# lim0606/pytorch-ardae-vae

Measured on AMD Instinct MI355X. Metric: AR-DAE-VAE train-steps/sec (batch 512, nz_cdae 256) on dbMNIST, higher is better.
Workload: dtype f32

## Files before the change

include/ardae_hip.h:

```cpp
#ifndef ARDAE_HIP_H
#define ARDAE_HIP_H

#include <stddef.h>
#include <stdint.h>

#ifdef __cplusplus
extern "C" {
#endif

#define ARDAE_ABI_VERSION 1

enum { ARDAE_ACT_NONE = 0, ARDAE_ACT_RELU = 1, ARDAE_ACT_SOFTPLUS = 2, ARDAE_ACT_ELU = 3, ARDAE_ACT_TANH = 4, ARDAE_ACT_LEAKY_RELU = 5, ARDAE_ACT_SWISH = 6 };

enum {
  ARDAE_EPI_ACT = 0,
  ARDAE_EPI_DACT = 1,
  ARDAE_EPI_CHAIN = 2,
  ARDAE_EPI_DAE_LOSS = 3
};

typedef struct ardae_lin_src {
  const float* x;
  int ld;
  int K;
  const float* wp;
} ardae_lin_src;

typedef struct ardae_linear_args {
  int M, Nout;
  int nsrc;
  ardae_lin_src src[2];
  int act;
  const float* bias;
  const float* rowbias;
  int rowbias_ld;
  int rows_per_group;
  const float* rowscale;
  const float* rowscale_w;
  const float* S; int ldS;
  const float* R; int ldR;
  const float* Q; int ldQ;
  const float* sigma;
  const float* eps; int ldeps;
  float scale;
  float* Y;  int ldY;
  float* Y2; int ldY2;
  float* colsum;
  float* tile_loss;
} ardae_linear_args;

const char* ardae_last_error(void);
int ardae_abi_version(void);

size_t ardae_packed_floats(int nout, int k);
int ardae_linear_row_tiles(int M, int nout);
int ardae_linear_col_panels(int M, int nout);
int ardae_pack_weight(const float* W, int ldw, int nout, int k, int transpose, float* out, void* stream);
int ardae_linear(const ardae_linear_args* args, int epilogue, void* stream);
int ardae_linear_chain_eligible(const ardae_linear_args* layers, int nl, int epilogue);
int ardae_linear_chain(const ardae_linear_args* layers, int nl, int epilogue, void* stream);
int ardae_linear_wide_layers_eligible(const ardae_linear_args* layers, int nl, int epilogue);
int ardae_linear_wide_layers(const ardae_linear_args* layers, int nl, int epilogue, void* stream);


#define ARDAE_WGRAD_MAX_PROBLEMS 20
typedef struct ardae_wgrad_problem {
  int M, O, I;
  int npairs;
  const float* G[2]; int ldG[2];
  const float* X[2]; int ldX[2];
  int bias_pair;
  const float* rowscale;
  int splits;
  float* partial;
  float* partial_vec;
  float* out; int ldout;
  float* out_bias;
  float* out_rowscale; int ld_rowscale;
  float beta;
} ardae_wgrad_problem;
int ardae_wgrad_splits(int M, int O, int I, int nproblems_hint);
int ardae_wgrad_batch(const ardae_wgrad_problem* problems, int nproblems, void* stream);


int ardae_latent_perturb(const float* latent, const float* z0, const float* xi, const float* eps, int B, int nz, int z,
                         float std_scale, float delta, float* xbar, float* sigma, float* std_b, void* stream);
int ardae_latent_perturb_nstd(const float* latent, const float* z0, const float* xi, const float* eps, int B, int nz, int nstd, int z,
                              float std_scale, float delta, float* xbar, float* sigma, float* std_b, void* stream);
int ardae_latent_perturb_draw_ok(int nz, int nstd, int z);
int ardae_latent_perturb_draw(const float* latent, const float* z0, int B, int nz, int z, float std_scale, float delta, uint64_t seed,
                              uint64_t offset_xi, uint64_t offset_eps, const void* state, uint64_t first_row, float* xbar, float* sigma,
                              float* eps_out, float* std_b, void* stream);
int ardae_center_scale(const float* latent, const float* z0, int B, int nz, int z, float std_scale, float* u, void* stream);
int ardae_philox_normal(float* out, int64_t n, uint64_t seed, uint64_t offset, void* stream);
int ardae_philox_uniform(float* out, int64_t n, uint64_t seed, uint64_t offset, void* stream);
int ardae_bernoulli(const float* p, int64_t rows, int cols, float* out, uint64_t seed, uint64_t offset, void* stream);
int ardae_adam_ref_step(float* p, const float* g, float* exp_avg, float* exp_avg_sq, float* max_exp_avg_sq, int64_t n,
                        double lr, double beta1, double beta2, double eps, int step, void* stream);
#define ARDAE_STEP_STATE_BYTES 32
int ardae_step_state_advance(void* state, uint64_t rng_inc, double lr, double beta1, double beta2, void* stream);
int ardae_philox_normal_dev(float* out, int64_t n, uint64_t seed, const void* state, uint64_t offset_add, void* stream);
int ardae_philox_normal_at(float* out, int64_t n, uint64_t seed, uint64_t offset, const void* state, uint64_t first_element,
                           void* stream);
int ardae_adam_ref_step_dev(float* p, const float* g, float* exp_avg, float* exp_avg_sq, float* max_exp_avg_sq, int64_t n,
                            double beta1, double beta2, double eps, const void* state, void* stream);
int ardae_train_state_advance(void* state, uint64_t rng_inc, double lr, double beta1, double beta2, double beta_init, double beta_fin,
                              int64_t beta_annealing, double std_scale, int64_t seed_rows, void* stream);
int ardae_seed_scale_dev(float* g, int64_t n, const void* state, void* stream);
#define ARDAE_WEIGHT_AVG_SWA 0
#define ARDAE_WEIGHT_AVG_POLYAK 1
int ardae_weight_avg(float* avg, const float* p, int64_t n, int kind, double decay, int64_t origin, const void* state, int64_t t,
                     void* stream);
int ardae_rmsprop_step(float* p, const float* g, float* square_avg, float* momentum_buffer, int64_t n, double lr,
                       double alpha, double eps, double momentum, void* stream);
int ardae_sgd_step(float* p, const float* g, int64_t n, double lr, void* stream);

typedef struct ardae_cdae_desc {
  int kind;
  int input_dim;
  int context_dim;
  int h_dim;
  int n_layers;
  int act;
} ardae_cdae_desc;
size_t ardae_cdae_param_floats(const ardae_cdae_desc* d);
size_t ardae_cdae_packed_floats(const ardae_cdae_desc* d);
size_t ardae_cdae_workspace_floats(const ardae_cdae_desc* d, int B, int S, int need_grads);
int ardae_cdae_pack(const ardae_cdae_desc* d, const float* params, float* packed, void* stream);
int ardae_cdae_loss_grads(const ardae_cdae_desc* d, const float* params, const float* packed, const float* xbar,
                          const float* sigma, const float* eps, const float* ctx, int B, int S, float* workspace,
                          size_t workspace_floats, float* loss, float* grads, float* score_out, void* stream);
int ardae_cdae_perturb_fused_ok(const ardae_cdae_desc* d, int nz, int nstd);
int ardae_cdae_perturb_loss_grads(const ardae_cdae_desc* d, const float* params, const float* packed, const float* latent, const float* z0,
                                  const float* ctx, int B, int nz, float std_scale, float delta, uint64_t seed, uint64_t offset_xi,
                                  uint64_t offset_eps, const void* state, uint64_t first_row, float* xbar, float* sigma, float* eps_out,
                                  float* std_b, float* workspace, size_t workspace_floats, float* loss, float* grads, void* stream);
int ardae_cdae_score(const ardae_cdae_desc* d, const float* params, const float* packed, const float* x,
                     const float* sigma, const float* ctx, int B, int S, float* workspace, size_t workspace_floats,
                     float* score_out, void* stream);


int ardae_dae_perturb(const float* x , const float* sigma , const float* eps ,
                      int B, int nsigma, int d, float* xbar, void* stream);
int ardae_dae_perturb_fused_ok(const ardae_cdae_desc* d, int nsigma);
int ardae_dae_perturb_loss_grads(const ardae_cdae_desc* d, const float* params, const float* packed, const float* x, int B, int nsigma,
                                 float delta, uint64_t seed, uint64_t offset_sigma, uint64_t offset_eps, const void* state,
                                 uint64_t first_row, float* xbar, float* sigma, float* eps_out, float* workspace,
                                 size_t workspace_floats, float* loss, float* grads, void* stream);

int ardae_dae_noise_perturb(const float* x , const float* eps , int B, int nsigma, int d, float sigma,
                            const void* dae_state, float* xbar, float* sigma_out , void* stream);
int ardae_dae_state_advance(void* state, uint64_t rng_inc, double lr, double beta1, double beta2, double sigma_max, double sigma_min,
                            int64_t sigma_annealing, void* stream);

int ardae_latent_noise_perturb(const float* latent, const float* z0, const float* eps, int B, int nz, int nstd, int z, float std_scale, float sigma,
                               const void* dae_state, float* xbar, float* sigma_out, void* stream);
int ardae_latent_noise_perturb_draw_ok(int nz, int nstd, int z);
int ardae_latent_noise_perturb_draw(const float* latent, const float* z0, int B, int nz, int nstd, int z, float std_scale, float sigma,
                                    const void* dae_state, uint64_t seed, uint64_t offset_eps, uint64_t first_row, float* xbar, float* sigma_out,
                                    float* eps_out, void* stream);

int ardae_philox_uniform_at(float* out, int64_t n, uint64_t seed, uint64_t offset, const void* state, uint64_t first_element, void* stream);
int ardae_recon_perturb(const float* x , const float* draw , int B, int nsigma, int d, int noise, float sigma,
                        const void* dae_state, float* xbar, float* sigma_out, float* target_out, void* stream);
int ardae_recon_perturb_draw(const float* x, int B, int nsigma, int d, int noise, float sigma, const void* dae_state, uint64_t seed, uint64_t offset,
                             uint64_t first_row, float* xbar, float* sigma_out, float* target_out, float* draw_out, void* stream);
int ardae_latent_recon_perturb(const float* latent, const float* z0, const float* draw, int B, int nz, int nstd, int z, float std_scale, int noise,
                               float sigma, const void* dae_state, float* xbar, float* sigma_out, float* target_out, void* stream);
int ardae_latent_recon_perturb_draw(const float* latent, const float* z0, int B, int nz, int nstd, int z, float std_scale, int noise, float sigma,
                                    const void* dae_state, uint64_t seed, uint64_t offset, uint64_t first_row, float* xbar, float* sigma_out,
                                    float* target_out, float* draw_out, void* stream);
int ardae_recon_score(const float* recon, const float* x, int n, int d, float sigma, const void* dae_state, float* out, void* stream);

#define ARDAE_FIT_STATE_BYTES 48
enum { ARDAE_ENERGY_REG = 0, ARDAE_ENERGY_1 = 1, ARDAE_ENERGY_2 = 2, ARDAE_ENERGY_3 = 3, ARDAE_ENERGY_4 = 4, ARDAE_ENERGY_NORMAL = 5 };
int ardae_energy(int kind, const float* x, int R, int d, float mu, float logvar, float* energy, float* grad, void* stream);
size_t ardae_energy_partial_floats(int R);
int ardae_energy_seed(int kind, const float* x, const float* score, int R, int d, float mu, float logvar, float alpha,
                      const void* fit_state, float* seed, float* mean_energy, float* partial, void* stream);
size_t ardae_gen_param_floats(int z_dim, int h_dim, int n_layers, int out_dim, int act);
size_t ardae_gen_packed_floats(int z_dim, int h_dim, int n_layers, int out_dim, int act);
size_t ardae_gen_workspace_floats(int z_dim, int h_dim, int n_layers, int out_dim, int act, int B);
int ardae_gen_pack(int z_dim, int h_dim, int n_layers, int out_dim, int act, const float* params, float* packed, void* stream);
int ardae_gen_forward(int z_dim, int h_dim, int n_layers, int out_dim, int act, const float* params, const float* packed, const float* z,
                      int B, float* workspace, size_t workspace_floats, float* x_out, void* stream);
int ardae_gen_backward(int z_dim, int h_dim, int n_layers, int out_dim, int act, const float* params, const float* packed, const float* z,
                       const float* dx, int B, float* workspace, size_t workspace_floats, float* grads, void* stream);
int ardae_gen_draw_fused_ok(int z_dim, int h_dim, int n_layers, int out_dim, int act);
int ardae_gen_draw_forward(int z_dim, int h_dim, int n_layers, int out_dim, int act, const float* params, const float* packed, int B,
                           uint64_t seed, uint64_t offset, const void* state, float* z_out, float* workspace, size_t workspace_floats,
                           float* x_out, void* stream);
int ardae_adam_torch_step_dev(float* p, const float* g, float* exp_avg, float* exp_avg_sq, int64_t n, double beta1, double beta2,
                              double eps, const void* state, void* stream);
int ardae_fit_state_advance(void* fit_state, uint64_t rng_inc, double lr0, double beta1, double beta2, int64_t lr_step_size,
                            double lr_gamma, double lr_min, double alpha_init, double alpha_fin, int64_t alpha_annealing, void* stream);


typedef struct ardae_model_desc {
  int kind;
  int input_dim, noise_dim, h_dim, z_dim;
  int n_layers;
  int act;
  int flags;
} ardae_model_desc;
enum { ARDAE_MODEL_NO_CENTER = 1,
       ARDAE_MODEL_HEAD_SHIFT = 1, ARDAE_MODEL_HEAD_MASK = 7 << 1,
       ARDAE_MODEL_CLIPPED = 16,
       ARDAE_MODEL_CLIP_Z0_SHIFT = 8, ARDAE_MODEL_CLIP_Z_SHIFT = 12, ARDAE_MODEL_CLIP_MASK = 0xff00 };
size_t ardae_model_param_floats(const ardae_model_desc* d);
size_t ardae_model_packed_floats(const ardae_model_desc* d);
size_t ardae_model_workspace_floats(const ardae_model_desc* d, int B, int nz, int mode);
int ardae_model_pack(const ardae_model_desc* d, const float* params, float* packed, void* stream);
int ardae_model_encode(const ardae_model_desc* d, const float* params, const float* packed, const float* x,
                       const float* noise, int B, int nz, float* workspace, size_t workspace_floats, float* z_out,
                       void* stream);
int ardae_model_encode_pair(const ardae_model_desc* d, const float* params, const float* packed, const float* x,
                            const float* noise, int B, int nz, float* workspace, size_t workspace_floats, float* z0_out,
                            float* z_out, int phase, void* stream);
int ardae_model_vae_forward(const ardae_model_desc* d, const float* params, const float* packed, const float* x,
                            const float* noise, int B, int nz, float beta, float* workspace, size_t workspace_floats,
                            float* z_out, float* losses, void* stream);
int ardae_model_vae_forward_dev(const ardae_model_desc* d, const float* params, const float* packed, const float* x,
                                const float* noise, int B, int nz, const void* state, float* workspace, size_t workspace_floats,
                                float* z_out, float* losses, void* stream);
int ardae_model_encode_hidden(const ardae_model_desc* d, const float* params, const float* packed, const float* x, int B,
                              float* workspace, size_t workspace_floats, float* z0_out, float* hidden_out, void* stream);
int ardae_model_encode_hidden_raw(const ardae_model_desc* d, const float* params, const float* packed, const float* x, const float* raw0, int B,
                                  float* workspace, size_t workspace_floats, float* z0_out, float* hidden_out, void* stream);
int ardae_model_decode(const ardae_model_desc* d, const float* params, const float* packed, const float* z, int R,
                       float* workspace, size_t workspace_floats, float* out0, float* out1, void* stream);
int ardae_model_loss_rows(const ardae_model_desc* d, const float* out0, const float* out1, const float* x, const float* z,
                          int rows, int nz, float* recon_row, float* prior_row, void* stream);
int ardae_model_vae_backward(const ardae_model_desc* d, const float* params, const float* packed, const float* x,
                             const float* noise, int B, int nz, float beta, float dloss, const float* dz_extra,
                             float* workspace, size_t workspace_floats, float* grads, float grads_beta, void* stream);
int ardae_model_vae_backward_dev(const ardae_model_desc* d, const float* params, const float* packed, const float* x,
                                 const float* noise, int B, int nz, const void* state, float dloss, const float* dz_extra,
                                 float* workspace, size_t workspace_floats, float* grads, float grads_beta, void* stream);
int ardae_model_vae_backward_decoder(const ardae_model_desc* d, const float* params, const float* packed, const float* x,
                                     const float* noise, int B, int nz, float beta, float dloss, float* workspace,
                                     size_t workspace_floats, void* stream);
int ardae_model_vae_backward_sampler(const ardae_model_desc* d, const float* params, const float* packed, const float* x,
                                     const float* noise, int B, int nz, const float* dz_extra, float seed_scale,
                                     float* workspace, size_t workspace_floats, float* grads, float grads_beta, void* stream);
int ardae_model_vae_backward_decoder_dev(const ardae_model_desc* d, const float* params, const float* packed, const float* x,
                                         const float* noise, int B, int nz, const void* state, float dloss, float* workspace,
                                         size_t workspace_floats, void* stream);
int ardae_model_vae_backward_sampler_dev(const ardae_model_desc* d, const float* params, const float* packed, const float* x,
                                         const float* noise, int B, int nz, const float* dz_extra, const void* state,
                                         float* workspace, size_t workspace_floats, float* grads, float grads_beta, void* stream);


int ardae_vae_head_fused_ok(const ardae_model_desc* d);
int ardae_vae_kld_rows(const float* mu, const float* lv, int B, int z, float* kld, void* stream);
int ardae_vae_head(const ardae_model_desc* d, const float* params, const float* packed, const float* hid, const float* eps, int B, uint64_t seed,
                   uint64_t offset, const void* state, int variant, float* mu, float* lv, float* z_out, float* eps_out, float* kld, void* stream);
int ardae_vae_forward(const ardae_model_desc* d, const float* params, const float* packed, const float* x, const float* eps, int B, float beta,
                      float loss_scale, uint64_t seed, uint64_t offset, const void* state, float* workspace, size_t workspace_floats, float* z_out,
                      float* eps_out, float* losses, void* stream);
int ardae_vae_forward_dev(const ardae_model_desc* d, const float* params, const float* packed, const float* x, const float* eps, int B,
                          const void* beta_state, float loss_scale, uint64_t seed, uint64_t offset, const void* state, float* workspace,
                          size_t workspace_floats, float* z_out, float* eps_out, float* losses, void* stream);
int ardae_vae_backward(const ardae_model_desc* d, const float* params, const float* packed, const float* x, int B, float beta, float loss_scale,
                       float* workspace, size_t workspace_floats, float* grads, float grads_beta, void* stream);
int ardae_vae_backward_dev(const ardae_model_desc* d, const float* params, const float* packed, const float* x, int B, const void* beta_state,
                           float loss_scale, float* workspace, size_t workspace_floats, float* grads, float grads_beta, void* stream);
int ardae_vae_encode_stats(const ardae_model_desc* d, const float* params, const float* packed, const float* x, int B, float* workspace,
                           size_t workspace_floats, float* mu_out, float* lv_out, void* stream);
int ardae_vae_iwae_draw(const float* mu, const float* lv, const float* eps, int B, int k, int z, uint64_t seed, uint64_t offset,
                        uint64_t first_element, float* z_out, float* logq, float* eps_out, void* stream);

int ardae_vae_aux_elbo_rows(const ardae_model_desc* d, const float* params, const float* packed, const float* x, const float* eps, int B, uint64_t seed,
                            uint64_t offset0, uint64_t offset1, uint64_t first_image, float* workspace, size_t workspace_floats, float* recon_rows,
                            float* kld_rows, void* stream);
int ardae_vae_pair_kld_rows(const float* mu1, const float* lv1, const float* mu2, const float* lv2, int B, int n, float* kld, void* stream);
int ardae_vae_aux_iwae_draw(const ardae_model_desc* d, const float* params, const float* packed, const float* x, const float* mu0, const float* lv0,
                            const float* eps, int B, int k, uint64_t seed, uint64_t offset0, uint64_t offset1, uint64_t first_image, float* workspace,
                            size_t workspace_floats, float* z_out, float* logq, float* eps_out, void* stream);

size_t ardae_conv_tail_workspace_floats(const ardae_model_desc* d, int R, int variant);
int ardae_conv_tail(const ardae_model_desc* d, const float* params, const float* packed, const float* u1, int R, int variant, float* workspace,
                    size_t workspace_floats, float* logits, void* stream);

size_t ardae_resconv_tail_workspace_floats(const ardae_model_desc* d, int R, int variant);
int ardae_resconv_tail(const ardae_model_desc* d, const float* params, const float* packed, const float* y14, int R, int variant, float* workspace,
                       size_t workspace_floats, float* logits, void* stream);

size_t ardae_resconv_mid_workspace_floats(const ardae_model_desc* d, int R, int variant);
int ardae_resconv_mid(const ardae_model_desc* d, const float* params, const float* packed, const float* y8, int R, int variant, float* workspace,
                      size_t workspace_floats, float* y14, void* stream);

int ardae_relaxed_bernoulli(const float* logit, const float* u, int64_t n, float temperature, float* sample, float* mean,
                            void* stream);
int ardae_gaussian_sample(const float* mu, const float* logvar, const float* eps, int64_t n, float* sample, void* stream);
int ardae_cholesky_batched(const float* A, int batch, int n, float* L, void* stream);

int ardae_iwae_proposal(const float* zs, const float* prop_noise, int B, int ke, int k, int z, float jitter, uint64_t seed, uint64_t offset,
                        uint64_t first_element, float* newz, float* logq, float* eps_out, float* mu, float* chol, void* stream);
int ardae_iwae_reduce(const float* recon, const float* prior, const float* logq, int B, int k, float* out, void* stream);

int ardae_philox_normal_scaled_at(float* out, int64_t n, uint64_t seed, uint64_t offset, const void* state, uint64_t first_element, int width,
                                  int nslots, const float* scale, void* stream);
int ardae_sample_logvar(const float* z, int B, int nz, int zd, float eps, float* logvar, void* stream);
int ardae_hist2d(const float* pts, int64_t n, int64_t row_stride, int nslots, int64_t slot_stride, int col_x, int col_y, double lo, double hi,
                 int bins, int64_t* counts, void* stream);
int ardae_hist2d_wide(const float* pts, int64_t n, int64_t row_stride, int nslots, int64_t slot_stride, int col_x, int col_y, double lo, double hi,
                      int bins, int64_t* counts, void* stream);


#define ARDAE_LOG_RECORD_FLOATS 16
int ardae_log_scalars(const float* cdae_loss, const float* model_losses, const float* std_b, int B, float beta, float d_lr,
                      const void* state, float* ring, int capacity, void* stream);
int ardae_log_scalars_dev(const float* cdae_loss, const float* model_losses, const float* std_b, int B, const void* beta_state, float d_lr,
                          const void* state, float* ring, int capacity, void* stream);
int ardae_gather_rows(const float* table, const int64_t* idx, int B, int D, float* out, void* stream);


#define ARDAE_DP_UNIQUE_ID_BYTES 128
const char* ardae_dp_backend(void);
int ardae_dp_unique_id(void* host_id);
int ardae_dp_comm_create(const void* host_id, int nranks, int rank, void** comm_out);
int ardae_dp_comm_query(void* comm, int* nranks, int* rank, int* device);
int ardae_dp_comm_destroy(void* comm);
int ardae_dp_allreduce_mean(void* comm, float* buf, size_t n, void* stream);


typedef struct ardae_profile_entry {
  char name[96];
  int calls;
  double total_ms;
  double flops;
  double bytes;
} ardae_profile_entry;
int ardae_profile_enable(int on);
int ardae_debug_stamp(unsigned long long* slots, int slot, void* stream);
int ardae_profile_report(ardae_profile_entry* entries, int max_entries);

#ifdef __cplusplus
}
#endif
#endif
```

pytorch-ardae-vae_amd/csrc/cdae.hip:

```cpp
#include <vector>

#include "ardae_hip.h"
#include "common.h"
#include "elementwise.h"
#include "host_util.h"

namespace ardae {
namespace {

bool cond_kind(int kind) { return kind < 2 || kind == 10 || kind == 11 || kind == 13 || kind == 16 || kind == 17; }
bool input_encoder_kind(int kind) { return kind < 2 || kind == 10 || kind == 11; }
bool sigma_column_kind(int kind) { return kind < 4 || kind == 16 || kind == 17; }

struct CdaeLayout {
  int kind, z, c, h, L, act;
  bool cond, enc_inp, grad, has_sigma;
  std::vector<Lin> ctx, inp, neg;
  size_t total = 0;
  int k1() const { return enc_inp ? h : z; }
  int sigma_col() const { return cond ? k1() + h : z; }

  explicit CdaeLayout(const ardae_cdae_desc& d)
      : kind(d.kind), z(d.input_dim), c(d.context_dim), h(d.h_dim), L(d.n_layers), act(d.act), cond(cond_kind(d.kind)), enc_inp(input_encoder_kind(d.kind)), grad(d.kind % 2 == 0), has_sigma(sigma_column_kind(d.kind)) {
    size_t off = 0;
    auto add = [&](std::vector<Lin>& v, int out, int in) { v.push_back(next_lin(off, out, in)); };
    if (cond)
      for (int l = 0; l < L; ++l) add(ctx, h, l == 0 ? c : h);
    if (enc_inp)
      for (int l = 0; l < L; ++l) add(inp, h, l == 0 ? z : h);
    for (int l = 0; l < L; ++l) add(neg, h, l == 0 ? sigma_col() + (has_sigma ? 1 : 0) : h);
    add(neg, grad ? 1 : z, h);
    total = off;
  }
};

struct PackedLayout {
  std::vector<size_t> ctx_f, ctx_b, inp_f, inp_b, neg_f, neg_b;
  size_t w1_f, w1_b, w1c_f, w1c_b, w1s;
  size_t fc_f, fc_b;
  PackedLayout(const CdaeLayout& P, PackList& pl) {
    const size_t L = P.L;
    for (auto* v : {&ctx_f, &ctx_b, &inp_f, &inp_b, &neg_f, &neg_b}) v->assign(L, 0);
    if (P.cond)
      for (size_t l = 0; l < L; ++l) { pl.pair(P.ctx[l], ctx_f[l], ctx_b[l]); if (P.enc_inp) pl.pair(P.inp[l], inp_f[l], inp_b[l]); }
    const Lin& W1 = P.neg[0];
    pl.pair(W1, w1_f, w1_b, 0, P.k1());
    w1c_f = w1c_b = 0;
    if (P.cond) pl.pair(W1, w1c_f, w1c_b, P.k1(), P.h);
    w1s = P.has_sigma ? pl.take(P.h) : 0;
    for (size_t l = 1; l < L; ++l) pl.pair(P.neg[l], neg_f[l], neg_b[l]);
    fc_f = fc_b = 0;
    if (!P.grad) pl.pair(P.neg[L], fc_f, fc_b);
  }
  explicit PackedLayout(const CdaeLayout& P, PackList&& sizing = PackList()) : PackedLayout(P, sizing) {}
};

int desc_ok(const ardae_cdae_desc* d) {
  ARDAE_CHECK_ARG(d != nullptr, "cdae: desc is NULL");
  ARDAE_CHECK_ARG((d->kind >= 0 && d->kind <= 3) || d->kind == 6 || d->kind == 7 || d->kind == 10 || d->kind == 11 || d->kind == 13 || d->kind == 16 || d->kind == 17,
                  "cdae: kind must be 0 (mlp-grad), 1 (mlp-res), 2 (unconditional grad), 3 (unconditional res), 6 (plain DAE grad), 7 (plain DAE res), "
                  "10 (plain conditional DAE grad), 11 (plain conditional DAE res), 13 (conditional DAE without an input encoder), "
                  "16 (mlp-grad without an input encoder) or 17 (mlp-res without an input encoder)");
  ARDAE_CHECK_ARG(!cond_kind(d->kind) || d->context_dim >= 1, "cdae: kinds 0 / 1 / 10 / 11 / 13 / 16 / 17 need context_dim >= 1 (got %d)", d->context_dim);
  ARDAE_CHECK_ARG(cond_kind(d->kind) || d->context_dim == 0, "cdae: kinds 2 / 3 / 6 / 7 have no context: context_dim must be 0 (got %d)", d->context_dim);
  ARDAE_CHECK_ARG(d->input_dim >= 1 && d->h_dim >= 1 && d->n_layers >= 1, "cdae: bad dimensions");
  ARDAE_CHECK_ARG(d->n_layers <= 6, "cdae: n_layers <= 6 supported (3L+1 gradient problems per batch)");
  ARDAE_CHECK_ARG(d->act > ACT_NONE && d->act <= ACT_LAST, "cdae: unknown activation %d", d->act);
  return 0;
}

struct CdaeWs {
  std::vector<float*> cL, a, hh, e, r, tau, taup, pbar, qbar, chat;
  float *cb, *gbar, *gbuf, *tile_loss, *chain_cnt, *Qsum, *cs_taup;
  int ltiles, ctiles;
};

void cdae_carve(const CdaeLayout& P, Bump& ws, int B, int S, bool need_grads, CdaeWs& W) {
  const int N = B * S, h = P.h, L = P.L, z = P.z;
  const size_t Bh = (size_t)B * h, Nh = (size_t)N * h;
  const bool cond = P.cond, enc = P.enc_inp, score = enc || P.grad;
  for (auto* v : {&W.cL, &W.a, &W.hh, &W.e, &W.r, &W.tau, &W.taup, &W.pbar, &W.qbar, &W.chat}) v->assign(L + 1, nullptr);
  W.cb = W.chain_cnt = W.Qsum = W.cs_taup = nullptr;
  if (cond) {
    for (int l = 1; l <= L; ++l) W.cL[l] = ws.take(Bh);
    W.cb = ws.take(Bh);
  }
  for (int l = 1; l <= L; ++l) {
    if (enc) W.a[l] = ws.take(Nh);
    W.hh[l] = ws.take(Nh);
    if (score) W.e[l] = ws.take(Nh);
    if (enc) W.r[l] = ws.take(Nh);
  }
  if (need_grads)
    for (int l = 1; l <= L; ++l) {
      if (enc) W.tau[l] = ws.take(Nh);
      if (score) W.taup[l] = ws.take(Nh);
      if (enc) W.pbar[l] = ws.take(Nh);
      W.qbar[l] = ws.take(Nh);
    }
  W.gbar = ws.take((size_t)N * z);
  W.gbuf = ws.take((size_t)N * z);
  W.ltiles = linear_row_tiles(N, z) * linear_col_panels(N, z);
  W.tile_loss = ws.take(W.ltiles);
  if (enc) W.chain_cnt = ws.take((size_t)LINEAR_SMALL_CHAIN_COUNTER_WORDS * ((N + 15) / 16));
  W.ctiles = linear_row_tiles(N, h);
  if (!need_grads) return;
  if (cond) {
    W.Qsum = ws.take(Bh);
    for (int l = 1; l <= L; ++l) W.chat[l] = ws.take(Bh);
  }
  if (score) W.cs_taup = ws.take((size_t)W.ctiles * h);
}

void cdae_wgrads(const CdaeLayout& P, const CdaeWs& W, const float* xbar, const float* sigma, const float* ctx, int B, int S, WgradList& wl, Bump& ws) {
  const int N = B * S, h = P.h, L = P.L, z = P.z;
  const std::vector<float*>&a = W.a, &hh = W.hh, &e = W.e, &r = W.r, &tau = W.tau, &taup = W.taup, &qhat = W.qbar, &phat = W.pbar;
  const int ld1 = P.neg[0].in;
  const size_t gW1 = P.neg[0].w;
  auto push = [&](const Lin& lin, int I, const float* s, const float* t, const float* ghat, const float* x, bool first) {
    const bool scol = first && P.has_sigma;
    const float* rs = scol ? sigma : nullptr;
    float* out_rs = scol ? wl.g(gW1 + P.sigma_col()) : nullptr;
    const int ld = first ? ld1 : I, ld_rs = scol ? ld1 : 0;
    if (P.grad) wl.push2(N, h, I, s, t, I, ghat, x, I, 1, rs, wl.g(lin.w), ld, wl.g(lin.b), out_rs, ld_rs);
    else wl.push2(N, h, I, ghat, x, I, nullptr, nullptr, 0, 0, rs, wl.g(lin.w), ld, wl.g(lin.b), out_rs, ld_rs);
  };
  if (P.enc_inp)
    for (int l = 1; l <= L; ++l)
      push(P.inp[l - 1], l == 1 ? z : h, r[l], l == 1 ? W.gbar : tau[l - 1], phat[l], l == 1 ? xbar : a[l - 1], false);
  push(P.neg[0], P.k1(), e[1], P.enc_inp ? tau[L] : W.gbar, qhat[1], P.enc_inp ? a[L] : xbar, true);
  if (P.cond) wl.push2(B, h, h, W.Qsum, W.cL[L], h, nullptr, nullptr, 0, -1, nullptr, wl.g(gW1 + P.k1()), ld1, nullptr, nullptr, 0);
  for (int l = 2; l <= L; ++l)
    push(P.neg[l - 1], h, e[l], taup[l - 1], qhat[l], hh[l - 1], false);
  if (!P.grad) wl.push2(N, z, h, W.gbar, hh[L], h, nullptr, nullptr, 0, 0, nullptr, wl.g(P.neg[L].w), h, wl.g(P.neg[L].b), nullptr, 0);
  if (P.cond)
    for (int l = 1; l <= L; ++l)
      wl.push2(B, h, P.ctx[l - 1].in, W.chat[l], l == 1 ? ctx : W.cL[l - 1], l == 1 ? P.c : h, nullptr, nullptr, 0, 0, nullptr,
               wl.g(P.ctx[l - 1].w), P.ctx[l - 1].in, wl.g(P.ctx[l - 1].b), nullptr, 0);
  wl.assign(ws, P.cond ? 3 * L + 1 : L + 1);
}

size_t workspace_floats(const CdaeLayout& P, int B, int S, bool need_grads) {
  Bump ws;
  CdaeWs W;
  cdae_carve(P, ws, B, S, need_grads, W);
  if (need_grads) {
    WgradList wl(nullptr);
    cdae_wgrads(P, W, nullptr, nullptr, nullptr, B, S, wl, ws);
  }
  return ws.off;
}

int cdae_pack_impl(const CdaeLayout& P, const float* params, float* packed, hipStream_t st) {
  PackList pl(params, packed);
  const PackedLayout K(P, pl);
  if (P.has_sigma) ARDAE_TRY(launch_gather_strided(params + P.neg[0].w + P.sigma_col(), P.neg[0].in, P.h, packed + K.w1s, st));
  return pl.launch(st);
}

LinArgs lin_args(int act, int M, int Nout, const float* x, int ldx, int K, const float* wp, LinArgs a) {
  a.M = M; a.Nout = Nout; a.nsrc = 1; a.act = act;
  a.src[0].x = x; a.src[0].ld = ldx; a.src[0].K = K; a.src[0].wp = wp;
  return a;
}

struct LayerRun {
  int epi;
  hipStream_t st;
  bool one_by_one;
  std::vector<LinArgs> v;
  LayerRun(int epi_, hipStream_t st_, bool one_by_one_ = false) : epi(epi_), st(st_), one_by_one(one_by_one_) {}
  void add(const LinArgs& a) { v.push_back(a); }
  int flush() {
    size_t i = 0;
    while (i < v.size()) {
      size_t n = one_by_one ? 1 : v.size() - i;
      while (n >= 2 && !linear_chain_eligible(v.data() + i, (int)n, epi)) --n;
      if (n >= 2) {
        ARDAE_TRY(launch_linear_chain(v.data() + i, (int)n, epi, st));
        i += n;
        continue;
      }
      size_t m = one_by_one ? 1 : std::min<size_t>(v.size() - i, 6);
      while (m >= 2 && !linear_wide_layers_eligible(v.data() + i, (int)m, epi)) --m;
      if (m >= 2) {
        ARDAE_TRY(launch_linear_wide_layers(v.data() + i, (int)m, epi, st));
        i += m;
      } else {
        ARDAE_TRY(launch_linear(v[i], epi, st));
        i += 1;
      }
    }
    v.clear();
    return 0;
  }
};

int cdae_impl(const ardae_cdae_desc* d, const float* params, const float* packed, const float* xbar, const float* sigma,
              const float* eps, const float* ctx, int B, int S, float* workspace, size_t ws_floats, float* loss, float* grads,
              float* score_out, bool need_grads, hipStream_t st, bool first_ready = false) {
  ARDAE_TRY(desc_ok(d));
  const CdaeLayout P(*d);
  const bool cond = P.cond, grad = P.grad;
  const bool enc = P.enc_inp;
  ARDAE_CHECK_ARG(cond || ctx == nullptr, "cdae: kinds 2 / 3 / 6 / 7 take no context: ctx must be NULL");
  const bool ctx_ready = first_ready && cond && !enc;
  ARDAE_CHECK_ARG(params && packed && xbar && (sigma || (!P.has_sigma && !need_grads)) && (ctx || !cond) && workspace, "cdae: null pointer argument");
  ARDAE_CHECK_ARG(B > 0 && S > 0 && (int64_t)B * S < (int64_t)1 << 30, "cdae: bad batch (B=%d, S=%d)", B, S);
  ARDAE_CHECK_ARG(!need_grads || (eps && loss && grads), "cdae: loss/grads/eps must be given");
  ARDAE_CHECK_ARG(need_grads || score_out, "cdae: score_out is NULL");
  const PackedLayout K(P);
  const int N = B * S, h = P.h, L = P.L, z = P.z, act = P.act, k1 = P.k1();
  Bump ws(workspace, ws_floats);
  CdaeWs W;
  cdae_carve(P, ws, B, S, need_grads, W);
  WgradList wl(grads);
  if (need_grads) cdae_wgrads(P, W, xbar, sigma, ctx, B, S, wl, ws);
  ARDAE_CHECK_ARG(ws.ok, "cdae: workspace too small (%zu < %zu floats)", ws_floats, ws.off);
  const std::vector<float*>&cL = W.cL, &a = W.a, &hh = W.hh, &e = W.e, &r = W.r, &tau = W.tau, &taup = W.taup, &pbar = W.pbar, &qbar = W.qbar, &chat = W.chat;
  float *cb = W.cb, *gbar = W.gbar, *Qsum = W.Qsum, *cs_taup = W.cs_taup;
  float* g = score_out ? score_out : W.gbuf;
  const float* x1 = enc ? a[L] : xbar;
  const float* wfc = params + P.neg[L].w;

  auto ctx_layer = [&](int l) { LinArgs A{}; A.bias = params + P.ctx[l - 1].b; A.Y = cL[l]; A.ldY = h;
                                return lin_args(act, B, h, l == 1 ? ctx : cL[l - 1], l == 1 ? P.c : h, P.ctx[l - 1].in, packed + K.ctx_f[l - 1], A); };
  auto inp_layer = [&](int l) { LinArgs A{}; A.bias = params + P.inp[l - 1].b; A.Y = a[l]; A.ldY = h;
                                return lin_args(act, N, h, l == 1 ? xbar : a[l - 1], l == 1 ? z : h, P.inp[l - 1].in, packed + K.inp_f[l - 1], A); };
  auto ctx_bias = [&]() {
    LinArgs A{}; A.bias = params + P.neg[0].b; A.Y = cb; A.ldY = h;
    return lin_args(ACT_NONE, B, h, cL[L], h, h, packed + K.w1c_f, A);
  };
  auto energy_layer = [&](int l) {
    LinArgs A{}; A.Y = hh[l]; A.ldY = h;
    if (l == 1 && P.has_sigma) { A.rowscale = sigma; A.rowscale_w = packed + K.w1s; }
    if (l == 1 && cond) { A.rowbias = cb; A.rowbias_ld = h; A.rows_per_group = S; } else A.bias = params + P.neg[l - 1].b;
    if (grad && l == L) { A.Y2 = e[L]; A.ldY2 = h; A.R = wfc; }
    return l == 1 ? lin_args(act, N, h, x1, k1, k1, packed + K.w1_f, A) : lin_args(act, N, h, hh[l - 1], h, h, packed + K.neg_f[l - 1], A);
  };
  auto e_layer = [&](int l) {
    LinArgs A{}; A.S = hh[l - 1]; A.ldS = h; A.Y = e[l - 1]; A.ldY = h;
    return lin_args(act, N, h, e[l], h, h, packed + K.neg_b[l - 1], A);
  };
  auto r_layer = [&](int l) {
    LinArgs A{}; A.S = a[l - 1]; A.ldS = h; A.Y = r[l - 1]; A.ldY = h;
    return l > L ? lin_args(act, N, h, e[1], h, h, packed + K.w1_b, A) : lin_args(act, N, h, r[l], h, h, packed + K.inp_b[l - 1], A);
  };
  auto g_layer = [&](LinArgs A) {
    A.Y = g; A.ldY = z;
    if (grad) return lin_args(ACT_NONE, N, z, enc ? r[1] : e[1], h, h, packed + (enc ? K.inp_b[0] : K.w1_b), A);
    A.bias = params + P.neg[L].b;
    return lin_args(ACT_NONE, N, z, hh[L], h, h, packed + K.fc_f, A);
  };

  if (!need_grads && enc && grad && N == B && linear_small_eligible(inp_layer(1), EPI_ACT)) {
    std::vector<LinArgs> pr; std::vector<int> ep, lv;
    int level = 0;
    auto add = [&](const LinArgs& A, int epi, int lev) { pr.push_back(A); ep.push_back(epi); lv.push_back(lev); };
    for (int l = 1; l <= L; ++l, ++level) { add(ctx_layer(l), EPI_ACT, level); add(inp_layer(l), EPI_ACT, level); }
    add(ctx_bias(), EPI_ACT, level++);
    for (int l = 1; l <= L; ++l) add(energy_layer(l), EPI_ACT, level++);
    for (int l = L; l >= 2; --l) add(e_layer(l), EPI_DACT, level++);
    for (int l = L + 1; l >= 2; --l) add(r_layer(l), EPI_DACT, level++);
    add(g_layer(LinArgs{}), EPI_ACT, level++);
    return launch_linear_small_chain(pr.data(), ep.data(), lv.data(), (int)pr.size(), W.chain_cnt, st);
  }
  {
    LayerRun run(EPI_ACT, st);
    if (enc && !first_ready && linear_small_eligible(inp_layer(1), EPI_ACT)) {
      for (int l = 1; l <= L; ++l) ARDAE_TRY(launch_linear_pair(ctx_layer(l), inp_layer(l), EPI_ACT, st));
      ARDAE_TRY(launch_linear(ctx_bias(), EPI_ACT, st));
    } else if (cond) {
      if (!ctx_ready) {
        for (int l = 1; l <= L; ++l) ARDAE_TRY(launch_linear(ctx_layer(l), EPI_ACT, st));
        ARDAE_TRY(launch_linear(ctx_bias(), EPI_ACT, st));
      }
      if (enc) for (int l = first_ready ? 2 : 1; l <= L; ++l) run.add(inp_layer(l));
    }
    for (int l = !enc && first_ready ? 2 : 1; l <= L; ++l) run.add(energy_layer(l));
    ARDAE_TRY(run.flush());
  }
  if (grad) {
    LayerRun run(EPI_DACT, st);
    for (int l = L; l >= 2; --l) run.add(e_layer(l));
    if (enc) for (int l = L + 1; l >= 2; --l) run.add(r_layer(l));
    ARDAE_TRY(run.flush());
  }
  if (!need_grads) return launch_linear(g_layer(LinArgs{}), EPI_ACT, st);
  const float inv_nz = 1.0f / ((float)N * (float)z);
  {
    LinArgs A{}; A.sigma = sigma; A.eps = eps; A.ldeps = z; A.scale = inv_nz; A.Y2 = gbar; A.ldY2 = z; A.tile_loss = W.tile_loss;
    ARDAE_TRY(launch_linear(g_layer(A), EPI_DAE_LOSS, st));
  }
  ARDAE_TRY(launch_sum_scale(W.tile_loss, W.ltiles, inv_nz, loss, st));

  const std::vector<float*>&qhat = qbar, &phat = pbar;
  if (grad) {
    LayerRun run(EPI_CHAIN, st);
    if (enc)
      for (int l = 1; l <= L; ++l) {
        LinArgs A{}; A.S = a[l]; A.ldS = h; A.R = r[l]; A.ldR = h; A.Y = tau[l]; A.ldY = h; A.Y2 = pbar[l]; A.ldY2 = h;
        run.add(l == 1 ? lin_args(act, N, h, gbar, z, z, packed + K.inp_f[0], A) : lin_args(act, N, h, tau[l - 1], h, h, packed + K.inp_f[l - 1], A));
      }
    for (int l = 1; l <= L; ++l) {
      LinArgs A{}; A.S = hh[l]; A.ldS = h; A.R = e[l]; A.ldR = h; A.Y = taup[l]; A.ldY = h; A.Y2 = qbar[l]; A.ldY2 = h;
      if (l == L) A.colsum = cs_taup;
      run.add(l == 1 ? lin_args(act, N, h, enc ? tau[L] : gbar, k1, k1, packed + K.w1_f, A) : lin_args(act, N, h, taup[l - 1], h, h, packed + K.neg_f[l - 1], A));
    }
    ARDAE_TRY(run.flush());
    ARDAE_TRY(launch_segment_sum(cs_taup, h, 1, W.ctiles, h, -1.0f, grads + P.neg[L].w, h, st));
  } else {
    LinArgs A{}; A.S = hh[L]; A.ldS = h; A.Y = qhat[L]; A.ldY = h;
    ARDAE_TRY(lin1(EPI_DACT, act, N, h, gbar, z, z, packed + K.fc_b, A, st));
  }
  {
    LayerRun run(EPI_DACT, st, cond && !grad);
    for (int l = L; l >= 2; --l) {
      LinArgs A{}; A.S = hh[l - 1]; A.ldS = h; A.Y = qhat[l - 1]; A.ldY = h;
      if (grad) { A.Q = qbar[l - 1]; A.ldQ = h; }
      run.add(lin_args(act, N, h, qhat[l], h, h, packed + K.neg_b[l - 1], A));
    }
    if (enc)
      for (int l = L + 1; l >= 2; --l) {
        LinArgs A{}; A.S = a[l - 1]; A.ldS = h; A.Y = phat[l - 1]; A.ldY = h;
        if (grad) { A.Q = pbar[l - 1]; A.ldQ = h; }
        run.add(l > L ? lin_args(act, N, h, qhat[1], h, h, packed + K.w1_b, A) : lin_args(act, N, h, phat[l], h, h, packed + K.inp_b[l - 1], A));
      }
    ARDAE_TRY(run.flush());
  }
  if (cond) {
    ARDAE_TRY(launch_segment_sum(qhat[1], h, B, S, h, 1.0f, Qsum, h, st));
    for (int l = L + 1; l >= 2; --l) {
      LinArgs A{}; A.S = cL[l - 1]; A.ldS = h; A.Y = chat[l - 1]; A.ldY = h;
      ARDAE_TRY(lin1(EPI_DACT, act, B, h, l > L ? Qsum : chat[l], h, h, packed + (l > L ? K.w1c_b : K.ctx_b[l - 1]), A, st));
    }
  }

  return wl.launch(st);
}

}

int dae_front_slots(const ardae_cdae_desc* d, int N, float* workspace, size_t ws_floats, size_t* w1, size_t* b1, float** h1) {
  ARDAE_TRY(desc_ok(d));
  const CdaeLayout P(*d);
  ARDAE_CHECK_ARG(!P.cond, "dae_perturb_loss_grads: the network must be unconditional");
  const size_t need = workspace_floats(P, N, 1, true);
  ARDAE_CHECK_ARG(ws_floats >= need, "dae_perturb_loss_grads: workspace too small (%zu < %zu floats)", ws_floats, need);
  Bump ws(workspace, ws_floats);
  CdaeWs W;
  cdae_carve(P, ws, N, 1, true, W);
  *w1 = P.neg[0].w; *b1 = P.neg[0].b; *h1 = W.hh[1];
  return 0;
}
int dae_loss_grads_from_h1(const ardae_cdae_desc* d, const float* params, const float* packed, const float* xbar, const float* sigma, const float* eps,
                           int N, float* workspace, size_t ws_floats, float* loss, float* grads, hipStream_t st) {
  return cdae_impl(d, params, packed, xbar, sigma, eps, nullptr, N, 1, workspace, ws_floats, loss, grads, nullptr, true, st, true);
}

}

using namespace ardae;

extern "C" {

size_t ardae_cdae_param_floats(const ardae_cdae_desc* d) {
  if (desc_ok(d) != 0) return 0;
  return CdaeLayout(*d).total;
}
size_t ardae_cdae_packed_floats(const ardae_cdae_desc* d) {
  if (desc_ok(d) != 0) return 0;
  PackList pl;
  PackedLayout(CdaeLayout(*d), pl);
  return pl.total();
}
size_t ardae_cdae_workspace_floats(const ardae_cdae_desc* d, int B, int S, int need_grads) {
  if (desc_ok(d) != 0 || B <= 0 || S <= 0) return 0;
  return workspace_floats(CdaeLayout(*d), B, S, need_grads != 0);
}
int ardae_cdae_pack(const ardae_cdae_desc* d, const float* params, float* packed, void* stream) {
  ARDAE_TRY(desc_ok(d));
  ARDAE_CHECK_ARG(params && packed, "cdae_pack: null pointer");
  return cdae_pack_impl(CdaeLayout(*d), params, packed, (hipStream_t)stream);
}
int ardae_cdae_loss_grads(const ardae_cdae_desc* d, const float* params, const float* packed, const float* xbar,
                          const float* sigma, const float* eps, const float* ctx, int B, int S, float* workspace,
                          size_t workspace_floats, float* loss, float* grads, float* score_out, void* stream) {
  return cdae_impl(d, params, packed, xbar, sigma, eps, ctx, B, S, workspace, workspace_floats, loss, grads, score_out, true,
                   (hipStream_t)stream);
}
int ardae_cdae_perturb_fused_ok(const ardae_cdae_desc* d, int nz, int nstd) {
  if (desc_ok(d) != 0) return 0;
  const CdaeLayout P(*d);
  return P.cond && P.has_sigma && nstd == 1 && latent_perturb_draw_fwd_ok(nz, P.z, P.h, P.act) ? 1 : 0;
}
int ardae_cdae_perturb_loss_grads(const ardae_cdae_desc* d, const float* params, const float* packed, const float* latent, const float* z0,
                                  const float* ctx, int B, int nz, float std_scale, float delta, uint64_t seed, uint64_t offset_xi,
                                  uint64_t offset_eps, const void* state, uint64_t first_row, float* xbar, float* sigma, float* eps_out,
                                  float* std_b, float* workspace, size_t ws_floats, float* loss, float* grads, void* stream) {
  ARDAE_TRY(desc_ok(d));
  ARDAE_CHECK_ARG(ardae_cdae_perturb_fused_ok(d, nz, 1), "cdae_perturb_loss_grads: shape not eligible (nz=%d): use ardae_latent_perturb* + ardae_cdae_loss_grads", nz);
  ARDAE_CHECK_ARG(params && packed && workspace && B > 0, "cdae_perturb_loss_grads: null pointer argument");
  const CdaeLayout P(*d);
  const PackedLayout K(P);
  ARDAE_CHECK_ARG(ws_floats >= workspace_floats(P, B, nz, true), "cdae_perturb_loss_grads: workspace too small");
  Bump ws(workspace, ws_floats);
  CdaeWs W;
  cdae_carve(P, ws, B, nz, true, W);
  const hipStream_t st = (hipStream_t)stream;
  if (!P.enc_inp) {
    ARDAE_CHECK_ARG(latent && z0 && ctx && xbar && sigma && eps_out && std_b && loss && grads, "cdae_perturb_loss_grads: null pointer argument");
    const int h = P.h, L = P.L;
    for (int l = 1; l <= L; ++l) {
      LinArgs A{}; A.bias = params + P.ctx[l - 1].b; A.Y = W.cL[l]; A.ldY = h;
      ARDAE_TRY(launch_linear(lin_args(P.act, B, h, l == 1 ? ctx : W.cL[l - 1], l == 1 ? P.c : h, P.ctx[l - 1].in, packed + K.ctx_f[l - 1], A), EPI_ACT, st));
    }
    LinArgs A{}; A.bias = params + P.neg[0].b; A.Y = W.cb; A.ldY = h;
    ARDAE_TRY(launch_linear(lin_args(ACT_NONE, B, h, W.cL[L], h, h, packed + K.w1c_f, A), EPI_ACT, st));
    const bool seed_e = P.grad && L == 1;
    ARDAE_TRY(launch_latent_perturb_draw_fwd(latent, z0, B, nz, P.z, std_scale, delta, seed, offset_xi, offset_eps, state, first_row, xbar, sigma, eps_out,
                                             std_b, packed + K.w1_f, W.cb, h, P.act, W.hh[1], st, packed + K.w1s, seed_e ? params + P.neg[L].w : nullptr,
                                             seed_e ? W.e[1] : nullptr));
    return cdae_impl(d, params, packed, xbar, sigma, eps_out, ctx, B, nz, workspace, ws_floats, loss, grads, nullptr, true, st, true);
  }
  ARDAE_TRY(launch_latent_perturb_draw_fwd(latent, z0, B, nz, P.z, std_scale, delta, seed, offset_xi, offset_eps, state, first_row, xbar, sigma,
                                           eps_out, std_b, packed + K.inp_f[0], params + P.inp[0].b, P.h, P.act, W.a[1],
                                           (hipStream_t)stream));
  return cdae_impl(d, params, packed, xbar, sigma, eps_out, ctx, B, nz, workspace, ws_floats, loss, grads, nullptr, true, (hipStream_t)stream,
                   true);
}
int ardae_cdae_score(const ardae_cdae_desc* d, const float* params, const float* packed, const float* x, const float* sigma,
                     const float* ctx, int B, int S, float* workspace, size_t workspace_floats, float* score_out, void* stream) {
  return cdae_impl(d, params, packed, x, sigma, nullptr, ctx, B, S, workspace, workspace_floats, nullptr, nullptr, score_out, false,
                   (hipStream_t)stream);
}

}
```

pytorch-ardae-vae_amd/csrc/elementwise.h:

```cpp
#pragma once
#include "ardae_hip.h"
#include "common.h"

namespace ardae {

struct DevFloat {
  float v;
  const float* p;
  DevFloat(float v_) : v(v_), p(nullptr) {}
  explicit DevFloat(const float* p_) : v(0.f), p(p_) {}
};
DevFloat train_state_beta(const void* state);
DevFloat train_state_seed_scale(const void* state);

int launch_latent_perturb(const float* latent, const float* z0, const float* xi, const float* eps, int B, int nz, int nstd, int zd,
                          float std_scale, float delta, float* xbar, float* sigma, float* std_b, hipStream_t st);
bool latent_perturb_draw_ok(int nz, int nstd, int zd);
int launch_latent_perturb_draw(const float* latent, const float* z0, int B, int nz, int zd, float std_scale, float delta, uint64_t seed,
                               uint64_t off_xi, uint64_t off_eps, const void* state, uint64_t first_row, float* xbar, float* sigma,
                               float* eps_out, float* std_b, hipStream_t st);
bool latent_perturb_draw_fwd_ok(int nz, int zd, int h, int act);
int launch_latent_perturb_draw_fwd(const float* latent, const float* z0, int B, int nz, int zd, float std_scale, float delta, uint64_t seed,
                                   uint64_t off_xi, uint64_t off_eps, const void* state, uint64_t first_row, float* xbar, float* sigma,
                                   float* eps_out, float* std_b, const float* wp1, const float* bias1, int h, int act, float* a1_out,
                                   hipStream_t st, const float* w1s = nullptr, const float* wfc = nullptr, float* e1_out = nullptr);
int launch_center_scale(const float* latent, const float* z0, int B, int nz, int zd, float std_scale, float* u,
                        hipStream_t st);
int launch_segment_sum(const float* in, int ld, int groups, int rows_per_group, int cols, float scale, float* out, int ldout,
                       hipStream_t st);
int launch_sum_scale(const float* in, int n, float scale, float* out, hipStream_t st);
int launch_gather_strided(const float* src, int stride, int n, float* dst, hipStream_t st);
int launch_philox_normal(float* out, int64_t n, uint64_t seed, uint64_t offset, hipStream_t st);
int launch_philox_normal_dev(float* out, int64_t n, uint64_t seed, const void* state, uint64_t offset_add, hipStream_t st);
int launch_philox_normal_at(float* out, int64_t n, uint64_t seed, uint64_t offset, const void* state, uint64_t first_element, hipStream_t st);
int launch_step_state_advance(void* state, uint64_t rng_inc, double lr, double beta1, double beta2, hipStream_t st);
int launch_train_state_advance(void* state, uint64_t rng_inc, double lr, double beta1, double beta2, double beta_init, double beta_fin,
                               int64_t beta_annealing, double std_scale, int64_t seed_rows, hipStream_t st);
int launch_dae_state_advance(void* state, uint64_t rng_inc, double lr, double beta1, double beta2, double sigma_max, double sigma_min,
                             int64_t sigma_annealing, hipStream_t st);
DevFloat dae_state_sigma(const void* state);
int launch_adam_ref_dev(float* p, const float* g, float* m, float* v, float* vmax, int64_t n, double beta1, double beta2, double eps,
                        const void* state, hipStream_t st);
int launch_philox_uniform(float* out, int64_t n, uint64_t seed, uint64_t offset, hipStream_t st);
int launch_bernoulli(const float* p, int64_t rows, int cols, float* out, uint64_t seed, uint64_t offset, hipStream_t st);

int launch_adam_ref(float* p, const float* g, float* m, float* v, float* vmax, int64_t n, double lr, double beta1, double beta2,
                    double eps, int step, hipStream_t st);
int launch_weight_avg(float* avg, const float* p, int64_t n, int kind, double decay, int64_t origin, const void* state, int64_t t,
                      hipStream_t st);
int launch_rmsprop(float* p, const float* g, float* sq, float* buf, int64_t n, double lr, double alpha, double eps,
                   double momentum, hipStream_t st);

int launch_axpy(const float* x, int64_t n, DevFloat alpha, float* y, hipStream_t st);
int launch_scale(float* y, int64_t n, DevFloat alpha, hipStream_t st);
int launch_fill(float* y, int64_t n, float v, hipStream_t st);
int launch_copy(const float* x, int64_t n, float* y, hipStream_t st);
int launch_copy2d(const float* x, int64_t ldx, float* y, int64_t ldy, int64_t rows, int64_t cols, hipStream_t st);
int launch_affine(const float* x, int64_t n, float alpha, float beta, float* y, hipStream_t st);
int launch_vae_loss(int kind, const float* o0, const float* o1, const float* x, const float* z, int rows, int nz, int D, int zd,
                    DevFloat beta, int write_grads, float gscale, const float* dz_extra, float* rec_row, float* pri_row, float* do0,
                    float* do1, float* dzq, hipStream_t st);
int launch_vae_loss_finalize(const float* rec_row, const float* pri_row, int rows, DevFloat beta, float* losses, hipStream_t st);

}
```

pytorch-ardae-vae_amd/csrc/elementwise.hip:

```cpp
#include "elementwise.h"
#include "linear.h"
#include "philox.h"

namespace ardae {
namespace {

__device__ __forceinline__ int64_t step_state_advance1(StepState* s, uint64_t rng_inc, double lr, double beta1, double beta2) {
  s->rng_offset += rng_inc;
  const int64_t t = s->adam_step + 1;
  s->adam_step = t;
  const double bc1 = 1.0 - pow(beta1, (double)t), bc2 = 1.0 - pow(beta2, (double)t);
  s->adam_step_size = (float)(lr / bc1);
  s->adam_sqrt_bc2 = (float)sqrt(bc2);
  return t;
}

__global__ void step_state_advance_kernel(StepState* s, uint64_t rng_inc, double lr, double beta1, double beta2) {
  if (blockIdx.x != 0 || threadIdx.x != 0) return;
  step_state_advance1(s, rng_inc, lr, beta1, beta2);
}

__global__ void train_state_advance_kernel(TrainState* s, uint64_t rng_inc, double lr, double beta1, double beta2, double beta_init,
                                           double beta_fin, int64_t beta_annealing, double std_scale, int64_t seed_rows) {
#pragma clang fp contract(off)
// ... 177 lines not shown
    }
  } else {
#pragma unroll
    for (int j = 0; j < NV; ++j) ev[j] = (t + 256 * j < per_image) ? eps[base + t + 256 * j] : 0.f;
  }
  float s = 0.f;
#pragma unroll
  for (int j = 0; j < NV; ++j) {
    u[j] = std_scale * (u[j] - z0d);
    if (t + 256 * j < per_image) s += u[j];
  }
  red[t] = s;
  __syncthreads();
  if (t < zd) {
    float acc = 0.f;
    for (int g = 0; g < RG; ++g) acc += red[g * zd + t];
    stat[t] = acc / (float)nz;
  }
  __syncthreads();
  const float mean = stat[d];
  __syncthreads();
  float ss = 0.f;
#pragma unroll
  for (int j = 0; j < NV; ++j) {
    const float c = u[j] - mean;
    if (t + 256 * j < per_image) ss += c * c;
  }
  red[t] = ss;
  __syncthreads();
  if (t < zd) {
    float acc = 0.f;
    for (int g = 0; g < RG; ++g) acc += red[g * zd + t];
    stat[t] = sqrtf(acc / (float)(nz - 1));
  }
  __syncthreads();
  if (t == 0) {
    float acc = 0.f;
    for (int i = 0; i < zd; ++i) acc += stat[i];
    red[0] = delta * (acc / (float)zd);
  }
  __syncthreads();
  const float sb = red[0];
  if (t == 0 && (!FWD || blockIdx.y == 0)) std_b[b] = sb;
  const int r0 = t / zd;
  if (FWD) __syncthreads();
#pragma unroll
  for (int j = 0; j < NV; ++j) {
    if (t + 256 * j < per_image && j >= j0 && j < j1) {
      const size_t row = (size_t)b * nz + r0 + RG * j;
      const float sg = sb * (DRAW ? nbuf[xi_at + r0 + RG * (j - j0)] : xi[row]);
      const float xb = u[j] + sg * ev[j];
      xbar[base + t + 256 * j] = xb;
      if (FWD) nbuf[(r0 + RG * (j - j0)) * (zd + LP_XPAD) + d] = xb;
      if (d == 0) sigma[row] = sg;
    }
  }
  if (FWD) {
    __syncthreads();
    const int lane = t & 63, wave = t >> 6, l31 = lane & 31, hh = lane >> 5;
    const int kch = zd >> 3, nrb = rows_sl >> 5, ncb = dr.h >> 5, ld = zd + LP_XPAD;
    for (int cb = wave; cb < ncb; cb += 4) {
      f32x4 bv[8];
      const float* bp = dr.wp1 + (size_t)cb * kch * 256 + lane * 4;
#pragma unroll
      for (int c = 0; c < 8; ++c)
        if (c < kch) bv[c] = *reinterpret_cast<const f32x4*>(bp + (size_t)c * 256);
      const int col = cb * 32 + l31;
      const float bc = SC ? dr.bias1[(size_t)b * dr.h + col] : dr.bias1[col];
      const float wsg = SC ? dr.w1s[col] : 0.f, wv = (SC && dr.wfc) ? dr.wfc[col] : 0.f;
      for (int rb = 0; rb < nrb; ++rb) {
        f32x16 acc;
#pragma unroll
        for (int r = 0; r < 16; ++r) acc[r] = 0.f;
        const float* arow = nbuf + (rb * 32 + l31) * ld + 4 * hh;
#pragma unroll
        for (int c = 0; c < 8; ++c)
          if (c < kch) {
            const f32x4 av = *reinterpret_cast<const f32x4*>(arow + 8 * c);
#pragma unroll
            for (int q = 0; q < 4; ++q) acc = __builtin_amdgcn_mfma_f32_32x32x2f32(av[q], bv[c][q], acc, 0, 0, 0);
          }
        float* yo = dr.a1_out + ((size_t)b * nz + RG * j0 + rb * 32 + 4 * hh) * dr.h + col;
#pragma unroll
        for (int r = 0; r < 16; ++r) {
          const int rr = (r & 3) + 8 * (r >> 2);
          if (SC) {
            const float y = act_fwd<FWD>(acc[r] + bc + sb * nbuf[xi_at + rb * 32 + 4 * hh + rr] * wsg);
            yo[(size_t)rr * dr.h] = y;
            if (dr.e1_out) dr.e1_out[(yo - dr.a1_out) + (size_t)rr * dr.h] = -wv * act_d1<FWD>(y);
          } else {
            yo[(size_t)rr * dr.h] = act_fwd<FWD>(acc[r] + bc);
          }
        }
      }
    }
  }
}

__global__ void center_scale_kernel(const float* __restrict__ latent, const float* __restrict__ z0, int64_t n, int nz, int zd,
                                    float std_scale, float* __restrict__ u) {
  const int64_t e = (int64_t)blockIdx.x * blockDim.x + threadIdx.x;
  if (e >= n) return;
  const int64_t row = e / zd;
  const int d = (int)(e - row * zd);
  u[e] = std_scale * (latent[e] - z0[(row / nz) * zd + d]);
}

template <int NT>
__global__ __launch_bounds__(NT) void segment_sum_kernel(const float* __restrict__ in, int ld, int rows_per_group, int cols,
                                                         float scale, float* __restrict__ out, int ldout) {
  constexpr int RL = NT / 64;
  __shared__ float red[NT];
  const int g = blockIdx.x, c = blockIdx.y * 64 + (threadIdx.x & 63), rl = threadIdx.x >> 6;
  float s[8];
#pragma unroll
  for (int j = 0; j < 8; ++j) s[j] = 0.f;
  if (c < cols) {
    const float* p = in + (size_t)g * rows_per_group * ld + c;
    int r = rl;
    for (; r + 7 * RL < rows_per_group; r += 8 * RL) {
#pragma unroll
      for (int j = 0; j < 8; ++j) s[j] += p[(size_t)(r + j * RL) * ld];
    }
    for (; r < rows_per_group; r += RL) s[0] += p[(size_t)r * ld];
  }
  red[threadIdx.x] = ((s[0] + s[1]) + (s[2] + s[3])) + ((s[4] + s[5]) + (s[6] + s[7]));
  __syncthreads();
  if (rl == 0 && c < cols) {
    float t = 0.f;
#pragma unroll
    for (int j = 0; j < RL; ++j) t += red[threadIdx.x + 64 * j];
    out[(size_t)g * ldout + c] = scale * t;
  }
}

__global__ __launch_bounds__(256) void sum_scale_kernel(const float* __restrict__ in, int n, float scale, float* __restrict__ out) {
  __shared__ float red[256];
  float s = 0.f;
  for (int i = threadIdx.x; i < n; i += 256) s += in[i];
  red[threadIdx.x] = s;
  __syncthreads();
  for (int w = 128; w > 0; w >>= 1) {
    if ((int)threadIdx.x < w) red[threadIdx.x] += red[threadIdx.x + w];
    __syncthreads();
  }
  if (threadIdx.x == 0) out[0] = red[0] * scale;
}

__global__ void gather_strided_kernel(const float* __restrict__ src, int stride, int n, float* __restrict__ dst) {
  const int i = blockIdx.x * blockDim.x + threadIdx.x;
  if (i < n) dst[i] = src[(size_t)i * stride];
}

__global__ void adam_ref_kernel(float* __restrict__ p, const float* __restrict__ g, float* __restrict__ m, float* __restrict__ v,
                                float* __restrict__ vmax, int64_t n, float beta1, float beta2, float eps, float step_size,
                                float sqrt_bc2, const StepState* state) {
  if (state) {
    step_size = state->adam_step_size;
    sqrt_bc2 = state->adam_sqrt_bc2;
  }
  for (int64_t i = (int64_t)blockIdx.x * blockDim.x + threadIdx.x; i < n; i += (int64_t)gridDim.x * blockDim.x) {
    const float gi = g[i];
    const float mi = m[i] * beta1 + (1.f - beta1) * gi;
    float vi = v[i] * beta2 + (1.f - beta2) * gi * gi;
    m[i] = mi;
    v[i] = vi;
    if (vmax) {
      vi = fmaxf(vmax[i], vi);
      vmax[i] = vi;
    }
    const float denom = (sqrtf(vi) + eps) / sqrt_bc2;
    p[i] = p[i] - step_size * (mi / denom);
  }
}

__global__ void rmsprop_kernel(float* __restrict__ p, const float* __restrict__ g, float* __restrict__ sq, float* __restrict__ buf,
                               int64_t n, float lr, float alpha, float eps, float momentum) {
  for (int64_t i = (int64_t)blockIdx.x * blockDim.x + threadIdx.x; i < n; i += (int64_t)gridDim.x * blockDim.x) {
    const float gi = g[i];
    const float s = sq[i] * alpha + (1.f - alpha) * gi * gi;
    sq[i] = s;
    const float avg = sqrtf(s) + eps;
    if (momentum > 0.f) {
      const float bi = buf[i] * momentum + gi / avg;
      buf[i] = bi;
      p[i] = p[i] - lr * bi;
    } else {
      p[i] = p[i] - lr * (gi / avg);
    }
  }
}

__device__ __forceinline__ float weight_avg1(float a, float q, float w, bool first) {
#pragma clang fp contract(off)
  return first ? q : a + (q - a) * w;
}

__global__ __launch_bounds__(256) void weight_avg_kernel(float* __restrict__ avg, const float* __restrict__ p, int64_t n, int kind,
                                                         float w_polyak, int64_t origin, const StepState* state, int64_t t_host) {
  const int64_t t = state ? state->adam_step : t_host;
  if (t < origin) return;
  const int64_t k = t - origin;
  const bool first = k == 0;
  const float w = kind == ARDAE_WEIGHT_AVG_SWA ? (float)(1.0 / (double)(k + 1)) : w_polyak;
  const uintptr_t ma = reinterpret_cast<uintptr_t>(avg) & 15, mp = reinterpret_cast<uintptr_t>(p) & 15;
  int64_t head = n, nvec = 0;
  if (ma == mp) {
    head = (int64_t)((16 - ma) & 15) / 4;
    if (head > n) head = n;
    nvec = (n - head) / 4;
  }
  const int64_t tail0 = head + 4 * nvec;
  const int64_t tid = (int64_t)blockIdx.x * blockDim.x + threadIdx.x, stride = (int64_t)gridDim.x * blockDim.x;
  f32x4* __restrict__ av = reinterpret_cast<f32x4*>(avg + head);
  const f32x4* __restrict__ pv = reinterpret_cast<const f32x4*>(p + head);
  for (int64_t i = tid; i < nvec; i += stride) {
    const f32x4 q = pv[i];
    f32x4 a = first ? q : av[i];
    a.x = weight_avg1(a.x, q.x, w, first);
    a.y = weight_avg1(a.y, q.y, w, first);
    a.z = weight_avg1(a.z, q.z, w, first);
    a.w = weight_avg1(a.w, q.w, w, first);
    av[i] = a;
  }
  for (int64_t i = tid; i < head; i += stride) avg[i] = weight_avg1(avg[i], p[i], w, first);
  for (int64_t i = tail0 + tid; i < n; i += stride) avg[i] = weight_avg1(avg[i], p[i], w, first);
}

__global__ void axpy_kernel(const float* __restrict__ x, int64_t n, float alpha, const float* __restrict__ alpha_dev, float* __restrict__ y) {
  if (alpha_dev) alpha = *alpha_dev;
  for (int64_t i = (int64_t)blockIdx.x * blockDim.x + threadIdx.x; i < n; i += (int64_t)gridDim.x * blockDim.x) y[i] += alpha * x[i];
}

__global__ __launch_bounds__(256) void scale_kernel(float* __restrict__ y, int64_t n, float alpha, const float* __restrict__ alpha_dev) {
  if (alpha_dev) alpha = *alpha_dev;
  int64_t head = (int64_t)((16 - (reinterpret_cast<uintptr_t>(y) & 15)) & 15) / 4;
  if (head > n) head = n;
  const int64_t nvec = (n - head) / 4, tail0 = head + 4 * nvec;
  const int64_t tid = (int64_t)blockIdx.x * blockDim.x + threadIdx.x, stride = (int64_t)gridDim.x * blockDim.x;
  f32x4* __restrict__ yv = reinterpret_cast<f32x4*>(y + head);
  for (int64_t i = tid; i < nvec; i += stride) {
    f32x4 v = yv[i];
    v.x *= alpha; v.y *= alpha; v.z *= alpha; v.w *= alpha;
    yv[i] = v;
  }
  for (int64_t i = tid; i < head; i += stride) y[i] *= alpha;
  for (int64_t i = tail0 + tid; i < n; i += stride) y[i] *= alpha;
}

__global__ void fill_kernel(float* __restrict__ y, int64_t n, float v) {
  for (int64_t i = (int64_t)blockIdx.x * blockDim.x + threadIdx.x; i < n; i += (int64_t)gridDim.x * blockDim.x) y[i] = v;
}
__global__ void copy2d_kernel(const float* __restrict__ x, int64_t ldx, float* __restrict__ y, int64_t ldy, int64_t rows, int64_t cols) {
  const int64_t n = rows * cols;
  for (int64_t i = (int64_t)blockIdx.x * blockDim.x + threadIdx.x; i < n; i += (int64_t)gridDim.x * blockDim.x) {
    const int64_t r = i / cols, c = i - r * cols;
    y[r * ldy + c] = x[r * ldx + c];
  }
}

__global__ void affine_kernel(const float* __restrict__ x, int64_t n, float alpha, float beta, float* __restrict__ y) {
  for (int64_t i = (int64_t)blockIdx.x * blockDim.x + threadIdx.x; i < n; i += (int64_t)gridDim.x * blockDim.x) y[i] = alpha * x[i] + beta;
}

__device__ __forceinline__ float block_sum_256(float v, float* red) {
#pragma unroll
  for (int off = 32; off > 0; off >>= 1) v += __shfl_xor(v, off);
  __syncthreads();
  if ((threadIdx.x & 63) == 0) red[threadIdx.x >> 6] = v;
  __syncthreads();
  return (red[0] + red[1]) + (red[2] + red[3]);
}

template <int KIND>
__global__ __launch_bounds__(256) void vae_loss_kernel(const float* __restrict__ o0, const float* __restrict__ o1,
                                                       const float* __restrict__ x, const float* __restrict__ z, int nz, int D, int zd,
                                                       float beta, const float* __restrict__ beta_dev, int write_grads, float gscale,
                                                       const float* __restrict__ dz_extra, float* __restrict__ rec_row,
                                                       float* __restrict__ pri_row, float* __restrict__ do0, float* __restrict__ do1,
                                                       float* __restrict__ dzq) {
  __shared__ float red[4];
  if (beta_dev) beta = *beta_dev;
  const int r = blockIdx.x;
  const float* xr = x + (size_t)(r / nz) * D;
  const size_t base = (size_t)r * D;
  const float LOG2PI = 1.8378770664093453f;
  float acc = 0.f;
  for (int d = threadIdx.x; d < D; d += 256) {
    const float t = xr[d];
    if (KIND == 0) {
      const float l = o0[base + d];
      const float e = __expf(-fabsf(l));
      acc += fmaxf(l, 0.f) - l * t + (e < 1e-4f ? e * (1.f - 0.5f * e) : __logf(1.f + e));
      if (write_grads) {
        const float sg = l >= 0.f ? 1.f / (1.f + e) : e / (1.f + e);
        do0[base + d] = gscale * (sg - t);
      }
    } else {
      const float mu = o0[base + d], lv = o1[base + d];
      const float iv = __expf(-lv), df = t - mu;
      acc += 0.5f * (lv + df * df * iv + LOG2PI);
      if (write_grads) {
        do0[base + d] = -gscale * df * iv;
        do1[base + d] = 0.5f * gscale * (1.f - df * df * iv);
      }
    }
  }
  const float rec = block_sum_256(acc, red);
  float pa = 0.f;
  for (int d = threadIdx.x; d < zd; d += 256) {
    const float zv = z[(size_t)r * zd + d];
    pa += 0.5f * (zv * zv + LOG2PI);
    if (write_grads) dzq[(size_t)r * zd + d] = gscale * beta * zv + (dz_extra ? dz_extra[(size_t)r * zd + d] : 0.f);
  }
  const float pri = block_sum_256(pa, red);
  if (threadIdx.x == 0) {
    rec_row[r] = rec;
    pri_row[r] = pri;
  }
}

__global__ __launch_bounds__(256) void vae_loss_finalize_kernel(const float* __restrict__ rec_row, const float* __restrict__ pri_row,
                                                                int rows, float beta, const float* __restrict__ beta_dev,
                                                                float* __restrict__ losses) {
  __shared__ float red[4];
  if (beta_dev) beta = *beta_dev;
  float a = 0.f, b = 0.f;
  for (int i = threadIdx.x; i < rows; i += 256) {
    a += rec_row[i];
    b += pri_row[i];
  }
  const float ra = block_sum_256(a, red);
  const float rb = block_sum_256(b, red);
  if (threadIdx.x == 0) {
    const float inv = 1.f / (float)rows;
    losses[0] = (ra + beta * rb) * inv;
    losses[1] = ra * inv;
    losses[2] = rb * inv;
  }
}

inline int grid_for(int64_t n, int cap = 4096) {
// ... 83 lines not shown
                  "latent_perturb: need B>0, nz>=2 (unbiased std), nstd>=1, 1<=z<=256 (B=%d nz=%d nstd=%d z=%d)", B, nz, nstd, zd);
  int zp = 1;
  while (zp < zd) zp <<= 1;
  const int64_t per_image = (int64_t)nz * zd;
  const bool reg_ok = nstd == 1 && zp == zd && zd <= 256 && per_image >= 256 * 4;
  const PerturbDraw nodraw{};
#define ARDAE_LP_REG(NV_)                                                                                                                      \
  hipLaunchKernelGGL((latent_perturb_reg_kernel<NV_, false>), dim3(B), dim3(256), 0, st, latent, z0, xi, eps, nz, zd, std_scale, delta, xbar, \
                     sigma, std_b, nodraw)
  if (reg_ok && per_image <= 256 * 8) ARDAE_LP_REG(8);
  else if (reg_ok && per_image <= 256 * 16) ARDAE_LP_REG(16);
  else if (reg_ok && per_image <= 256 * 32) ARDAE_LP_REG(32);
  else if (reg_ok && per_image <= 256 * 64) ARDAE_LP_REG(64);
  else if (reg_ok && per_image <= 256 * 96) ARDAE_LP_REG(96);
  else
    hipLaunchKernelGGL(latent_perturb_kernel, dim3(B), dim3(256), 0, st, latent, z0, xi, eps, nz, nstd, zd, zp, std_scale, delta, xbar,
                       sigma, std_b);
#undef ARDAE_LP_REG
  ARDAE_LAUNCH_CHECK();
  return 0;
}

int launch_center_scale(const float* latent, const float* z0, int B, int nz, int zd, float std_scale, float* u, hipStream_t st) {
  ARDAE_CHECK_ARG(latent && z0 && u && B > 0 && nz > 0 && zd > 0, "center_scale: bad arguments");
  const int64_t n = (int64_t)B * nz * zd;
  hipLaunchKernelGGL(center_scale_kernel, dim3((unsigned)((n + 255) / 256)), dim3(256), 0, st, latent, z0, n, nz, zd, std_scale, u);
  ARDAE_LAUNCH_CHECK();
  return 0;
}

int launch_segment_sum(const float* in, int ld, int groups, int rows_per_group, int cols, float scale, float* out, int ldout,
                       hipStream_t st) {
  ARDAE_CHECK_ARG(in && out && groups > 0 && rows_per_group > 0 && cols > 0 && ld >= cols && ldout >= cols, "segment_sum: bad arguments");
  if ((int64_t)groups * ceil_div(cols, 64) < 256 && rows_per_group >= 128)
    hipLaunchKernelGGL(segment_sum_kernel<1024>, dim3(groups, ceil_div(cols, 64)), dim3(1024), 0, st, in, ld, rows_per_group, cols, scale, out, ldout);
  else
    hipLaunchKernelGGL(segment_sum_kernel<256>, dim3(groups, ceil_div(cols, 64)), dim3(256), 0, st, in, ld, rows_per_group, cols, scale, out, ldout);
  ARDAE_LAUNCH_CHECK();
  return 0;
}

int launch_sum_scale(const float* in, int n, float scale, float* out, hipStream_t st) {
  ARDAE_CHECK_ARG(in && out && n > 0, "sum_scale: bad arguments");
  hipLaunchKernelGGL(sum_scale_kernel, dim3(1), dim3(256), 0, st, in, n, scale, out);
  ARDAE_LAUNCH_CHECK();
  return 0;
}

int launch_gather_strided(const float* src, int stride, int n, float* dst, hipStream_t st) {
  ARDAE_CHECK_ARG(src && dst && n > 0 && stride > 0, "gather_strided: bad arguments");
  hipLaunchKernelGGL(gather_strided_kernel, dim3((n + 255) / 256), dim3(256), 0, st, src, stride, n, dst);
  ARDAE_LAUNCH_CHECK();
  return 0;
}

int launch_philox_normal(float* out, int64_t n, uint64_t seed, uint64_t offset, hipStream_t st) {
  ARDAE_CHECK_ARG(out && n > 0, "philox_normal: bad arguments");
  const int64_t q = (n + 3) / 4;
  hipLaunchKernelGGL(philox_normal_kernel, dim3((unsigned)((q + 255) / 256)), dim3(256), 0, st, out, n, seed, offset,
                     (const StepState*)nullptr, (uint64_t)0);
  ARDAE_LAUNCH_CHECK();
  return 0;
}

int launch_philox_normal_at(float* out, int64_t n, uint64_t seed, uint64_t offset, const void* state, uint64_t first_element, hipStream_t st) {
  ARDAE_CHECK_ARG(out && n > 0, "philox_normal_at: bad arguments");
  ARDAE_CHECK_ARG((first_element & 3) == 0, "philox_normal_at: first_element must be a multiple of 4 (one Philox counter = 4 normals)");
  const int64_t q = (n + 3) / 4;
  hipLaunchKernelGGL(philox_normal_kernel, dim3((unsigned)((q + 255) / 256)), dim3(256), 0, st, out, n, seed, offset,
                     (const StepState*)state, first_element >> 2);
  ARDAE_LAUNCH_CHECK();
  return 0;
}

int launch_philox_normal_dev(float* out, int64_t n, uint64_t seed, const void* state, uint64_t offset_add, hipStream_t st) {
  ARDAE_CHECK_ARG(state, "philox_normal_dev: bad arguments");
  return launch_philox_normal_at(out, n, seed, offset_add, state, 0, st);
}

int launch_step_state_advance(void* state, uint64_t rng_inc, double lr, double beta1, double beta2, hipStream_t st) {
  ARDAE_CHECK_ARG(state, "step_state_advance: null state");
  hipLaunchKernelGGL(step_state_advance_kernel, dim3(1), dim3(64), 0, st, (StepState*)state, rng_inc, lr, beta1, beta2);
  ARDAE_LAUNCH_CHECK();
  return 0;
}

int launch_train_state_advance(void* state, uint64_t rng_inc, double lr, double beta1, double beta2, double beta_init, double beta_fin,
                               int64_t beta_annealing, double std_scale, int64_t seed_rows, hipStream_t st) {
  ARDAE_CHECK_ARG(state, "train_state_advance: null state");
  ARDAE_CHECK_ARG(beta_annealing != 0 && seed_rows > 0, "train_state_advance: beta_annealing must be positive (or negative: no annealing) and seed_rows positive");
  hipLaunchKernelGGL(train_state_advance_kernel, dim3(1), dim3(64), 0, st, (TrainState*)state, rng_inc, lr, beta1, beta2, beta_init, beta_fin,
                     beta_annealing, std_scale, seed_rows);
  ARDAE_LAUNCH_CHECK();
  return 0;
}

int launch_dae_state_advance(void* state, uint64_t rng_inc, double lr, double beta1, double beta2, double sigma_max, double sigma_min,
                             int64_t sigma_annealing, hipStream_t st) {
  ARDAE_CHECK_ARG(state, "dae_state_advance: null state");
  hipLaunchKernelGGL(dae_state_advance_kernel, dim3(1), dim3(64), 0, st, (DaeState*)state, rng_inc, lr, beta1, beta2, sigma_max, sigma_min,
                     sigma_annealing);
  ARDAE_LAUNCH_CHECK();
  return 0;
}

DevFloat train_state_beta(const void* state) { return DevFloat(&((const TrainState*)state)->beta); }
DevFloat train_state_seed_scale(const void* state) { return DevFloat(&((const TrainState*)state)->seed_scale); }
DevFloat dae_state_sigma(const void* state) { return DevFloat(&((const DaeState*)state)->sigma); }

int launch_philox_uniform(float* out, int64_t n, uint64_t seed, uint64_t offset, hipStream_t st) {
  ARDAE_CHECK_ARG(out && n > 0, "philox_uniform: bad arguments");
  const int64_t q = (n + 3) / 4;
  hipLaunchKernelGGL(philox_uniform_kernel, dim3((unsigned)((q + 255) / 256)), dim3(256), 0, st, out, n, seed, offset);
  ARDAE_LAUNCH_CHECK();
  return 0;
}

int launch_bernoulli(const float* p, int64_t rows, int cols, float* out, uint64_t seed, uint64_t offset, hipStream_t st) {
  ARDAE_CHECK_ARG(p && out && rows > 0 && cols > 0, "bernoulli: bad arguments");
  const int64_t q = (rows * cols + 3) / 4;
  hipLaunchKernelGGL(bernoulli_kernel, dim3((unsigned)((q + 255) / 256)), dim3(256), 0, st, p, rows, cols, out, seed, offset);
  ARDAE_LAUNCH_CHECK();
  return 0;
}

int launch_adam_ref(float* p, const float* g, float* m, float* v, float* vmax, int64_t n, double lr, double beta1, double beta2,
                    double eps, int step, hipStream_t st) {
  ARDAE_CHECK_ARG(p && g && m && v && n > 0 && step >= 1, "adam_ref: bad arguments");
  const double bc1 = 1.0 - pow(beta1, step), bc2 = 1.0 - pow(beta2, step);
  hipLaunchKernelGGL(adam_ref_kernel, dim3(grid_for(n)), dim3(256), 0, st, p, g, m, v, vmax, n, (float)beta1, (float)beta2,
                     (float)eps, (float)(lr / bc1), (float)sqrt(bc2), (const StepState*)nullptr);
  ARDAE_LAUNCH_CHECK();
  return 0;
}

int launch_adam_ref_dev(float* p, const float* g, float* m, float* v, float* vmax, int64_t n, double beta1, double beta2, double eps,
                        const void* state, hipStream_t st) {
  ARDAE_CHECK_ARG(p && g && m && v && n > 0 && state, "adam_ref_dev: bad arguments");
  hipLaunchKernelGGL(adam_ref_kernel, dim3(grid_for(n)), dim3(256), 0, st, p, g, m, v, vmax, n, (float)beta1, (float)beta2,
                     (float)eps, 0.f, 1.f, (const StepState*)state);
  ARDAE_LAUNCH_CHECK();
  return 0;
}

int launch_rmsprop(float* p, const float* g, float* sq, float* buf, int64_t n, double lr, double alpha, double eps, double momentum,
                   hipStream_t st) {
  ARDAE_CHECK_ARG(p && g && sq && n > 0 && (momentum <= 0.0 || buf), "rmsprop: bad arguments");
  hipLaunchKernelGGL(rmsprop_kernel, dim3(grid_for(n)), dim3(256), 0, st, p, g, sq, buf, n, (float)lr, (float)alpha, (float)eps,
                     (float)momentum);
  ARDAE_LAUNCH_CHECK();
  return 0;
}

int launch_weight_avg(float* avg, const float* p, int64_t n, int kind, double decay, int64_t origin, const void* state, int64_t t,
                      hipStream_t st) {
  ARDAE_CHECK_ARG(avg && p && n > 0 && origin >= 1, "weight_avg: bad arguments");
  ARDAE_CHECK_ARG(kind == ARDAE_WEIGHT_AVG_SWA || (kind == ARDAE_WEIGHT_AVG_POLYAK && decay >= 0.0 && decay <= 1.0),
                  "weight_avg: kind must be ARDAE_WEIGHT_AVG_SWA or ARDAE_WEIGHT_AVG_POLYAK (0 <= decay <= 1)");
  ARDAE_CHECK_ARG((const char*)avg + n * 4 <= (const char*)p || (const char*)p + n * 4 <= (const char*)avg, "weight_avg: avg and p overlap");
  hipLaunchKernelGGL(weight_avg_kernel, dim3(grid_for((n + 3) / 4)), dim3(256), 0, st, avg, p, n, kind, (float)(1.0 - decay), origin,
                     (const StepState*)state, t);
  ARDAE_LAUNCH_CHECK();
  return 0;
}

int launch_axpy(const float* x, int64_t n, DevFloat alpha, float* y, hipStream_t st) {
  ARDAE_CHECK_ARG(x && y && n > 0, "axpy: bad arguments");
  hipLaunchKernelGGL(axpy_kernel, dim3(grid_for(n)), dim3(256), 0, st, x, n, alpha.v, alpha.p, y);
  ARDAE_LAUNCH_CHECK();
  return 0;
}

int launch_scale(float* y, int64_t n, DevFloat alpha, hipStream_t st) {
  ARDAE_CHECK_ARG(y && n > 0, "scale: bad arguments");
  hipLaunchKernelGGL(scale_kernel, dim3(grid_for((n + 3) / 4)), dim3(256), 0, st, y, n, alpha.v, alpha.p);
  ARDAE_LAUNCH_CHECK();
  return 0;
}

int launch_fill(float* y, int64_t n, float v, hipStream_t st) {
  ARDAE_CHECK_ARG(y && n > 0, "fill: bad arguments");
  hipLaunchKernelGGL(fill_kernel, dim3(grid_for(n)), dim3(256), 0, st, y, n, v);
  ARDAE_LAUNCH_CHECK();
  return 0;
}

int launch_copy2d(const float* x, int64_t ldx, float* y, int64_t ldy, int64_t rows, int64_t cols, hipStream_t st) {
  ARDAE_CHECK_ARG(x && y && rows > 0 && cols > 0 && ldx >= cols && ldy >= cols, "copy2d: bad arguments");
  hipLaunchKernelGGL(copy2d_kernel, dim3(grid_for(rows * cols)), dim3(256), 0, st, x, ldx, y, ldy, rows, cols);
  ARDAE_LAUNCH_CHECK();
  return 0;
}

int launch_copy(const float* x, int64_t n, float* y, hipStream_t st) { return launch_copy2d(x, n, y, n, 1, n, st); }

int launch_affine(const float* x, int64_t n, float alpha, float beta, float* y, hipStream_t st) {
  ARDAE_CHECK_ARG(x && y && n > 0, "affine: bad arguments");
  hipLaunchKernelGGL(affine_kernel, dim3(grid_for(n)), dim3(256), 0, st, x, n, alpha, beta, y);
  ARDAE_LAUNCH_CHECK();
  return 0;
}

int launch_vae_loss(int kind, const float* o0, const float* o1, const float* x, const float* z, int rows, int nz, int D, int zd,
                    DevFloat beta, int write_grads, float gscale, const float* dz_extra, float* rec_row, float* pri_row, float* do0,
                    float* do1, float* dzq, hipStream_t st) {
  ARDAE_CHECK_ARG(o0 && x && z && rec_row && pri_row && rows > 0 && nz > 0 && D > 0 && zd > 0, "vae_loss: bad arguments");
  ARDAE_CHECK_ARG(kind == 0 || (kind == 1 && o1), "vae_loss: kind 1 needs the logvar head");
  ARDAE_CHECK_ARG(!write_grads || (do0 && dzq && (kind == 0 || do1)), "vae_loss: gradient outputs missing");
  if (kind == 0)
    hipLaunchKernelGGL(vae_loss_kernel<0>, dim3(rows), dim3(256), 0, st, o0, o1, x, z, nz, D, zd, beta.v, beta.p, write_grads, gscale, dz_extra,
                       rec_row, pri_row, do0, do1, dzq);
  else
    hipLaunchKernelGGL(vae_loss_kernel<1>, dim3(rows), dim3(256), 0, st, o0, o1, x, z, nz, D, zd, beta.v, beta.p, write_grads, gscale, dz_extra,
                       rec_row, pri_row, do0, do1, dzq);
  ARDAE_LAUNCH_CHECK();
  return 0;
}

int launch_vae_loss_finalize(const float* rec_row, const float* pri_row, int rows, DevFloat beta, float* losses, hipStream_t st) {
  ARDAE_CHECK_ARG(rec_row && pri_row && losses && rows > 0, "vae_loss_finalize: bad arguments");
  hipLaunchKernelGGL(vae_loss_finalize_kernel, dim3(1), dim3(256), 0, st, rec_row, pri_row, rows, beta.v, beta.p, losses);
  ARDAE_LAUNCH_CHECK();
  return 0;
}

}
```

pytorch-ardae-vae_amd/csrc/host_util.h:

```cpp
#pragma once
#include <algorithm>
#include <cstring>
#include <vector>

#include "common.h"
#include "elementwise.h"
#include "linear.h"
#include "wgrad.h"

namespace ardae {

inline size_t al64(size_t n) { return (n + 63) & ~size_t(63); }
inline unsigned nblk(int64_t n) { return (unsigned)((n + 255) / 256); }

struct Bump {
  float* base; size_t cap; size_t off = 0; bool ok = true;
  Bump(float* b, size_t c) : base(b), cap(c) {}
  Bump() : base(nullptr), cap(~size_t(0) >> 2) {}
  float* take(size_t n) {
    size_t o = off; off += al64(n);
    if (off > cap) { ok = false; return base; }
    return base ? base + o : nullptr;
  }
};

inline int lin1(int epi, int act, int M, int Nout, const float* x, int ldx, int K, const float* wp, LinArgs a, hipStream_t st) {
  a.M = M; a.Nout = Nout; a.nsrc = 1; a.act = act;
  a.src[0].x = x; a.src[0].ld = ldx; a.src[0].K = K; a.src[0].wp = wp;
  return launch_linear(a, epi, st);
}
inline int lin2(int epi, int act, int M, int Nout, const float* x0, int ld0, int K0, const float* wp0, const float* x1, int ld1, int K1, const float* wp1,
                LinArgs a, hipStream_t st) {
  a.M = M; a.Nout = Nout; a.nsrc = 2; a.act = act;
  a.src[0].x = x0; a.src[0].ld = ld0; a.src[0].K = K0; a.src[0].wp = wp0;
  a.src[1].x = x1; a.src[1].ld = ld1; a.src[1].K = K1; a.src[1].wp = wp1;
  return launch_linear(a, epi, st);
}

inline int dense_fwd(int act, int M, int n, const float* x, int ldx, int K, const float* wp, const float* bias, float* y, hipStream_t st) {
  LinArgs A{}; A.bias = bias; A.Y = y; A.ldY = n;
  return lin1(EPI_ACT, act, M, n, x, ldx, K, wp, A, st);
}
inline int dense_bwd(int act, int M, int n, const float* g, int K, const float* wp, const float* S, float* y, hipStream_t st, const float* Q = nullptr) {
  LinArgs A{}; A.S = S; A.ldS = n; A.Q = Q; A.ldQ = Q ? n : 0; A.Y = y; A.ldY = n;
  return lin1(EPI_DACT, act, M, n, g, K, K, wp, A, st);
}
inline int dense_bwd2(int act, int M, int n, const float* g0, const float* wp0, const float* g1, const float* wp1, int K, const float* S, float* y,
                      hipStream_t st) {
  LinArgs A{}; A.S = S; A.ldS = n; A.Y = y; A.ldY = n;
  return lin2(EPI_DACT, act, M, n, g0, K, K, wp0, g1, K, K, wp1, A, st);
}

struct Lin { size_t w, b; int out, in; };
inline Lin next_lin(size_t& off, int out, int in, int nbias = -1) {
  Lin l; l.out = out; l.in = in; l.w = off; off += (size_t)out * in; l.b = off; off += nbias < 0 ? out : nbias;
  return l;
}

struct PackList {
  std::vector<PackItem> items;
  const float* params; float* packed;
  size_t off = 0;
  PackList() : params(nullptr), packed(nullptr) {}
  PackList(const float* params_, float* packed_) : params(params_), packed(packed_) {}
  size_t take(size_t n) { size_t o = off; off += al64(n); return o; }
  size_t panel(size_t src, int ldw, int nout, int k, bool transpose, bool src_in_packed = false) {
    const size_t o = take(packed_floats(nout, k));
    if (packed) {
      if (items.empty()) items.reserve(PACK_BATCH_MAX);
      items.push_back(PackItem{(src_in_packed ? packed : params) + src, ldw, nout, k, transpose ? 1 : 0, packed + o});
    }
    return o;
  }
  void pair(const Lin& l, size_t& f, size_t& b, int col0 = 0, int k = 0) {
    if (k == 0) k = l.in;
    f = panel(l.w + col0, l.in, l.out, k, false);
    b = panel(l.w + col0, l.in, k, l.out, true);
  }
  size_t total() const { return off; }
  int launch(hipStream_t st) { return launch_pack_batch(items.data(), (int)items.size(), st); }
};

struct WgradList {
  std::vector<WgradProblem> probs;
  float* grads;
  float beta;
  size_t next = 0;
  explicit WgradList(float* grads_, float beta_ = 0.f) : grads(grads_), beta(beta_) {}
  float* g(size_t off) const { return grads ? grads + off : nullptr; }

  WgradProblem& push(int M, int O, int I, const float* G, const float* X, int ldX, float* out, int ldout, float* out_bias) {
    WgradProblem p;
    memset(&p, 0, sizeof(p));
    p.M = M; p.O = O; p.I = I; p.npairs = 1;
    p.G[0] = G; p.ldG[0] = O; p.X[0] = X; p.ldX[0] = ldX;
    p.bias_pair = out_bias ? 0 : -1;
    p.out = out; p.ldout = ldout; p.out_bias = out_bias; p.beta = beta;
    return add(p);
  }
  WgradProblem& push2(int M, int O, int I, const float* G0, const float* X0, int ldX0, const float* G1, const float* X1, int ldX1, int bias_pair,
                      const float* rowscale, float* out, int ldout, float* out_bias, float* out_rs, int ld_rs) {
    WgradProblem p;
    memset(&p, 0, sizeof(p));
    p.M = M; p.O = O; p.I = I;
    p.npairs = G1 ? 2 : 1;
    p.G[0] = G0; p.ldG[0] = O; p.X[0] = X0; p.ldX[0] = ldX0;
    p.G[1] = G1; p.ldG[1] = O; p.X[1] = X1; p.ldX[1] = ldX1;
    p.bias_pair = bias_pair; p.rowscale = rowscale;
    p.out = out; p.ldout = ldout; p.out_bias = out_bias; p.out_rowscale = out_rs; p.ld_rowscale = ld_rs; p.beta = beta;
    return add(p);
  }
  WgradProblem& add(const WgradProblem& p) {
    if (probs.empty()) probs.reserve(WGRAD_MAX_PROBLEMS + 2);
    probs.push_back(p);
    return probs.back();
  }
  size_t pending() const { return probs.size() - next; }
  void assign(Bump& ws, int hint, size_t n = ~size_t(0)) {
    const size_t end = next + std::min(n, pending());
    for (size_t i = next; i < end; ++i) {
      WgradProblem& p = probs[i];
      p.splits = wgrad_splits(p.M, p.O, p.I, hint);
      p.partial = ws.take((size_t)p.splits * p.O * p.I);
      p.partial_vec = ws.take((size_t)p.splits * 2 * p.O);
    }
  }
  int launch(hipStream_t st, size_t n = ~size_t(0)) {
    const size_t end = next + std::min(n, pending());
    while (next < end) {
      const size_t m = std::min<size_t>(end - next, WGRAD_MAX_PROBLEMS);
      ARDAE_TRY(launch_wgrad_batch(probs.data() + next, (int)m, st));
      next += m;
    }
    return 0;
  }
};

inline int cat_fwd(int act, int B, int rpg, int n, const float* ctx, int cw, const float* wp_ctx, const float* bias, const float* s, int sd, const float* wp_s,
                   float* rb, float* y, hipStream_t st) {
  ARDAE_TRY(dense_fwd(ACT_NONE, B, n, ctx, cw, cw, wp_ctx, bias, rb, st));
  LinArgs A{}; A.Y = y; A.ldY = n; A.rowbias = rb; A.rowbias_ld = n; A.rows_per_group = rpg;
  return lin1(EPI_ACT, act, B * rpg, n, s, sd, sd, wp_s, A, st);
}
inline int cat_bwd(int M, int n, const float* dpre, int sd, const float* wb_s, const float* qs, float* ds, int cw, const float* wb_ctx, const float* qc,
                   float* dctx, hipStream_t st) {
  auto half = [&](int k, const float* wb, const float* q, float* y) {
    if (q) return dense_bwd(ACT_NONE, M, k, dpre, n, wb, q, y, st, q);
    return dense_fwd(ACT_NONE, M, k, dpre, n, n, wb, nullptr, y, st);
  };
  ARDAE_TRY(half(sd, wb_s, qs, ds));
  return dctx ? half(cw, wb_ctx, qc, dctx) : 0;
}
inline void cat_wgrads(WgradList& wl, int M, const Lin& l, int cw, const float* dpre, const float* s, const float* ctx) {
  const int sd = l.in - cw;
  wl.push(M, l.out, sd, dpre, s, sd, wl.g(l.w + cw), l.in, wl.g(l.b));
  wl.push(M, l.out, cw, dpre, ctx, cw, wl.g(l.w), l.in, nullptr);
}

inline int noise_or_zero(const float*& noise, float* zero, size_t n, hipStream_t st) {
  if (noise) return 0;
  noise = zero;
  return launch_fill(zero, (int64_t)n, 0.f, st);
}

struct GaussFamily;
enum { CAP_GAUSS_DECODER = 1,
       CAP_HIDDEN = 2,
       CAP_HIDDEN_RAW = 4 };
struct Family {
  int (*desc_check)(const ardae_model_desc* d);
  unsigned (*caps)(const ardae_model_desc& d);
  size_t (*param_floats)(const ardae_model_desc&);
  size_t (*packed_floats)(const ardae_model_desc&);
  size_t (*workspace_floats)(const ardae_model_desc&, int B, int nz, int mode);
  int (*pack)(const ardae_model_desc&, const float* params, float* packed, hipStream_t);
  int (*encode)(const ardae_model_desc&, const float* params, const float* packed, const float* x, const float* noise, int B, int nz,
                float* workspace, size_t wsf, float* z_out, float* hidden_out, hipStream_t, const float* raw0);
  int (*decode)(const ardae_model_desc&, const float* params, const float* packed, const float* z, int R, float* workspace, size_t wsf,
                float* out0, hipStream_t, float* out1);
  int (*vae_forward)(const ardae_model_desc&, const float* params, const float* packed, const float* x, const float* noise, int B, int nz,
                     DevFloat beta, float* workspace, size_t wsf, float* z_out, float* losses, hipStream_t);
  int (*vae_backward)(const ardae_model_desc&, const float* params, const float* packed, const float* x, const float* noise, int B, int nz,
                      DevFloat beta, float dloss, const float* dz_extra, float* workspace, size_t wsf, float* grads, float grads_beta, hipStream_t);
  const GaussFamily* gauss;
  int (*encode_pair)(const ardae_model_desc&, const float* params, const float* packed, const float* x, const float* noise, int B, int nz,
                     float* workspace, size_t wsf, float* z0_out, float* z_out, int phase, hipStream_t);
  int (*vae_backward_decoder)(const ardae_model_desc&, const float* params, const float* packed, const float* x, const float* noise, int B, int nz,
                              DevFloat beta, float dloss, float* workspace, size_t wsf, hipStream_t);
  int (*vae_backward_sampler)(const ardae_model_desc&, const float* params, const float* packed, const float* x, const float* noise, int B, int nz,
                              const float* dz_extra, DevFloat seed_scale, float* workspace, size_t wsf, float* grads, float grads_beta, hipStream_t);
};
inline unsigned no_caps(const ardae_model_desc&) { return 0; }
inline int desc_flags_ok(const ardae_model_desc* d, int allowed) {
  ARDAE_CHECK_ARG((d->flags & ~allowed) == 0,
                  "model: unknown flags %d (ARDAE_MODEL_NO_CENTER / the sampler-head bits / ARDAE_MODEL_CLIPPED: residual-conv kinds 5 / 6 only; "
                  "the log-variance clip codes: kinds 3 / 7 only)", d->flags);
  ARDAE_CHECK_ARG(((d->flags >> ARDAE_MODEL_CLIP_Z0_SHIFT) & 15) <= 10 && ((d->flags >> ARDAE_MODEL_CLIP_Z_SHIFT) & 15) <= 10, "model: unknown log-variance clip code");
  return 0;
}
const Family* family_of(int kind);
inline const Family& family(const ardae_model_desc* d) { return *family_of(d->kind); }

template <class Layout, class Packed> size_t family_param_floats(const ardae_model_desc& d) { return Layout(d).total; }
template <class Layout, class Packed> size_t family_packed_floats(const ardae_model_desc& d) {
  const Layout P(d);
  PackList pl;
  const Packed K(P, pl);
  return pl.total();
}
template <class Layout, class Packed> int family_pack(const ardae_model_desc& d, const float* params, float* packed, hipStream_t st) {
  const Layout P(d);
  PackList pl(params, packed);
  const Packed K(P, pl);
  return pl.launch(st);
}

template <class Layout, class Packed, class Ws> struct Entry {
  const Layout P; const Packed K; Bump ws; Ws W{};
  template <class... CarveArgs> Entry(const ardae_model_desc& d, float* workspace, size_t wsf, CarveArgs... args) : P(d), K(P), ws(workspace, wsf) {
    carve(P, K, ws, args..., W);
  }
};

int launch_mul_dact(const float* x, const float* S, int act, float* y, int64_t n, hipStream_t st);
int launch_nhwc_nchw(const float* in, int B, int HW, int C, float* out, bool to_nhwc, hipStream_t st);

}
```

pytorch-ardae-vae_amd/csrc/ipmodel.h:

```cpp
#pragma once
#include "host_util.h"
#include "mlp.h"

namespace ardae {

struct IpBufs { float *z, *out0, *out1, *dout0, *dout1, *dzq, *dz, *rec_row, *pri_row; };

struct IpEncodeOut { float* z_out; float* hidden_out; const float* raw0; bool std0; };

struct IpTraitsBase {
  static constexpr bool mlp_decoder = false;
  static constexpr bool direct_z = false;
  struct Grads { float* grads; float beta; };
  template <class Entry> static Grads grads_of(Entry&, const float*, const float*, float* grads, float grads_beta) { return {grads, grads_beta}; }
  template <class Layout> static size_t extra_floats(const Layout&, int, int, int) { return 0; }
  template <class Layout> static int rows_ok(const Layout&, int, bool) { return 0; }
  template <class Entry> static int hidden_copy(Entry&, float*, int, hipStream_t) { return 0; }
};

template <class F> size_t ip_workspace_floats(const ardae_model_desc& d, int B, int nz, int mode) {
  const typename F::Layout P(d);
  const typename F::Packed K(P);
  if constexpr (F::mlp_decoder)
    if (mode == 2) return K.dec.decode_floats((size_t)B * nz);
  const int m = mode == 3 ? 0 : mode;
  Bump ws;
  typename F::Ws W{};
  carve(P, K, ws, B, nz, m, W);
  if (m == 1) {
    WgradList wl(nullptr);
    F::wgrads(P, K, W, nullptr, nullptr, B, nz, wl, ws);
  }
  return ws.off + F::extra_floats(P, B, nz, mode);
}

template <class F> int ip_encode(const ardae_model_desc& d, const float* params, const float* packed, const float* x, const float* noise, int B, int nz,
                                 float* workspace, size_t wsf, float* z_out, float* hidden_out, hipStream_t st, const float* raw0) {
  typename F::Entry entry(d, workspace, wsf, B, nz, 0);
  auto& [P, K, ws, W] = entry;
  const size_t nn = F::noise_floats(P, B, nz);
  float* zero = noise ? nullptr : F::zero_noise(entry, nn);
  ARDAE_CHECK_ARG(ws.ok, "model_encode: internal workspace accounting error");
  ARDAE_TRY(F::rows_ok(P, nz, true));
  ARDAE_CHECK_ARG(!hidden_out || nz == 1, "model_encode: the hidden context is defined for nz == 1");
  const IpEncodeOut enc{z_out, hidden_out, raw0, noise == nullptr};
  ARDAE_TRY(noise_or_zero(noise, zero, nn, st));
  ARDAE_TRY(F::sampler_fwd(entry, params, packed, x, noise, B, nz, &enc, st));
  if (z_out && !F::direct_z) ARDAE_TRY(launch_copy(F::bufs(W).z, (size_t)B * nz * d.z_dim, z_out, st));
  if (hidden_out) ARDAE_TRY(F::hidden_copy(entry, hidden_out, B, st));
  return 0;
}

template <class F> int ip_decode(const ardae_model_desc& d, const float* params, const float* packed, const float* z, int R, float* workspace, size_t wsf,
                                 float* out0, hipStream_t st, float*) {
  typename F::Entry entry(d, workspace, wsf, R, 1, 2);
  ARDAE_CHECK_ARG(entry.ws.ok, "model_decode: internal workspace accounting error");
  ARDAE_TRY(F::decoder_fwd(entry, params, packed, z, R, st));
  return launch_copy(F::bufs(entry.W).out0, (size_t)R * d.input_dim, out0, st);
}

template <class F> int ip_vae_forward(const ardae_model_desc& d, const float* params, const float* packed, const float* x, const float* noise, int B, int nz,
                                      DevFloat beta, float* workspace, size_t wsf, float* z_out, float* losses, hipStream_t st) {
  typename F::Entry entry(d, workspace, wsf, B, nz, 1);
  auto& [P, K, ws, W] = entry;
  ARDAE_CHECK_ARG(ws.ok, "model_vae_forward: internal workspace accounting error");
  ARDAE_TRY(F::rows_ok(P, nz, false));
  const IpBufs G = F::bufs(W);
  const int R = B * nz;
  ARDAE_TRY(F::sampler_fwd(entry, params, packed, x, noise, B, nz, nullptr, st));
  ARDAE_TRY(launch_copy(G.z, (size_t)R * d.z_dim, z_out, st));
  ARDAE_TRY(F::decoder_fwd(entry, params, packed, G.z, R, st));
  ARDAE_TRY(launch_vae_loss(G.out1 ? 1 : 0, G.out0, G.out1, x, G.z, R, nz, d.input_dim, d.z_dim, beta, 0, 0.f, nullptr, G.rec_row, G.pri_row, nullptr,
                            nullptr, nullptr, st));
  return launch_vae_loss_finalize(G.rec_row, G.pri_row, R, beta, losses, st);
}

template <class F> int ip_backward(const ardae_model_desc& d, const float* params, const float* packed, const float* x, const float* noise, int B, int nz,
                                   DevFloat beta, float dloss, const float* dz_extra, DevFloat seed_scale, float* workspace, size_t wsf, float* grads,
                                   float grads_beta, int phases, hipStream_t st) {
  typename F::Entry entry(d, workspace, wsf, B, nz, 1);
  ARDAE_CHECK_ARG(entry.ws.ok, "model_vae_backward: internal workspace accounting error");
  typename F::Grads g = F::grads_of(entry, params, packed, grads, grads_beta);
  const IpBufs G = F::bufs(entry.W);
  const int R = B * nz;
  if (phases & 1) {
    ARDAE_TRY(launch_vae_loss(G.out1 ? 1 : 0, G.out0, G.out1, x, G.z, R, nz, d.input_dim, d.z_dim, beta, 1, dloss / (float)R,
                              phases == 3 ? dz_extra : nullptr, G.rec_row, G.pri_row, G.dout0, G.dout1, G.dzq, st));
    ARDAE_TRY(F::decoder_bwd(entry, packed, R, g, st));
  }
  if (!(phases & 2)) return 0;
  if (phases == 2 && dz_extra) ARDAE_TRY(launch_axpy(dz_extra, (int64_t)R * d.z_dim, seed_scale, G.dz, st));
  return F::sampler_bwd(entry, params, packed, x, noise, B, nz, g, st);
}
template <class F> int ip_vae_backward(const ardae_model_desc& d, const float* params, const float* packed, const float* x, const float* noise, int B,
                                       int nz, DevFloat beta, float dloss, const float* dz_extra, float* workspace, size_t wsf, float* grads,
                                       float grads_beta, hipStream_t st) {
  return ip_backward<F>(d, params, packed, x, noise, B, nz, beta, dloss, dz_extra, 1.f, workspace, wsf, grads, grads_beta, 3, st);
}
template <class F> int ip_vae_backward_decoder(const ardae_model_desc& d, const float* params, const float* packed, const float* x, const float* noise,
                                               int B, int nz, DevFloat beta, float dloss, float* workspace, size_t wsf, hipStream_t st) {
  return ip_backward<F>(d, params, packed, x, noise, B, nz, beta, dloss, nullptr, 0.f, workspace, wsf, nullptr, 0.f, 1, st);
}
template <class F> int ip_vae_backward_sampler(const ardae_model_desc& d, const float* params, const float* packed, const float* x, const float* noise,
                                               int B, int nz, const float* dz_extra, DevFloat seed_scale, float* workspace, size_t wsf, float* grads,
                                               float grads_beta, hipStream_t st) {
  return ip_backward<F>(d, params, packed, x, noise, B, nz, 0.f, 0.f, dz_extra, seed_scale, workspace, wsf, grads, grads_beta, 2, st);
}

template <class F> constexpr Family ip_family(int (*pack)(const ardae_model_desc&, const float*, float*, hipStream_t) =
                                                  family_pack<typename F::Layout, typename F::Packed>) {
  Family f{};
  f.desc_check = F::desc_check; f.caps = F::caps;
  f.param_floats = family_param_floats<typename F::Layout, typename F::Packed>;
  f.packed_floats = family_packed_floats<typename F::Layout, typename F::Packed>;
  f.workspace_floats = ip_workspace_floats<F>; f.pack = pack; f.encode = ip_encode<F>;
  if constexpr (F::mlp_decoder) f.decode = mlp_decode<typename F::Layout, typename F::Packed>;
  else f.decode = ip_decode<F>;
  f.vae_forward = ip_vae_forward<F>; f.vae_backward = ip_vae_backward<F>;
  return f;
}
}
```

pytorch-ardae-vae_amd/csrc/model.hip:

```cpp
#include <vector>

#include "ardae_hip.h"
#include "common.h"
#include "auxconvvae.h"
#include "auxmodel.h"
#include "auxvae.h"
#include "convmodel.h"
#include "convvae.h"
#include "resmodel.h"
#include "vaemodel.h"
#include "ipmodel.h"
#include "elementwise.h"
#include "mlp.h"

namespace ardae {
namespace {

struct ModelLayout {
  int kind, D, nd, h, zd, nl, act;
  std::vector<Lin> inp, stack, dec, heads;
  std::vector<bool> stack_noise;
  size_t total = 0;
  explicit ModelLayout(const ardae_model_desc& d)
      : kind(d.kind), D(d.input_dim), nd(d.noise_dim), h(d.h_dim), zd(d.z_dim), nl(d.n_layers), act(d.act) {
    size_t off = 0;
    auto add = [&](std::vector<Lin>& v, int out, int in) { v.push_back(next_lin(off, out, in)); };
    const int n_inp = kind == 0 ? nl + 2 : nl;
    for (int l = 0; l < n_inp; ++l) add(inp, h, l == 0 ? D : h);
    if (kind == 0) {
      add(stack, h, h + nd); stack_noise.push_back(true);
      add(stack, zd, h); stack_noise.push_back(false);
    } else {
      for (int l = 0; l < nl; ++l) { add(stack, h, h + nd); stack_noise.push_back(true); }
      add(stack, zd, h + nd); stack_noise.push_back(true);
    }
    const int n_dec = kind == 0 ? nl + 1 : nl;
    for (int l = 0; l < n_dec; ++l) add(dec, h, l == 0 ? zd : h);
    add(heads, D, h);
    if (kind == 1) add(heads, D, h);
    total = off;
  }
};

struct ModelPacked {
  MlpStack inp;
  std::vector<size_t> sh_f, sh_b, sn_f;
  MlpDecoder dec;
  ModelPacked(const ModelLayout& P, PackList& pl) : inp(P.inp.data(), P.inp.size(), pl) {
    const size_t ns = P.stack.size();
    sh_f.resize(ns); sh_b.resize(ns); sn_f.assign(ns, 0);
    for (size_t i = 0; i < ns; ++i) {
      const Lin& l = P.stack[i];
      pl.pair(l, sh_f[i], sh_b[i], 0, P.h);
      if (P.stack_noise[i]) sn_f[i] = pl.panel(l.w + P.h, l.in, l.out, P.nd, false);
    }
    dec = MlpDecoder(P.dec.data(), P.dec.size(), P.heads.data(), (int)P.heads.size(), pl);
  }
  explicit ModelPacked(const ModelLayout& P, PackList&& sizing = PackList()) : ModelPacked(P, sizing) {}
};

struct ModelWs {
  float* x2;
  std::vector<float*> e;
  float* rb;
  std::vector<float*> t;
  float* z;
  MlpDecoder::Bufs D;
  float *rec_row, *pri_row;
  std::vector<float*> dt, de;
  float* drb;
};

void carve(const ModelLayout& P, const ModelPacked& K, Bump& ws, int B, int nz, int mode, ModelWs& W) {
  const size_t R = (size_t)B * nz, h = P.h;
  W.x2 = ws.take((size_t)B * P.D);
  K.inp.carve(ws, B, W.e);
  W.rb = ws.take((size_t)B * h);
  W.t.assign(P.stack.size(), nullptr);
  for (size_t i = 1; i < P.stack.size(); ++i) W.t[i] = ws.take(R * h);
  W.z = ws.take(R * P.zd);
  if (mode == 0) return;
  K.dec.carve(ws, R, true, W.D);
  W.rec_row = ws.take(R); W.pri_row = ws.take(R);
  W.dt.assign(P.stack.size(), nullptr);
  for (size_t i = 1; i < P.stack.size(); ++i) W.dt[i] = ws.take(R * h);
  K.inp.carve(ws, B, W.de);
  W.drb = ws.take((size_t)B * h);
}
using MlpEntry = Entry<ModelLayout, ModelPacked, ModelWs>;

int encode_trunk(const ModelLayout& P, const ModelPacked& K, const float* params, const float* packed, const float* x, int B,
                 ModelWs& W, hipStream_t st) {
  const int h = P.h;
  const float* x_in = x;
  if (P.kind == 0) {
    ARDAE_TRY(launch_affine(x, (int64_t)B * P.D, 2.f, -1.f, W.x2, st));
    x_in = W.x2;
  }
  ARDAE_TRY(K.inp.fwd(params, packed, P.act, B, x_in, W.e.data(), st));
  return dense_fwd(ACT_NONE, B, h, W.e[P.inp.size()], h, h, packed + K.sh_f[0], params + P.stack[0].b, W.rb, st);
}

int encode_stack(const ModelLayout& P, const ModelPacked& K, const float* params, const float* packed, const float* noise,
                 int B, int nz, const float* rb, const std::vector<float*>& t, float* zdst, bool keep_hidden, hipStream_t st) {
  const int R = B * nz, h = P.h, act = P.act;
  const size_t ns = P.stack.size();
  if (!keep_hidden && ns == 2 && P.stack_noise[0] && !P.stack_noise[1] && P.stack[0].out == h) {
    LinArgs A{}; A.M = R; A.Nout = h; A.act = act; A.nsrc = 1;
    A.rowbias = rb; A.rowbias_ld = h; A.rows_per_group = nz;
    A.src[0].x = noise; A.src[0].ld = P.nd; A.src[0].K = P.nd; A.src[0].wp = packed + K.sn_f[0];
    if (sampler_tail_eligible(A, P.stack[1].out))
      return launch_sampler_tail(A, packed + K.sh_f[1], params + P.stack[1].b, zdst, P.stack[1].out, P.stack[1].out, st);
  }
  for (size_t i = 0; i < ns; ++i) {
    const bool last = i + 1 == ns;
    const int out = P.stack[i].out;
    LinArgs A{}; A.Y = last ? zdst : t[i + 1]; A.ldY = out; A.M = R; A.Nout = out; A.act = last ? ACT_NONE : act;
    int n = 0;
    if (i == 0) {
      A.rowbias = rb; A.rowbias_ld = h; A.rows_per_group = nz;
    } else {
      A.bias = params + P.stack[i].b;
      A.src[n].x = t[i]; A.src[n].ld = h; A.src[n].K = h; A.src[n].wp = packed + K.sh_f[i]; ++n;
    }
    if (P.stack_noise[i]) {
      A.src[n].x = noise; A.src[n].ld = P.nd; A.src[n].K = P.nd; A.src[n].wp = packed + K.sn_f[i]; ++n;
    }
    A.nsrc = n;
    ARDAE_TRY(launch_linear(A, EPI_ACT, st));
  }
  return 0;
}

struct MlpTraits : IpTraitsBase {
  using Layout = ModelLayout; using Packed = ModelPacked; using Ws = ModelWs; using Entry = MlpEntry;
  static constexpr bool mlp_decoder = true;
  static constexpr bool direct_z = true;
  static int desc_check(const ardae_model_desc* d) { return mlp_desc_check(d, 0); }
  static unsigned caps(const ardae_model_desc& d) { return d.kind == 1 ? CAP_GAUSS_DECODER : 0; }
  static IpBufs bufs(const ModelWs& W) { return {W.z, W.D.o[0], W.D.o[1], W.D.dox[0], W.D.dox[1], W.D.dzq, W.D.dz, W.rec_row, W.pri_row}; }
  static void wgrads(const ModelLayout& P, const ModelPacked& K, const ModelWs& W, const float* x, const float* noise, int B, int nz, WgradList& wl, Bump& ws) {
    const int R = B * nz, h = P.h;
    const size_t ns = P.stack.size();
    K.dec.wgrads(wl, R, W.z, W.D);
    for (size_t i = 0; i < ns; ++i) {
      const Lin& L = P.stack[i];
      const float* G = (i == ns - 1) ? W.D.dz : W.dt[i + 1];
      if (i == 0) wl.push(B, L.out, h, W.drb, W.e[P.inp.size()], h, wl.g(L.w), L.in, nullptr);
      else wl.push(R, L.out, h, G, W.t[i], h, wl.g(L.w), L.in, P.stack_noise[i] ? nullptr : wl.g(L.b));
      if (P.stack_noise[i]) wl.push(R, L.out, P.nd, G, noise, P.nd, wl.g(L.w + h), L.in, wl.g(L.b));
    }
    K.inp.wgrads(wl, B, P.kind == 0 ? W.x2 : x, W.e.data(), W.de.data());
    wl.assign(ws, (int)(P.heads.size() + P.dec.size() + 2 * ns + P.inp.size()));
  }
  static size_t extra_floats(const ModelLayout& P, int B, int nz, int mode) {
    if (mode == 3) return (P.stack.size() - 1) * al64((size_t)B * P.h) + al64((size_t)B * P.nd);
    return al64((size_t)B * nz * P.nd);
  }
  static size_t noise_floats(const ModelLayout& P, int B, int nz) { return (size_t)B * nz * P.nd; }
  static float* zero_noise(Entry& e, size_t n) { return e.ws.take(n); }
  static int sampler_fwd(Entry& e, const float* params, const float* packed, const float* x, const float* noise, int B, int nz, const IpEncodeOut* enc,
                         hipStream_t st) {
    ARDAE_TRY(encode_trunk(e.P, e.K, params, packed, x, B, e.W, st));
    return encode_stack(e.P, e.K, params, packed, noise, B, nz, e.W.rb, e.W.t, enc && enc->z_out ? enc->z_out : e.W.z, enc == nullptr, st);
  }
  static int decoder_fwd(Entry& e, const float* params, const float* packed, const float* z, int R, hipStream_t st) {
    return e.K.dec.fwd(params, packed, e.P.act, R, z, e.W.D.hid.data(), e.W.D.o, st);
  }
  static int decoder_bwd(Entry& e, const float* packed, int R, Grads&, hipStream_t st) { return e.K.dec.bwd(packed, e.P.act, R, e.W.D, st); }
  static int sampler_bwd(Entry& e, const float*, const float* packed, const float* x, const float* noise, int B, int nz, Grads& g, hipStream_t st) {
    auto& [P, K, ws, W] = e;
    const int R = B * nz, h = P.h, act = P.act;
    const size_t ns = P.stack.size(), ninp = P.inp.size();
    for (size_t i = ns - 1; i >= 1; --i)
      ARDAE_TRY(dense_bwd(act, R, h, (i == ns - 1) ? W.D.dz : W.dt[i + 1], P.stack[i].out, packed + K.sh_b[i], W.t[i], W.dt[i], st));
    ARDAE_TRY(launch_segment_sum(W.dt[1], h, B, nz, h, 1.0f, W.drb, h, st));
    ARDAE_TRY(dense_bwd(act, B, h, W.drb, h, packed + K.sh_b[0], W.e[ninp], W.de[ninp], st));
    ARDAE_TRY(K.inp.bwd(packed, act, B, W.e.data(), W.de.data(), st));
    WgradList wl(g.grads, g.beta);
    wgrads(P, K, W, x, noise, B, nz, wl, ws);
    ARDAE_CHECK_ARG(ws.ok, "model_vae_backward: internal workspace accounting error");
    return wl.launch(st);
  }
};

int mlp_encode_pair(const ardae_model_desc& d, const float* params, const float* packed, const float* x, const float* noise, int B, int nz,
                    float* workspace, size_t wsf, float* z0_out, float* z_out, int phase, hipStream_t st) {
  MlpEntry entry(d, workspace, wsf, B, nz, 0);
  auto& [P, K, ws, W] = entry;
  std::vector<float*> t0(P.stack.size(), nullptr);
  for (size_t i = 1; i < P.stack.size(); ++i) t0[i] = ws.take((size_t)B * P.h);
  float* zero = ws.take((size_t)B * P.nd);
  ARDAE_CHECK_ARG(ws.ok, "model_encode_pair: internal workspace accounting error");
  if (phase != 2) {
    ARDAE_TRY(launch_fill(zero, (size_t)B * P.nd, 0.f, st));
    ARDAE_TRY(encode_trunk(P, K, params, packed, x, B, W, st));
    ARDAE_TRY(encode_stack(P, K, params, packed, zero, B, 1, W.rb, t0, z0_out, false, st));
  }
  if (phase != 1) ARDAE_TRY(encode_stack(P, K, params, packed, noise, B, nz, W.rb, W.t, z_out, false, st));
  return 0;
}

constexpr Family mlp_family() {
  Family f = ip_family<MlpTraits>();
  f.encode_pair = mlp_encode_pair;
  f.vae_backward_decoder = ip_vae_backward_decoder<MlpTraits>;
  f.vae_backward_sampler = ip_vae_backward_sampler<MlpTraits>;
  return f;
}
const Family MLP_FAMILY = mlp_family();

}

const Family* family_of(int kind) {
  static const Family* const by_kind[20] = {&MLP_FAMILY, &MLP_FAMILY, &CONV_FAMILY, &AUX_FAMILY, &AUXCONV_FAMILY, &RES_FAMILY, &RES_FAMILY, &AUX_FAMILY,
                                            &VAE_FAMILY, &VAE_FAMILY, nullptr, &CONVVAE_FAMILY, &RESVAE_FAMILY, nullptr, &AUXVAE_FAMILY,
                                            &AUXVAE_FAMILY, nullptr, &AUXCONVVAE_FAMILY, nullptr, &AUXRESVAE_FAMILY};
  return kind >= 0 && kind <= 19 ? by_kind[kind] : nullptr;
}

}

using namespace ardae;

static int desc_ok(const ardae_model_desc* d) {
  ARDAE_CHECK_ARG(d != nullptr, "model: desc is NULL");
  ARDAE_CHECK_ARG(family_of(d->kind) != nullptr,
                  "model: kind must be 0 (MNISTIPVAE), 1 (ToyIPVAE concat), 2 (ConvIPVAE), 3 (MNISTAuxIPVAE), 4 (MNISTConvAuxIPVAE), 5 (ResConvIPVAE), "
                  "6 (MNISTResConvAuxIPVAE), 7 (ToyAuxIPVAE), 8 (MNISTVAE), 9 (ToyVAE), 11 (MNISTConvVAE) or 12 (MNISTResConvVAE), or 14 (MNISTAuxVAE) or 15 (ToyAuxVAE), or 17 (MNISTConvAuxVAE), or 19 (MNISTResConvAuxVAE)");
  return family(d).desc_check(d);
}

extern "C" {

size_t ardae_model_param_floats(const ardae_model_desc* d) { return desc_ok(d) ? 0 : family(d).param_floats(*d); }
size_t ardae_model_packed_floats(const ardae_model_desc* d) { return desc_ok(d) ? 0 : family(d).packed_floats(*d); }
size_t ardae_model_workspace_floats(const ardae_model_desc* d, int B, int nz, int mode) {
  if (desc_ok(d) || B <= 0 || nz <= 0) return 0;
  return family(d).workspace_floats(*d, B, nz, mode);
}

int ardae_model_pack(const ardae_model_desc* d, const float* params, float* packed, void* stream) {
  ARDAE_TRY(desc_ok(d));
  ARDAE_CHECK_ARG(params && packed, "model_pack: null pointer");
  return family(d).pack(*d, params, packed, (hipStream_t)stream);
}

static int model_common(const ardae_model_desc* d, const float* params, const float* packed, const float* x, int B, int nz,
                        float* workspace, size_t wsf, int mode) {
  ARDAE_TRY(desc_ok(d));
  ARDAE_CHECK_ARG(params && packed && x && workspace, "model: null pointer argument");
  ARDAE_CHECK_ARG(B > 0 && nz > 0 && (int64_t)B * nz < (int64_t)1 << 30, "model: bad batch (B=%d nz=%d)", B, nz);
  const size_t need = ardae_model_workspace_floats(d, B, nz, mode);
  ARDAE_CHECK_ARG(wsf >= need, "model: workspace too small (%zu < %zu floats)", wsf, need);
  return 0;
}

int ardae_model_encode(const ardae_model_desc* d, const float* params, const float* packed, const float* x, const float* noise,
                       int B, int nz, float* workspace, size_t workspace_floats_, float* z_out, void* stream) {
  ARDAE_TRY(model_common(d, params, packed, x, B, nz, workspace, workspace_floats_, 0));
  ARDAE_CHECK_ARG(z_out, "model_encode: z_out is NULL");
  return family(d).encode(*d, params, packed, x, noise, B, nz, workspace, workspace_floats_, z_out, nullptr, (hipStream_t)stream, nullptr);
}

int ardae_model_encode_pair(const ardae_model_desc* d, const float* params, const float* packed, const float* x, const float* noise,
                            int B, int nz, float* workspace, size_t workspace_floats_, float* z0_out, float* z_out, int phase,
                            void* stream) {
  ARDAE_TRY(desc_ok(d));
  ARDAE_CHECK_ARG(phase >= 0 && phase <= 2, "model_encode_pair: phase must be 0 (all), 1 (trunk + z0) or 2 (N-row stack)");
  ARDAE_CHECK_ARG(params && packed && x && (noise || phase == 1) && workspace && z0_out && z_out, "model_encode_pair: null pointer argument");
  ARDAE_CHECK_ARG(B > 0 && nz > 0 && (int64_t)B * nz < (int64_t)1 << 30, "model_encode_pair: bad batch (B=%d nz=%d)", B, nz);
  ARDAE_CHECK_ARG(workspace_floats_ >= ardae_model_workspace_floats(d, B, nz, 3), "model_encode_pair: workspace too small");
  if (family(d).encode_pair)
    return family(d).encode_pair(*d, params, packed, x, noise, B, nz, workspace, workspace_floats_, z0_out, z_out, phase, (hipStream_t)stream);
  if (phase != 2) ARDAE_TRY(ardae_model_encode(d, params, packed, x, nullptr, B, 1, workspace, workspace_floats_, z0_out, stream));
  if (phase == 1) return 0;
  return ardae_model_encode(d, params, packed, x, noise, B, nz, workspace, workspace_floats_, z_out, stream);
}

int ardae_model_encode_hidden_raw(const ardae_model_desc* d, const float* params, const float* packed, const float* x, const float* raw0, int B,
                                  float* workspace, size_t workspace_floats_, float* z0_out, float* hidden_out, void* stream) {
  ARDAE_TRY(model_common(d, params, packed, x, B, 1, workspace, workspace_floats_, 0));
  ARDAE_CHECK_ARG(family(d).caps(*d) & CAP_HIDDEN_RAW, "model_encode_hidden_raw: the clipped aux-resconv class only (kind 6 + ARDAE_MODEL_CLIPPED)");
  ARDAE_CHECK_ARG(z0_out || hidden_out, "model_encode_hidden_raw: nothing to return");
  return family(d).encode(*d, params, packed, x, nullptr, B, 1, workspace, workspace_floats_, z0_out, hidden_out, (hipStream_t)stream, raw0);
}
int ardae_model_encode_hidden(const ardae_model_desc* d, const float* params, const float* packed, const float* x, int B, float* workspace,
                              size_t workspace_floats_, float* z0_out, float* hidden_out, void* stream) {
  ARDAE_TRY(model_common(d, params, packed, x, B, 1, workspace, workspace_floats_, 0));
  ARDAE_CHECK_ARG(family(d).caps(*d) & CAP_HIDDEN, "model_encode_hidden: the hidden1a context exists for the aux models only (kinds 3, 4, 6, 7)");
  ARDAE_CHECK_ARG(hidden_out, "model_encode_hidden: hidden_out is NULL");
  return family(d).encode(*d, params, packed, x, nullptr, B, 1, workspace, workspace_floats_, z0_out, hidden_out, (hipStream_t)stream, nullptr);
}

int ardae_model_decode(const ardae_model_desc* d, const float* params, const float* packed, const float* z, int R, float* workspace,
                       size_t workspace_floats_, float* out0, float* out1, void* stream) {
  ARDAE_TRY(desc_ok(d));
  ARDAE_CHECK_ARG(params && packed && z && workspace && out0 && R > 0, "model_decode: bad arguments");
  ARDAE_CHECK_ARG(!(family(d).caps(*d) & CAP_GAUSS_DECODER) || out1, "model_decode: the Gaussian decoder needs out1 (logvar)");
  ARDAE_CHECK_ARG(workspace_floats_ >= family(d).workspace_floats(*d, R, 1, 2), "model_decode: workspace too small");
  return family(d).decode(*d, params, packed, z, R, workspace, workspace_floats_, out0, (hipStream_t)stream, out1);
}

int ardae_model_loss_rows(const ardae_model_desc* d, const float* out0, const float* out1, const float* x, const float* z, int rows,
                          int nz, float* recon_row, float* prior_row, void* stream) {
  ARDAE_TRY(desc_ok(d));
  return launch_vae_loss(family(d).caps(*d) & CAP_GAUSS_DECODER ? 1 : 0, out0, out1, x, z, rows, nz, d->input_dim, d->z_dim, 1.f, 0, 0.f, nullptr, recon_row, prior_row, nullptr,
                         nullptr, nullptr, (hipStream_t)stream);
}

static int vae_forward_entry(const ardae_model_desc* d, const float* params, const float* packed, const float* x, const float* noise, int B,
                             int nz, DevFloat beta, float* workspace, size_t workspace_floats_, float* z_out, float* losses, void* stream) {
  ARDAE_TRY(model_common(d, params, packed, x, B, nz, workspace, workspace_floats_, 1));
  ARDAE_CHECK_ARG(noise && z_out && losses, "model_vae_forward: null pointer argument");
  return family(d).vae_forward(*d, params, packed, x, noise, B, nz, beta, workspace, workspace_floats_, z_out, losses, (hipStream_t)stream);
}

static int vae_backward_entry(const ardae_model_desc* d, const float* params, const float* packed, const float* x, const float* noise, int B,
                              int nz, DevFloat beta, float dloss, const float* dz_extra, float* workspace, size_t workspace_floats_,
                              float* grads, float grads_beta, void* stream) {
  ARDAE_TRY(model_common(d, params, packed, x, B, nz, workspace, workspace_floats_, 1));
  ARDAE_CHECK_ARG(noise && grads, "model_vae_backward: null pointer argument");
  return family(d).vae_backward(*d, params, packed, x, noise, B, nz, beta, dloss, dz_extra, workspace, workspace_floats_, grads, grads_beta,
                                (hipStream_t)stream);
}

static int vae_backward_decoder_entry(const ardae_model_desc* d, const float* params, const float* packed, const float* x, const float* noise,
                                      int B, int nz, DevFloat beta, float dloss, float* workspace, size_t workspace_floats_, void* stream) {
  ARDAE_TRY(model_common(d, params, packed, x, B, nz, workspace, workspace_floats_, 1));
  ARDAE_CHECK_ARG(noise, "model_vae_backward_decoder: null pointer argument");
  ARDAE_CHECK_ARG(family(d).vae_backward_decoder, "model_vae_backward_decoder: the conv model and the aux model have no split backward (use ardae_model_vae_backward)");
  return family(d).vae_backward_decoder(*d, params, packed, x, noise, B, nz, beta, dloss, workspace, workspace_floats_, (hipStream_t)stream);
}

static int vae_backward_sampler_entry(const ardae_model_desc* d, const float* params, const float* packed, const float* x, const float* noise,
                                      int B, int nz, const float* dz_extra, DevFloat seed_scale, float* workspace, size_t workspace_floats_,
                                      float* grads, float grads_beta, void* stream) {
  ARDAE_TRY(model_common(d, params, packed, x, B, nz, workspace, workspace_floats_, 1));
  ARDAE_CHECK_ARG(noise && grads, "model_vae_backward_sampler: null pointer argument");
  ARDAE_CHECK_ARG(family(d).vae_backward_sampler, "model_vae_backward_sampler: the conv model and the aux model have no split backward (use ardae_model_vae_backward)");
  return family(d).vae_backward_sampler(*d, params, packed, x, noise, B, nz, dz_extra, seed_scale, workspace, workspace_floats_, grads, grads_beta,
                                        (hipStream_t)stream);
}

int ardae_model_vae_forward(const ardae_model_desc* d, const float* params, const float* packed, const float* x, const float* noise,
                            int B, int nz, float beta, float* workspace, size_t workspace_floats_, float* z_out, float* losses,
                            void* stream) {
  return vae_forward_entry(d, params, packed, x, noise, B, nz, beta, workspace, workspace_floats_, z_out, losses, stream);
}
int ardae_model_vae_forward_dev(const ardae_model_desc* d, const float* params, const float* packed, const float* x, const float* noise,
                                int B, int nz, const void* state, float* workspace, size_t workspace_floats_, float* z_out, float* losses,
                                void* stream) {
  ARDAE_CHECK_ARG(state, "model_vae_forward_dev: state is NULL");
  return vae_forward_entry(d, params, packed, x, noise, B, nz, train_state_beta(state), workspace, workspace_floats_, z_out, losses, stream);
}

int ardae_model_vae_backward(const ardae_model_desc* d, const float* params, const float* packed, const float* x, const float* noise,
                             int B, int nz, float beta, float dloss, const float* dz_extra, float* workspace,
                             size_t workspace_floats_, float* grads, float grads_beta, void* stream) {
  return vae_backward_entry(d, params, packed, x, noise, B, nz, beta, dloss, dz_extra, workspace, workspace_floats_, grads, grads_beta, stream);
}
int ardae_model_vae_backward_dev(const ardae_model_desc* d, const float* params, const float* packed, const float* x, const float* noise,
                                 int B, int nz, const void* state, float dloss, const float* dz_extra, float* workspace,
                                 size_t workspace_floats_, float* grads, float grads_beta, void* stream) {
  ARDAE_CHECK_ARG(state, "model_vae_backward_dev: state is NULL");
  return vae_backward_entry(d, params, packed, x, noise, B, nz, train_state_beta(state), dloss, dz_extra, workspace, workspace_floats_, grads,
                            grads_beta, stream);
}

int ardae_model_vae_backward_decoder(const ardae_model_desc* d, const float* params, const float* packed, const float* x,
                                     const float* noise, int B, int nz, float beta, float dloss, float* workspace,
                                     size_t workspace_floats_, void* stream) {
  return vae_backward_decoder_entry(d, params, packed, x, noise, B, nz, beta, dloss, workspace, workspace_floats_, stream);
}
int ardae_model_vae_backward_decoder_dev(const ardae_model_desc* d, const float* params, const float* packed, const float* x,
                                         const float* noise, int B, int nz, const void* state, float dloss, float* workspace,
                                         size_t workspace_floats_, void* stream) {
  ARDAE_CHECK_ARG(state, "model_vae_backward_decoder_dev: state is NULL");
  return vae_backward_decoder_entry(d, params, packed, x, noise, B, nz, train_state_beta(state), dloss, workspace, workspace_floats_, stream);
}

int ardae_model_vae_backward_sampler(const ardae_model_desc* d, const float* params, const float* packed, const float* x,
                                     const float* noise, int B, int nz, const float* dz_extra, float seed_scale, float* workspace,
                                     size_t workspace_floats_, float* grads, float grads_beta, void* stream) {
  return vae_backward_sampler_entry(d, params, packed, x, noise, B, nz, dz_extra, seed_scale, workspace, workspace_floats_, grads, grads_beta,
                                    stream);
}
int ardae_model_vae_backward_sampler_dev(const ardae_model_desc* d, const float* params, const float* packed, const float* x,
                                         const float* noise, int B, int nz, const float* dz_extra, const void* state, float* workspace,
                                         size_t workspace_floats_, float* grads, float grads_beta, void* stream) {
  ARDAE_CHECK_ARG(state, "model_vae_backward_sampler_dev: state is NULL");
  return vae_backward_sampler_entry(d, params, packed, x, noise, B, nz, dz_extra, train_state_seed_scale(state), workspace, workspace_floats_,
                                    grads, grads_beta, stream);
}

}
```

pytorch-ardae-vae_amd/engine.py:

```python
import contextlib
from dataclasses import dataclass

import torch

from . import _lib as L
from . import dist
from . import rng
from .iwae import IwaeEvaluator
from .diagnostics import PosteriorDiagnostics
from .engine_common import RNG_STRIDE, CaptureLadder, _FlatOpt, bump_versions, capture_linear, check_batch, check_tensor, rebuild_step_state
from .score_engine import ArdaeCondScoreEngine
from .optim import WEIGHT_AVG_KINDS, unwrap_state_dict, wrap_state_dict


@dataclass
class TrainConfig:
    delta: float = 0.1
    std_scale: float = 1e4
    nz_cdae: int = 256
    nstd_cdae: int = 1
    nz_model: int = 1
    num_cdae_updates: int = 1
    beta: float = 1.0
    beta_init: float = None
    beta_annealing: int = None
    m_lr: float = 1e-4
    m_beta1: float = 0.5
    d_lr: float = 1e-4
    d_momentum: float = 0.5
    m_optimizer: str = "adam"
    d_optimizer: str = "rmsprop"
    d_beta1: float = 0.5
    cdae_ctx_type: str = "lt0"
    ctx_data_center: bool = True
    m_weight_avg: str = "none"
    m_weight_avg_start: int = 1000
    m_weight_avg_decay: float = 0.998
    m_weight_avg_freq: int = 1

    def __post_init__(self):
        if self.m_weight_avg != "none" and self.m_weight_avg not in WEIGHT_AVG_KINDS:
            raise NotImplementedError(f"unknown weight averaging: {self.m_weight_avg}")
        if int(self.m_weight_avg_freq) != 1:
            raise NotImplementedError(f"m_weight_avg_freq {self.m_weight_avg_freq}: only 1 is implemented (ivae_ardae.py:561,563 always pass 1)")
        if int(self.m_weight_avg_start) < 0 or not 0.0 <= float(self.m_weight_avg_decay) <= 1.0:
            raise ValueError(f"m_weight_avg_start must be >= 0 and m_weight_avg_decay in [0, 1] (got {self.m_weight_avg_start}, "
                             f"{self.m_weight_avg_decay})")
        if self.beta_annealing is not None and int(self.beta_annealing) != self.beta_annealing:
            raise ValueError(f"beta_annealing must be a whole number of steps or None (got {self.beta_annealing!r})")
        if self.beta_init is None and self.beta_annealing is not None and self.beta_annealing >= 1:
            raise ValueError(f"beta_annealing={self.beta_annealing} needs beta_init (--beta-init)")

    def beta_schedule(self):
        if self.beta_annealing is None or self.beta_annealing < 1:
            return None
        return float(self.beta_init), float(self.beta), int(self.beta_annealing)


def annealing_func(val_init, val_fin, val_annealing, step):
    if val_annealing is None:
        return float(val_fin)
    return float(val_init + (val_fin - val_init) / float(val_annealing) * float(min(val_annealing, step)))


class ArdaeEngine:

    RNG_STRIDE = RNG_STRIDE

    def __init__(self, model, cdae, cfg: TrainConfig, batch_size, process_group=None, graph=True, force_dp=False, dp_comm="auto"):
        model._require_gpu()
        cdae._require_gpu()
        if int(cdae._desc.kind) not in (0, 1, 16, 17):
            raise TypeError(f"ArdaeEngine trains a conditional AR-DAE (net.MLPGradCARDAE / net.MLPResCARDAE), not a {type(cdae).__name__}: its step "
                            "block has no slot for a noise level beside beta (a plain conditional DAE runs in ArdaeCondScoreEngine)")
        self.model, self.cdae, self.cfg = model, cdae, cfg
        self.B = int(batch_size)
        self.dev = model._flat.device
        self.pg = process_group
        self.world = dist.world_size(process_group)
        self.rank = dist.rank(process_group)
        self.dp = self.world > 1 or bool(force_dp)
        if isinstance(dp_comm, str):
            if dp_comm != "auto":
                raise ValueError(f"dp_comm must be a dist.DpComm, None or 'auto', got {dp_comm!r}")
            dp_comm = None
            if self.dp and torch.distributed.is_available() and torch.distributed.is_initialized() and \
                    "nccl" in str(torch.distributed.get_backend(process_group)):
                dp_comm = dist.DpComm(process_group)
        self.comm = dp_comm if self.dp else None
        if self.comm is not None and (self.comm.world, self.comm.rank) != (self.world, self.rank):
            raise ValueError(f"dp_comm is rank {self.comm.rank} of {self.comm.world}, the process group says {self.rank} of {self.world}")
        md, cd = model._desc, cdae._desc
        B, nzc, nzm = self.B, cfg.nz_cdae, cfg.nz_model
        N = B * nzc
        z, nd = model.z_dim, model._noise_width
        if cfg.cdae_ctx_type not in ("lt0", "hidden1a", "data"):
            raise NotImplementedError(f"cdae_ctx_type {cfg.cdae_ctx_type!r}")
        if cfg.cdae_ctx_type == "hidden1a" and not model.hidden_dim:
            raise NotImplementedError("hidden1a is the aux models' context (ivae_ardae.py:572-580)")
        self.hidden_ctx = cfg.cdae_ctx_type == "hidden1a"
        self.data_ctx = cfg.cdae_ctx_type == "data"
        self.clipped = bool(getattr(model, "_clipped", False))
        if self.clipped and not self.hidden_ctx:
            raise NotImplementedError("MNISTResConvAuxIPVAEClipped is built with --cdae-ctx-type hidden1a (the aux models' context, ivae_ardae.py:572-580)")
        ctx_dim = model.hidden_dim if self.hidden_ctx else int(model.input_dim) if self.data_ctx else z
        if int(cdae.context_dim) != ctx_dim:
            raise ValueError(f"cdae.context_dim = {cdae.context_dim}, but the {cfg.cdae_ctx_type} context has {ctx_dim} columns")
        f = lambda *s: torch.empty(*s, device=self.dev, dtype=torch.float32)
        S = nzc * int(cfg.nstd_cdae)
        ws_floats = max(L.query("ardae_cdae_workspace_floats", cd, B, S, 1),
                        L.query("ardae_model_workspace_floats", md, B, nzc, 3))
        self.ws = f(ws_floats)
        self.ws_vae = f(L.query("ardae_model_workspace_floats", md, B, nzm, 1))
        self.ws_small = f(max(L.query("ardae_cdae_workspace_floats", cd, B, nzm, 0),
                              L.query("ardae_model_workspace_floats", md, B, 1, 0)))
        self.ws_small_v = f(L.query("ardae_model_workspace_floats", md, B, 1, 0))
        self.z0, self.latent = f(B, z), f(N, z)
        self.noise_s, self.xi, self.eps = f(model._noise_numel(B, nzc)), f(B * S), f(B * S, z)
        self.xbar, self.sigma, self.std_b = f(B * S, z), f(B * S), f(B)
        self.noise_v, self.zv, self.z0v, self.u, self.g = f(model._noise_numel(B, nzm)), f(B * nzm, z), f(B, z), f(B * nzm, z), f(B * nzm, z)
        self.sigma0 = torch.zeros(B * nzm, device=self.dev)
        if self.clipped:
            self.raw_c, self.raw_v = f(2, B, model.noise_dim), f(2, B, model.noise_dim)
        self.ctx_c, self.ctx_v = (f(B, ctx_dim), f(B, ctx_dim)) if (self.hidden_ctx or self.data_ctx) else (self.z0, self.z0v)
        if self.data_ctx:
            self._ctx_half = torch.full((B, ctx_dim), 0.5 if cfg.ctx_data_center else 0.0, device=self.dev)
        self.loss_c, self.losses_m = f(1), f(3)
        self.grads_c = torch.zeros_like(cdae._flat)
        self.grads_m = torch.zeros_like(model._flat)
        self.n_c = cdae._flat.numel() - (1 if cdae._kind == "grad" else 0)
        self.step_count = 0
        self.state = torch.zeros(4, dtype=torch.int64, device=self.dev)
        self.sched = cfg.beta_schedule()
        train = None if self.sched is None else self.sched + (float(cfg.std_scale), B * nzm)
        self.opt_m = _FlatOpt(cfg.m_optimizer, model._flat, model._flat.numel(), cfg.m_lr, cfg.m_beta1, cfg.d_momentum, state=self.state, train=train)
        self.opt_c = _FlatOpt(cfg.d_optimizer, cdae._flat, self.n_c, cfg.d_lr, cfg.d_beta1, cfg.d_momentum)
        self.wavg = None if cfg.m_weight_avg == "none" else cfg.m_weight_avg
        self.avg = torch.zeros_like(model._flat) if self.wavg else None
        self._avg_origin = int(cfg.m_weight_avg_start) + 1
        self._avg_swap = None
        self._iwae = None
        self._diag = None
        if graph not in (True, False, "auto"):
            raise ValueError(f"graph must be True, False or 'auto', got {graph!r}")
        self.use_graph = bool(graph) and L.debug_knob("ARDAE_GRAPH", "1") != "0"
        self.graph_strict = graph is True
        self._graph, self._graph_key, self._xc, self._xv = None, None, None, None
        self._in_step, self._draws, self._warmed = False, 0, False
        self._last_beta, self._beta_stable = None, 0
        self.overlap = L.debug_knob("ARDAE_OVERLAP", "1") != "0"
        self.split_backward = int(md.kind) < 2 and L.debug_knob("ARDAE_SPLIT_BACKWARD", "1") != "0"
        self._side = torch.cuda.Stream(device=self.dev) if self.overlap else None
        self.fused_draws = L.debug_knob("ARDAE_FUSED_DRAW", "1") != "0"
        self.fused_first_layer = (L.debug_knob("ARDAE_FUSED_A1", "1") != "0"
                                  and (int(cd.kind) < 2 or ArdaeCondScoreEngine.FUSED_FIRST_NOENC_DEFAULT))
        self._cap_stream = torch.cuda.Stream(device=self.dev)
        self._stamps = None
        self._log = None
        self.opt_m.advance(self.RNG_STRIDE)
        self.repack()

    def attach_log(self, log):
        self._log, self._graph = log, None

    def _beta_arg(self, beta):
        if self.sched is None:
            return float(self.cfg.beta if beta is None else beta)
        if beta is not None:
            raise ValueError(f"beta={beta!r}: this engine computes beta on the device (TrainConfig(beta_init={self.cfg.beta_init}, "
                             f"beta_annealing={self.cfg.beta_annealing})); a second source is refused")
        return None

    def _refresh_train_state(self):
        if self.sched is not None:
            self.state[0] -= self.RNG_STRIDE
            self.state[1] -= 1
            self.opt_m.advance(self.RNG_STRIDE)

    def repack(self):
        self.model._packed = None
        self.cdae._packed = None
        self.pk_m = self.model._packed_weights()
        self.pk_c = self.cdae._packed_weights()

    def _pack_model(self):
        L.call("ardae_model_pack", self.model._desc, self.model._flat, self.pk_m)

    def _pack_cdae(self):
        L.call("ardae_cdae_pack", self.cdae._desc, self.cdae._flat, self.pk_c)

    def _check_batch(self, x, what):
        check_batch(x, what, self.dev, self.B, self.model.input_dim, "images")

    def _encode(self, x, noise, nz, out, ws):
        L.call("ardae_model_encode", self.model._desc, self.model._flat, self.pk_m, x, noise, self.B, nz, ws, ws.numel(), out)

    def _hidden(self, x, z0_out, out, ws, raws=None):
        if self.clipped:
            for k, (zo, ho) in enumerate(((None, out), (z0_out, None))):
                L.call("ardae_model_encode_hidden_raw", self.model._desc, self.model._flat, self.pk_m, x, raws[k], self.B, ws, ws.numel(), zo, ho)
            return
        L.call("ardae_model_encode_hidden", self.model._desc, self.model._flat, self.pk_m, x, self.B, ws, ws.numel(), z0_out, out)

    def _plan(self, xs, x_vae, noise, beta):
        cfg = self.cfg
        vae_draw = self.RNG_STRIDE - 1
        nlist = list(noise) if isinstance(noise, (list, tuple)) else [noise] * len(xs)
        nv = nlist[-1]["vae"] if nlist[-1] else self.noise_v
        side = "side" if self.overlap else "main"
        segs = []
        vae_fwd = ("run", "vae_fwd", side, (), lambda: self.vae_forward_part(x_vae, nlist[-1], beta, draw=vae_draw))
        if self.overlap:
            segs.append(vae_fwd)
        for i, xc in enumerate(xs):
            segs.append(("run", f"cdae_grads{i}", "main", (), lambda xc=xc, i=i: self._cdae_grads(xc, nlist[i], 3 * i)))
            if self.dp:
                segs.append(self._allreduce_seg(f"allreduce_c{i}", self.grads_c[:self.n_c]))
            segs.append(("run", f"cdae_update{i}", "main", (), self._cdae_update))
        if not self.overlap:
            segs.append(vae_fwd)
        segs.append(("run", "vae_bwd", "main", ("vae_fwd",) if self.overlap else (), lambda: self._vae_backward_grads(x_vae, nv, beta)))
        if self.dp:
            segs.append(self._allreduce_seg("allreduce_m", self.grads_m))

        def model_update():
            self._model_update()
            if self._log is not None:
                self._log.record(self._beta_arg(beta))
            self.opt_m.advance(self.RNG_STRIDE)
        segs.append(("run", "model_update", "main", (), model_update))
        if self._stamps is not None:
            def wrap(name, fn):
                def run():
                    self._stamp(name + " >")
                    fn()
                    self._stamp(name + " <")
                return run
            segs = [s if s[0] != "run" else (s[0], s[1], s[2], s[3], wrap(s[1], s[4])) for s in segs]
        return segs

    def _allreduce_seg(self, name, buf):
        if self.comm is not None:
            return ("run", name, "main", (), lambda: self.comm.allreduce_mean_(buf))
        return ("allreduce", buf)

    def _allreduce(self, buf):
        if self.comm is not None:
            self.comm.allreduce_mean_(buf)
        else:
            dist.allreduce_mean_(buf, self.pg, force=True)

    @staticmethod
    def _units(segs):
        needed = {d for s in segs if s[0] == "run" for d in s[3]}
        units, where, open_unit = [], {}, {}
        for s in segs:
            if s[0] == "allreduce":
                units.append(["allreduce", s[1]])
                open_unit.clear()
                continue
            _, name, stream, deps, fn = s
            waits = sorted({where[d] for d in deps if units[where[d]][1] != stream})
            k = open_unit.get(stream)
            if k is None or waits:
                units.append(["run", stream, waits, [], False])
                k = len(units) - 1
            units[k][3].append(fn)
            where[name] = k
            open_unit[stream] = None if name in needed else k
            if name in needed:
                units[k][4] = True
        return units

    def _run_units(self, units, graphs=None, capture=False):
        main = torch.cuda.current_stream()
        streams = {"main": main, "side": self._side}
        events, out = {}, []
        for k, u in enumerate(units):
            if u[0] == "allreduce":
                dist.allreduce_mean_(u[1], self.pg, force=self.dp)
                out.append(None)
                continue
            _, sname, waits, fns, record = u
            st = streams[sname]
            for w in waits:
                st.wait_event(events[w])
            if sname != "main" and not waits:
                st.wait_stream(main)
            if capture:
                out.append(capture_linear(fns, self._cap_stream))
                with torch.cuda.stream(st):
                    out[-1].replay()
            elif graphs is not None:
                if st is main:
                    graphs[k].replay()
                else:
                    with torch.cuda.stream(st):
                        graphs[k].replay()
            elif st is main:
                for fn in fns:
                    fn()
            else:
                with torch.cuda.stream(st):
                    for fn in fns:
                        fn()
            if record:
                events[k] = torch.cuda.Event()
                events[k].record(st)
        return out

    def _normal(self, out, draw=None):
        first = self.rank * out.numel()
        if not self._in_step:
            return rng.normal(None, self.dev, out=out, first_element=first)
        if draw is None:
            k = self._draws
            self._draws += 1
        else:
            k = draw
        if k >= self.RNG_STRIDE:
            raise RuntimeError("more Philox draws in one step than RNG_STRIDE reserves")
        L.call("ardae_philox_normal_at", out, out.numel(), rng.get_state()["seed"], k, self.state, first)
        return out

    def cdae_phase(self, x, noise=None, apply_update=True):
        self._require_trained("cdae_phase()")
        self._cdae_grads(x, noise)
        if self.dp:
            self._allreduce(self.grads_c[:self.n_c])
        if apply_update:
            self._cdae_update()

    def _cdae_grads(self, x, noise=None, draw0=None):
        self._check_batch(x, "cdae_phase")
        cfg = self.cfg
        B, nz, z = self.B, cfg.nz_cdae, self.model.z_dim
        nstd = int(cfg.nstd_cdae)
        fused = (not noise) and self._in_step and draw0 is not None and self.fused_draws and bool(L.query("ardae_latent_perturb_draw_ok", nz, nstd, z))
        if noise:
            ns, xi, eps = noise["sampler"], noise["sigma"].reshape(-1), noise["eps"]
        else:
            d = (None, None, None) if draw0 is None else (draw0, draw0 + 1, draw0 + 2)
            ns = self._normal(self.noise_s, d[0])
            xi, eps = (self.xi, self.eps) if fused else (self._normal(self.xi, d[1]), self._normal(self.eps, d[2]))
        if self.hidden_ctx:
            raws = None
            if self.clipped:
                if noise:
                    raws = torch.stack([noise["ctx_raw"].reshape(B, -1), noise["z0_raw"].reshape(B, -1)]).float().contiguous()
                else:
                    raws = self._normal(self.raw_c, None if draw0 is None else 9 + draw0 // 3)
            self._hidden(x, self.z0, self.ctx_c, self.ws_small, raws)
            self._encode(x, ns, nz, self.latent, self.ws)
        else:
            L.call("ardae_model_encode_pair", self.model._desc, self.model._flat, self.pk_m, x, ns, B, nz, self.ws, self.ws.numel(), self.z0,
                   self.latent, 0)
        if self.data_ctx:
            self._data_context(x, self.ctx_c)
        self._stamp("  sampler done")
        if fused and self.fused_first_layer and bool(L.query("ardae_cdae_perturb_fused_ok", self.cdae._desc, nz, nstd)):
            L.call("ardae_cdae_perturb_loss_grads", self.cdae._desc, self.cdae._flat, self.pk_c, self.latent, self.z0, self.ctx_c, B, nz,
                   cfg.std_scale, cfg.delta, rng.get_state()["seed"], d[1], d[2], self.state, self.rank * B * nz, self.xbar, self.sigma, eps,
                   self.std_b, self.ws, self.ws.numel(), self.loss_c, self.grads_c)
            return
        if fused:
            L.call("ardae_latent_perturb_draw", self.latent, self.z0, B, nz, z, cfg.std_scale, cfg.delta, rng.get_state()["seed"], d[1], d[2],
                   self.state, self.rank * B * nz, self.xbar, self.sigma, eps, self.std_b)
        else:
            L.call("ardae_latent_perturb_nstd", self.latent, self.z0, xi, eps, B, nz, nstd, z, cfg.std_scale, cfg.delta, self.xbar, self.sigma,
                   self.std_b)
        L.call("ardae_cdae_loss_grads", self.cdae._desc, self.cdae._flat, self.pk_c, self.xbar, self.sigma, eps, self.ctx_c, B, nz * nstd,
               self.ws, self.ws.numel(), self.loss_c, self.grads_c, None)

    def _cdae_update(self):
        if self._in_step and self.opt_c.adam:
            self.opt_c.advance()
        self.opt_c.apply(self.grads_c, self._in_step)
        if not self._in_step:
            self.opt_c.steps += 1
        self._pack_cdae()

    def _data_context(self, x, out):
        D = int(self.model.input_dim)
        L.call("ardae_center_scale", x, self._ctx_half, self.B, 1, D, 2.0 if self.cfg.ctx_data_center else 1.0, out)

    def vae_forward_part(self, x, noise=None, beta=None, draw=None):
        self._require_trained("vae_forward_part()")
        self._check_batch(x, "vae_forward_part")
        cfg = self.cfg
        beta = self._beta_arg(beta)
        dev = "_dev" if beta is None else ""
        B, nz, md = self.B, cfg.nz_model, self.model._desc
        nv = noise["vae"] if noise else self._normal(self.noise_v, draw)
        L.call("ardae_model_vae_forward" + dev, md, self.model._flat, self.pk_m, x, nv, B, nz, self.state if dev else beta, self.ws_vae,
               self.ws_vae.numel(), self.zv, self.losses_m)
        if self.hidden_ctx:
            raws = None
            if self.clipped:
                if noise:
                    raws = torch.stack([noise["vctx_raw"].reshape(B, -1), noise["vz0_raw"].reshape(B, -1)]).float().contiguous()
                else:
                    raws = self._normal(self.raw_v, None if draw is None else 12)
            self._hidden(x, self.z0v, self.ctx_v, self.ws_small_v, raws)
        else:
            self._encode(x, None, 1, self.z0v, self.ws_small_v)
        if self.data_ctx:
            self._data_context(x, self.ctx_v)
        L.call("ardae_center_scale", self.zv, self.z0v, B, nz, self.model.z_dim, cfg.std_scale, self.u)
        if self.split_backward:
            L.call("ardae_model_vae_backward_decoder" + dev, md, self.model._flat, self.pk_m, x, nv, B, nz, self.state if dev else beta, 1.0,
                   self.ws_vae, self.ws_vae.numel())
        return nv

    def vae_backward_part(self, x, nv, beta=None, apply_update=True):
        self._require_trained("vae_backward_part()")
        self._vae_backward_grads(x, nv, beta)
        if self.dp:
            self._allreduce(self.grads_m)
        if apply_update:
            self._model_update()

    def _vae_backward_grads(self, x, nv, beta=None):
        self._check_batch(x, "vae_backward_part")
        cfg = self.cfg
        beta = self._beta_arg(beta)
        dev = "_dev" if beta is None else ""
        B, nz, md = self.B, cfg.nz_model, self.model._desc
        L.call("ardae_cdae_score", self.cdae._desc, self.cdae._flat, self.pk_c, self.u, self.sigma0, self.ctx_v, B, nz, self.ws_small,
               self.ws_small.numel(), self.g)
        seed_scale = self.state if dev else float(dist.entropy_seed_scale(cfg.std_scale, beta, B, nz))
        if self.split_backward:
            L.call("ardae_model_vae_backward_sampler" + dev, md, self.model._flat, self.pk_m, x, nv, B, nz, self.g, seed_scale, self.ws_vae,
                   self.ws_vae.numel(), self.grads_m, 0.0)
        else:
            if dev:
                L.call("ardae_seed_scale_dev", self.g, self.g.numel(), self.state)
            else:
                self.g.mul_(seed_scale)
            L.call("ardae_model_vae_backward" + dev, md, self.model._flat, self.pk_m, x, nv, B, nz, self.state if dev else beta, 1.0, self.g,
                   self.ws_vae, self.ws_vae.numel(), self.grads_m, 0.0)

    def _model_update(self):
        self.opt_m.apply(self.grads_m, self._in_step)
        if self.avg is not None:
            L.call("ardae_weight_avg", self.avg, self.model._flat, self.avg.numel(), WEIGHT_AVG_KINDS[self.wavg], float(self.cfg.m_weight_avg_decay),
                   self._avg_origin, self.state, 0)
        if not self._in_step:
            self.step_count += 1
            self.opt_m.steps = self.step_count
            self.opt_m.advance(self.RNG_STRIDE)
        self._pack_model()

    def vae_phase(self, x, noise=None, beta=None, apply_update=True):
        nv = self.vae_forward_part(x, noise, beta)
        self.vae_backward_part(x, nv, beta, apply_update)

    def _step_body(self, xs, x_vae, noise, beta, capture=False):
        self._in_step, self._draws = True, 0
        try:
            units = self._units(self._plan(xs, x_vae, noise, beta))
            graphs = self._run_units(units, capture=capture)
            return (units, graphs) if capture else None
        finally:
            self._in_step = False

    def _replay(self):
        units, graphs = self._graph
        self._run_units(units, graphs=graphs)

    def enable_stamps(self, on=True):
        self._stamps = {"buf": torch.zeros(256, dtype=torch.int64, device=self.dev), "names": []} if on else None
        self._graph = None

    def _stamp(self, name):
        st = self._stamps
        if st is None:
            return
        if name not in st["names"]:
            st["names"].append(name)
        L.call("ardae_debug_stamp", st["buf"], st["names"].index(name))

    def read_stamps(self):
        st = self._stamps
        torch.cuda.synchronize()
        v = st["buf"].cpu().tolist()
        t0 = min(v[i] for i in range(len(st["names"])))
        return sorted(((n, (v[i] - t0) / 100.0) for i, n in enumerate(st["names"])), key=lambda kv: kv[1])

    def plan_summary(self):
        if self._graph is None:
            return None
        return ["allreduce" if u[0] == "allreduce" else f"graph:{u[1]}" for u in self._graph[0]]

    def step(self, x_cdae, x_vae, noise=None, beta=None):
        self._require_trained("step()")
        many = isinstance(x_cdae, (list, tuple))
        xs = list(x_cdae) if many else [x_cdae] * self.cfg.num_cdae_updates
        for x in xs:
            self._check_batch(x, "step(x_cdae)")
        self._check_batch(x_vae, "step(x_vae)")
        if 3 * len(xs) >= self.RNG_STRIDE:
            raise ValueError("at most %d cDAE updates per step (Philox offsets reserved per step)" % ((self.RNG_STRIDE - 1) // 3))
        if self.clipped and len(xs) > 3:
            raise ValueError("at most 3 cDAE updates per step with MNISTResConvAuxIPVAEClipped (its std = 0 draws use Philox offsets 9 .. 12)")
        b = self._beta_arg(beta)
        if self.use_graph and noise is None:
            self._static_batches(len(xs))
            for buf, x in zip(self._xc, xs):
                if x is not buf:
                    buf.copy_(x.view(self.B, -1))
            if x_vae is not self._xv:
                self._xv.copy_(x_vae.view(self.B, -1))
            key = (b, tuple(tuple(x.shape) for x in self._xc), tuple(self._xv.shape))
            self._beta_stable = self._beta_stable + 1 if b == self._last_beta else 0
            self._last_beta = b
            if self._graph is not None and self._graph_key == key:
                self._replay()
            elif self._warmed and b is not None and self._beta_stable < 2:
                self._step_body(self._xc, self._xv, None, b)
            elif not self._warmed:
                self._step_body(self._xc, self._xv, None, b)
                self._warmed = True
            else:
                try:
                    g = self._step_body(self._xc, self._xv, None, b, capture=True)
                except Exception as exc:
                    if self.graph_strict:
                        raise RuntimeError(f"ArdaeEngine(graph=True): HIP graph capture failed ({exc}); pass graph='auto' to fall back to "
                                           "eager launches, or graph=False") from exc
                    self.use_graph = False
                    self._graph = None
                    import warnings
                    warnings.warn(f"ArdaeEngine: HIP graph capture failed ({exc}); continuing with eager launches")
                    self._step_body(self._xc, self._xv, None, b)
                else:
                    self._graph, self._graph_key = g, key
            self._count_step(len(xs))
            return
        self._step_body(xs, x_vae, noise, b)
        self._count_step(len(xs))

    def input_buffers(self, n_cdae=None):
        self._static_batches(self.cfg.num_cdae_updates if n_cdae is None else int(n_cdae))
        return list(self._xc), self._xv

    def _static_batches(self, n):
        if self._xc is None or len(self._xc) != n:
            flat = lambda: torch.empty(self.B, self.model.input_dim, device=self.dev, dtype=torch.float32)
            self._xc, self._xv, self._graph = [flat() for _ in range(n)], flat(), None

    def _count_step(self, n_cdae_updates):
        self.step_count += 1
        self.opt_m.steps = self.step_count
        self.opt_c.steps += n_cdae_updates

    def model_checkpoint(self):
        self._require_trained("model_checkpoint()")
        opt = self.opt_m.state_dict(self.model)
        if self.avg is not None:
            n_avg = self._n_avg()
            opt["param_groups"][0].update(n_avg=n_avg, step_counter=self.step_count)
            bufs = dict(enumerate(v.clone() for v in self.model.param_views(self.avg))) if n_avg else {}
            opt = wrap_state_dict(opt, self.wavg, bufs)
        return {"state_dict": {k: t.clone() for k, t in self.model.state_dict().items()},
                "optimizer": opt,
                "engine": {"state_version": 2, "step_count": self.step_count, "cdae_steps": self.opt_c.steps, "rng_seed": rng.get_state()["seed"],
                           "rng_host_offset": rng.get_state()["offset"], "step_state": self.state.cpu().clone()}}

    def cdae_checkpoint(self):
        return {"state_dict": {k: t.clone() for k, t in self.cdae.state_dict().items()}, "optimizer": self.opt_c.state_dict(self.cdae)}

    def load_checkpoints(self, model_ckpt, cdae_ckpt):
        self._require_trained("load_checkpoints()")
        m_opt, w_kind, w_bufs = unwrap_state_dict(model_ckpt["optimizer"])
        if self.avg is not None and w_kind is not None and w_kind != self.wavg:
            raise ValueError(f"model checkpoint: holds a {w_kind!r} average, but this engine was built with m_weight_avg={self.wavg!r}")
        self.model.load_state_dict(model_ckpt["state_dict"])
        self.cdae.load_state_dict(cdae_ckpt["state_dict"])
        eng = model_ckpt.get("engine")
        m_steps = self.opt_m.load_state_dict(self.model, m_opt, "model checkpoint")
        c_steps = self.opt_c.load_state_dict(self.cdae, cdae_ckpt["optimizer"], "cdae checkpoint")
        self.step_count = m_steps if (m_steps or eng is None) else int(eng["step_count"])
        self.opt_m.steps = self.step_count
        self.opt_c.steps = c_steps if (c_steps or eng is None) else int(eng.get("cdae_steps", 0))
        if eng is not None:
            rng.manual_seed(eng["rng_seed"], eng.get("rng_host_offset", rng.get_state()["offset"]))
            self.state.copy_(eng["step_state"].to(self.dev))
            if int(eng.get("state_version", 1)) < 2:
                self.opt_m.advance(self.RNG_STRIDE)
        else:
            rebuild_step_state(self.state, self.step_count, self.RNG_STRIDE, lambda: self.opt_m.advance(self.RNG_STRIDE))
        self._refresh_train_state()
        self.opt_c.state.zero_()
        self.opt_c.state[1] = self.opt_c.steps
        if self.avg is not None:
            self._load_average(m_opt, w_kind, w_bufs)
        self._graph = None
        if self._log is not None:
            self._log.resync()
        self.repack()

    def _n_avg(self):
        return max(0, self.step_count - self._avg_origin + 1)

# ... 79 lines not shown
```

pytorch-ardae-vae_amd/engine_common.py:

```python
import torch

from . import _lib as L

RNG_STRIDE = 16


def check_tensor(t, what, dev, shape=None, numel=None):
    if not torch.is_tensor(t):
        why = f"got a {type(t).__name__}"
    elif t.dtype != torch.float32:
        why = f"got {t.dtype}"
    elif t.numel() != numel if shape is None else t.dim() != len(shape) or any(w not in (None, g) for w, g in zip(shape, t.shape)):
        why = f"got shape {list(t.shape)}"
    elif not t.is_contiguous():
        why = f"got strides {tuple(t.stride())}; call .contiguous()"
    elif not t.is_cuda or t.device != dev:
        why = f"expected a tensor on {dev}, got one on {t.device}"
    else:
        return
    size = f"{numel} values" if shape is None else f"shape {list(shape)}"
    raise ValueError(f"{what} must be a contiguous float32 tensor of {size} on {dev}: {why}")


def check_batch(x, what, dev, B, width, rows="samples"):
    if not torch.is_tensor(x):
        raise TypeError(f"{what}: expected a tensor, got {type(x).__name__}")
    if x.dim() < 2 or x.size(0) != B or x.numel() != B * width:
        raise ValueError(f"{what}: expected {B} {rows} of {width} values (the engine was built with batch_size={B}; use drop_last or pad the "
                         f"last batch), got shape {tuple(x.shape)}")
    check_tensor(x, what, dev, numel=B * width)


def bump_versions(module):
    for p in module.parameters():
        torch.autograd.graph.increment_version(p)


def rebuild_step_state(block, n, stride, advance):
    block.zero_()
    block[0], block[1] = stride * n, n
    advance()


def capture_linear(fns, stream):
    g = torch.cuda.CUDAGraph()
    with torch.cuda.graph(g, stream=stream):
        for fn in fns:
            fn()
    return g


class CaptureLadder:

    def __init__(self, dev, graph):
        if graph not in (True, False):
            raise ValueError(f"graph must be True or False, got {graph!r}")
        self.on = bool(graph) and L.debug_knob("ARDAE_GRAPH", "1") != "0"
        self.stream = torch.cuda.Stream(device=dev)
        self.reset()

    def reset(self):
        self.graph, self.calls = None, 0

    def run(self, body, eager=False):
        if eager or not self.on or (self.graph is None and self.calls < 2):
            body()
        else:
            g = self.graph or capture_linear([body], self.stream)
            g.replay()
            self.graph = g
        self.calls += 1


class _FlatOpt:
    KINDS = ("sgd", "adam", "amsgrad", "rmsprop", "adam_torch")

    def __init__(self, kind, flat, n, lr, beta1, momentum, state=None, train=None, dae=None):
        if kind not in self.KINDS:
            raise NotImplementedError(f"unknown optimizer: {kind}")
        self.kind, self.flat, self.n, self.lr, self.beta1, self.momentum = kind, flat, int(n), float(lr), float(beta1), float(momentum)
        z = lambda: torch.zeros_like(flat)
        self.a = None if kind == "sgd" else z()
        self.b = None if kind == "sgd" else z()
        self.c = z() if kind == "amsgrad" else None
        self.steps, self.train, self.dae = 0, train, dae
        self.state = state if state is not None else torch.zeros(4, dtype=torch.int64, device=flat.device)

    @property
    def adam(self):
        return self.kind in ("adam", "amsgrad", "adam_torch")

    def advance(self, rng_inc=0):
        if self.train is not None:
            L.call("ardae_train_state_advance", self.state, rng_inc, self.lr, self.beta1, 0.999, *self.train)
        elif self.dae is not None:
            L.call("ardae_dae_state_advance", self.state, rng_inc, self.lr, self.beta1, 0.999, *self.dae)
        else:
            L.call("ardae_step_state_advance", self.state, rng_inc, self.lr, self.beta1, 0.999)

    def apply(self, grads, in_step):
        p, g = self.flat, grads
        if self.kind == "sgd":
            L.call("ardae_sgd_step", p, g, self.n, self.lr)
        elif self.kind == "rmsprop":
            L.call("ardae_rmsprop_step", p, g, self.a, self.b, self.n, self.lr, 0.99, 1e-8, self.momentum)
        elif self.kind == "adam_torch":
            if not in_step:
                raise NotImplementedError("adam_torch takes t and its bias corrections from the device block: it runs inside an engine's step")
            L.call("ardae_adam_torch_step_dev", p, g, self.a, self.b, self.n, self.beta1, 0.999, 1e-8, self.state)
        elif in_step:
            L.call("ardae_adam_ref_step_dev", p, g, self.a, self.b, self.c, self.n, self.beta1, 0.999, 1e-8, self.state)
        else:
            L.call("ardae_adam_ref_step", p, g, self.a, self.b, self.c, self.n, self.lr, self.beta1, 0.999, 1e-8, self.steps + 1)

    def state_names(self):
        return {"sgd": (), "adam": ("exp_avg", "exp_avg_sq"), "adam_torch": ("exp_avg", "exp_avg_sq"), "amsgrad": ("exp_avg", "exp_avg_sq", "max_exp_avg_sq"),
                "rmsprop": ("square_avg", "momentum_buffer")}[self.kind]

    def buffers(self):
        return [t for t in (self.a, self.b, self.c) if t is not None]

    def param_group(self, nparams):
        if self.kind == "sgd":
            g = {"lr": self.lr, "momentum": 0, "dampening": 0, "weight_decay": 0, "nesterov": False}
        elif self.adam:
            g = {"lr": self.lr, "betas": (self.beta1, 0.999), "eps": 1e-8, "weight_decay": 0, "amsgrad": self.kind == "amsgrad"}
        else:
            g = {"lr": self.lr, "momentum": self.momentum, "alpha": 0.99, "eps": 1e-8, "centered": False, "weight_decay": 0}
        g["params"] = list(range(nparams))
        return g

    @staticmethod
    def _kind_of_group(group):
        if "betas" in group:
            return "amsgrad" if group.get("amsgrad") else "adam"
        return "rmsprop" if "alpha" in group else "sgd"

    def state_dict(self, module):
        names, state = self.state_names(), {}
        if self.steps and names:
            views = [module.param_views(t, grads_only=True) for t in self.buffers()]
            for i, first in enumerate(views[0]):
                if first is not None:
                    state[i] = dict({"step": self.steps}, **{nm: v[i].clone() for nm, v in zip(names, views)})
        return {"state": state, "param_groups": [self.param_group(len(list(module.named_parameters())))]}

    def load_state_dict(self, module, sd, what):
        state, groups = sd["state"], sd.get("param_groups")
        if groups and self._kind_of_group(groups[0]) != ("adam" if self.kind == "adam_torch" else self.kind):
            raise ValueError(f"{what}: written by optimiser {self._kind_of_group(groups[0])!r}, but this engine was built with {self.kind!r} for that network")
        for t in self.buffers():
            t.zero_()
        steps = {int(st["step"]) for st in state.values()}
        if len(steps) > 1:
            raise ValueError(f"the fused engine keeps one step count per network ({what}: {sorted(steps)})")
        names = self.state_names()
        if state and not all(nm in next(iter(state.values())) for nm in names[:1]):
            raise ValueError(f"{what}: the checkpoint's optimiser state does not belong to {self.kind!r}")
        with torch.no_grad():
            for nm, buf in zip(names, self.buffers()):
                for i, t in enumerate(module.param_views(buf, grads_only=True)):
                    if t is not None and i in state and state[i].get(nm) is not None:
                        t.copy_(state[i][nm])
        return steps.pop() if steps else 0
```

Baseline: 219.4.

## Fuse optimizer step with weight repacking into a single kernel

Adds RMSprop and Adam update kernels that also write each updated parameter into its packed (tiled/transposed) layout, using a per-call table of layout entries that is filtered per block in shared memory. The engine calls these fused variants by default for both the CDAE and the model, and skips the separate pack launches. This is meant to save the pack kernels' extra launches and their re-read of the parameters. In exchange, each element does extra index arithmetic and scattered writes to the packed buffer, and the host rebuilds the table on every call.

```diff
diff --git a/include/ardae_hip.h b/include/ardae_hip.h
--- a/include/ardae_hip.h
+++ b/include/ardae_hip.h
@@ -127,6 +127,11 @@
 size_t ardae_cdae_packed_floats(const ardae_cdae_desc* d);
 size_t ardae_cdae_workspace_floats(const ardae_cdae_desc* d, int B, int S, int need_grads);
 int ardae_cdae_pack(const ardae_cdae_desc* d, const float* params, float* packed, void* stream);
+int ardae_cdae_rmsprop_repack_step(const ardae_cdae_desc* d, float* params, const float* g, float* square_avg, float* momentum_buffer,
+                                   int64_t n, double lr, double alpha, double eps, double momentum, float* packed, void* stream);
+int ardae_cdae_adam_ref_repack_step_dev(const ardae_cdae_desc* d, float* params, const float* g, float* exp_avg, float* exp_avg_sq,
+                                        float* max_exp_avg_sq, int64_t n, double beta1, double beta2, double eps, const void* state,
+                                        float* packed, void* stream);
 int ardae_cdae_loss_grads(const ardae_cdae_desc* d, const float* params, const float* packed, const float* xbar,
                           const float* sigma, const float* eps, const float* ctx, int B, int S, float* workspace,
                           size_t workspace_floats, float* loss, float* grads, float* score_out, void* stream);
@@ -211,6 +216,12 @@
 size_t ardae_model_packed_floats(const ardae_model_desc* d);
 size_t ardae_model_workspace_floats(const ardae_model_desc* d, int B, int nz, int mode);
 int ardae_model_pack(const ardae_model_desc* d, const float* params, float* packed, void* stream);
+int ardae_model_update_repack_ok(const ardae_model_desc* d);
+int ardae_model_rmsprop_repack_step(const ardae_model_desc* d, float* params, const float* g, float* square_avg, float* momentum_buffer,
+                                    int64_t n, double lr, double alpha, double eps, double momentum, float* packed, void* stream);
+int ardae_model_adam_ref_repack_step_dev(const ardae_model_desc* d, float* params, const float* g, float* exp_avg, float* exp_avg_sq,
+                                         float* max_exp_avg_sq, int64_t n, double beta1, double beta2, double eps, const void* state,
+                                         float* packed, void* stream);
 int ardae_model_encode(const ardae_model_desc* d, const float* params, const float* packed, const float* x,
                        const float* noise, int B, int nz, float* workspace, size_t workspace_floats, float* z_out,
                        void* stream);
diff --git a/pytorch-ardae-vae_amd/csrc/cdae.hip b/pytorch-ardae-vae_amd/csrc/cdae.hip
--- a/pytorch-ardae-vae_amd/csrc/cdae.hip
+++ b/pytorch-ardae-vae_amd/csrc/cdae.hip
@@ -1,59 +1,13 @@
 #include <vector>
 
 #include "ardae_hip.h"
+#include "cdae_layout.h"
 #include "common.h"
 #include "elementwise.h"
 #include "host_util.h"
 
 namespace ardae {
 namespace {
-
-bool cond_kind(int kind) { return kind < 2 || kind == 10 || kind == 11 || kind == 13 || kind == 16 || kind == 17; }
-bool input_encoder_kind(int kind) { return kind < 2 || kind == 10 || kind == 11; }
-bool sigma_column_kind(int kind) { return kind < 4 || kind == 16 || kind == 17; }
-
-struct CdaeLayout {
-  int kind, z, c, h, L, act;
-  bool cond, enc_inp, grad, has_sigma;
-  std::vector<Lin> ctx, inp, neg;
-  size_t total = 0;
-  int k1() const { return enc_inp ? h : z; }
-  int sigma_col() const { return cond ? k1() + h : z; }
-
-  explicit CdaeLayout(const ardae_cdae_desc& d)
-      : kind(d.kind), z(d.input_dim), c(d.context_dim), h(d.h_dim), L(d.n_layers), act(d.act), cond(cond_kind(d.kind)), enc_inp(input_encoder_kind(d.kind)), grad(d.kind % 2 == 0), has_sigma(sigma_column_kind(d.kind)) {
-    size_t off = 0;
-    auto add = [&](std::vector<Lin>& v, int out, int in) { v.push_back(next_lin(off, out, in)); };
-    if (cond)
-      for (int l = 0; l < L; ++l) add(ctx, h, l == 0 ? c : h);
-    if (enc_inp)
-      for (int l = 0; l < L; ++l) add(inp, h, l == 0 ? z : h);
-    for (int l = 0; l < L; ++l) add(neg, h, l == 0 ? sigma_col() + (has_sigma ? 1 : 0) : h);
-    add(neg, grad ? 1 : z, h);
-    total = off;
-  }
-};
-
-struct PackedLayout {
-  std::vector<size_t> ctx_f, ctx_b, inp_f, inp_b, neg_f, neg_b;
-  size_t w1_f, w1_b, w1c_f, w1c_b, w1s;
-  size_t fc_f, fc_b;
-  PackedLayout(const CdaeLayout& P, PackList& pl) {
-    const size_t L = P.L;
-    for (auto* v : {&ctx_f, &ctx_b, &inp_f, &inp_b, &neg_f, &neg_b}) v->assign(L, 0);
-    if (P.cond)
-      for (size_t l = 0; l < L; ++l) { pl.pair(P.ctx[l], ctx_f[l], ctx_b[l]); if (P.enc_inp) pl.pair(P.inp[l], inp_f[l], inp_b[l]); }
-    const Lin& W1 = P.neg[0];
-    pl.pair(W1, w1_f, w1_b, 0, P.k1());
-    w1c_f = w1c_b = 0;
-    if (P.cond) pl.pair(W1, w1c_f, w1c_b, P.k1(), P.h);
-    w1s = P.has_sigma ? pl.take(P.h) : 0;
-    for (size_t l = 1; l < L; ++l) pl.pair(P.neg[l], neg_f[l], neg_b[l]);
-    fc_f = fc_b = 0;
-    if (!P.grad) pl.pair(P.neg[L], fc_f, fc_b);
-  }
-  explicit PackedLayout(const CdaeLayout& P, PackList&& sizing = PackList()) : PackedLayout(P, sizing) {}
-};
 
 int desc_ok(const ardae_cdae_desc* d) {
   ARDAE_CHECK_ARG(d != nullptr, "cdae: desc is NULL");
@@ -154,8 +108,16 @@
 int cdae_pack_impl(const CdaeLayout& P, const float* params, float* packed, hipStream_t st) {
   PackList pl(params, packed);
   const PackedLayout K(P, pl);
-  if (P.has_sigma) ARDAE_TRY(launch_gather_strided(params + P.neg[0].w + P.sigma_col(), P.neg[0].in, P.h, packed + K.w1s, st));
   return pl.launch(st);
+}
+
+int cdae_repack_table(const ardae_cdae_desc* d, const float* params, float* packed, RepackTable& tb, size_t* packed_n) {
+  ARDAE_TRY(desc_ok(d));
+  ARDAE_CHECK_ARG(params && packed, "cdae update_repack: null pointer");
+  PackList pl(params, packed);
+  const PackedLayout K(CdaeLayout(*d), pl);
+  *packed_n = pl.total();
+  return pl.repack_table(tb);
 }
 
 LinArgs lin_args(int act, int M, int Nout, const float* x, int ldx, int K, const float* wp, LinArgs a) {
@@ -383,6 +345,23 @@
   ARDAE_CHECK_ARG(params && packed, "cdae_pack: null pointer");
   return cdae_pack_impl(CdaeLayout(*d), params, packed, (hipStream_t)stream);
 }
+int ardae_cdae_rmsprop_repack_step(const ardae_cdae_desc* d, float* params, const float* g, float* square_avg, float* momentum_buffer, int64_t n,
+                                   double lr, double alpha, double eps, double momentum, float* packed, void* stream) {
+  RepackTable tb;
+  size_t packed_n = 0;
+  ARDAE_TRY(cdae_repack_table(d, params, packed, tb, &packed_n));
+  ARDAE_CHECK_ARG(n > 0 && (size_t)n <= CdaeLayout(*d).total, "cdae_rmsprop_repack_step: n = %lld floats, the network has %zu", (long long)n, CdaeLayout(*d).total);
+  return launch_rmsprop_repack(params, g, square_avg, momentum_buffer, n, lr, alpha, eps, momentum, tb, packed, packed_n, (hipStream_t)stream);
+}
+int ardae_cdae_adam_ref_repack_step_dev(const ardae_cdae_desc* d, float* params, const float* g, float* exp_avg, float* exp_avg_sq,
+                                        float* max_exp_avg_sq, int64_t n, double beta1, double beta2, double eps, const void* state, float* packed,
+                                        void* stream) {
+  RepackTable tb;
+  size_t packed_n = 0;
+  ARDAE_TRY(cdae_repack_table(d, params, packed, tb, &packed_n));
+  ARDAE_CHECK_ARG(n > 0 && (size_t)n <= CdaeLayout(*d).total, "cdae_adam_ref_repack_step_dev: n = %lld floats, the network has %zu", (long long)n, CdaeLayout(*d).total);
+  return launch_adam_ref_repack_dev(params, g, exp_avg, exp_avg_sq, max_exp_avg_sq, n, beta1, beta2, eps, state, tb, packed, packed_n, (hipStream_t)stream);
+}
 int ardae_cdae_loss_grads(const ardae_cdae_desc* d, const float* params, const float* packed, const float* xbar,
                           const float* sigma, const float* eps, const float* ctx, int B, int S, float* workspace,
                           size_t workspace_floats, float* loss, float* grads, float* score_out, void* stream) {
diff --git a/pytorch-ardae-vae_amd/csrc/cdae_layout.h b/pytorch-ardae-vae_amd/csrc/cdae_layout.h
--- /dev/null
+++ b/pytorch-ardae-vae_amd/csrc/cdae_layout.h
@@ -0,0 +1,56 @@
+#pragma once
+#include <vector>
+
+#include "ardae_hip.h"
+#include "host_util.h"
+
+namespace ardae {
+
+inline bool cond_kind(int kind) { return kind < 2 || kind == 10 || kind == 11 || kind == 13 || kind == 16 || kind == 17; }
+inline bool input_encoder_kind(int kind) { return kind < 2 || kind == 10 || kind == 11; }
+inline bool sigma_column_kind(int kind) { return kind < 4 || kind == 16 || kind == 17; }
+
+struct CdaeLayout {
+  int kind, z, c, h, L, act;
+  bool cond, enc_inp, grad, has_sigma;
+  std::vector<Lin> ctx, inp, neg;
+  size_t total = 0;
+  int k1() const { return enc_inp ? h : z; }
+  int sigma_col() const { return cond ? k1() + h : z; }
+
+  explicit CdaeLayout(const ardae_cdae_desc& d)
+      : kind(d.kind), z(d.input_dim), c(d.context_dim), h(d.h_dim), L(d.n_layers), act(d.act), cond(cond_kind(d.kind)), enc_inp(input_encoder_kind(d.kind)), grad(d.kind % 2 == 0), has_sigma(sigma_column_kind(d.kind)) {
+    size_t off = 0;
+    auto add = [&](std::vector<Lin>& v, int out, int in) { v.push_back(next_lin(off, out, in)); };
+    if (cond)
+      for (int l = 0; l < L; ++l) add(ctx, h, l == 0 ? c : h);
+    if (enc_inp)
+      for (int l = 0; l < L; ++l) add(inp, h, l == 0 ? z : h);
+    for (int l = 0; l < L; ++l) add(neg, h, l == 0 ? sigma_col() + (has_sigma ? 1 : 0) : h);
+    add(neg, grad ? 1 : z, h);
+    total = off;
+  }
+};
+
+struct PackedLayout {
+  std::vector<size_t> ctx_f, ctx_b, inp_f, inp_b, neg_f, neg_b;
+  size_t w1_f, w1_b, w1c_f, w1c_b, w1s;
+  size_t fc_f, fc_b;
+  PackedLayout(const CdaeLayout& P, PackList& pl) {
+    const size_t L = P.L;
+    for (auto* v : {&ctx_f, &ctx_b, &inp_f, &inp_b, &neg_f, &neg_b}) v->assign(L, 0);
+    if (P.cond)
+      for (size_t l = 0; l < L; ++l) { pl.pair(P.ctx[l], ctx_f[l], ctx_b[l]); if (P.enc_inp) pl.pair(P.inp[l], inp_f[l], inp_b[l]); }
+    const Lin& W1 = P.neg[0];
+    pl.pair(W1, w1_f, w1_b, 0, P.k1());
+    w1c_f = w1c_b = 0;
+    if (P.cond) pl.pair(W1, w1c_f, w1c_b, P.k1(), P.h);
+    w1s = P.has_sigma ? pl.column(W1.w + P.sigma_col(), W1.in, P.h) : 0;
+    for (size_t l = 1; l < L; ++l) pl.pair(P.neg[l], neg_f[l], neg_b[l]);
+    fc_f = fc_b = 0;
+    if (!P.grad) pl.pair(P.neg[L], fc_f, fc_b);
+  }
+  explicit PackedLayout(const CdaeLayout& P, PackList&& sizing = PackList()) : PackedLayout(P, sizing) {}
+};
+
+}
diff --git a/pytorch-ardae-vae_amd/csrc/elementwise.h b/pytorch-ardae-vae_amd/csrc/elementwise.h
--- a/pytorch-ardae-vae_amd/csrc/elementwise.h
+++ b/pytorch-ardae-vae_amd/csrc/elementwise.h
@@ -51,6 +51,25 @@
 int launch_rmsprop(float* p, const float* g, float* sq, float* buf, int64_t n, double lr, double alpha, double eps,
                    double momentum, hipStream_t st);
 
+struct RepackEntry { uint32_t first, span, ldw, rows, cols, mode; uint64_t out; };
+constexpr int REPACK_MAX = 64;
+struct RepackTable { int n; RepackEntry e[REPACK_MAX]; };
+__host__ __device__ inline int64_t repack_offset(const RepackEntry& E, uint32_t i) {
+  const uint32_t d = i - E.first;
+  if (d > E.span) return -1;
+  const uint32_t r = d / E.ldw, c = d - r * E.ldw;
+  if (c >= E.cols) return -1;
+  if (E.mode == 2) return (int64_t)(E.out + r);
+  const uint32_t nn = E.mode ? c : r, kk = E.mode ? r : c, K = E.mode ? E.rows : E.cols;
+  const uint32_t kchunks = (K + 7) >> 3;
+  const uint64_t blk = (uint64_t)(nn >> 5) * kchunks + (kk >> 3);
+  return (int64_t)(E.out + ((blk * 64 + (nn & 31) + 32 * ((kk >> 2) & 1)) << 2) + (kk & 3));
+}
+int launch_rmsprop_repack(float* p, const float* g, float* sq, float* buf, int64_t n, double lr, double alpha, double eps, double momentum,
+                          const RepackTable& table, float* packed, size_t packed_n, hipStream_t st);
+int launch_adam_ref_repack_dev(float* p, const float* g, float* m, float* v, float* vmax, int64_t n, double beta1, double beta2, double eps,
+                               const void* state, const RepackTable& table, float* packed, size_t packed_n, hipStream_t st);
+
 int launch_axpy(const float* x, int64_t n, DevFloat alpha, float* y, hipStream_t st);
 int launch_scale(float* y, int64_t n, DevFloat alpha, hipStream_t st);
 int launch_fill(float* y, int64_t n, float v, hipStream_t st);
diff --git a/pytorch-ardae-vae_amd/csrc/elementwise.hip b/pytorch-ardae-vae_amd/csrc/elementwise.hip
--- a/pytorch-ardae-vae_amd/csrc/elementwise.hip
+++ b/pytorch-ardae-vae_amd/csrc/elementwise.hip
@@ -353,6 +353,35 @@
   if (i < n) dst[i] = src[(size_t)i * stride];
 }
 
+__device__ __forceinline__ float adam_ref1(const float* __restrict__ p, const float* __restrict__ g, float* __restrict__ m, float* __restrict__ v,
+                                           float* __restrict__ vmax, int64_t i, float beta1, float beta2, float eps, float step_size, float sqrt_bc2) {
+  const float gi = g[i];
+  const float mi = m[i] * beta1 + (1.f - beta1) * gi;
+  float vi = v[i] * beta2 + (1.f - beta2) * gi * gi;
+  m[i] = mi;
+  v[i] = vi;
+  if (vmax) {
+    vi = fmaxf(vmax[i], vi);
+    vmax[i] = vi;
+  }
+  const float denom = (sqrtf(vi) + eps) / sqrt_bc2;
+  return p[i] - step_size * (mi / denom);
+}
+
+__device__ __forceinline__ float rmsprop1(const float* __restrict__ p, const float* __restrict__ g, float* __restrict__ sq, float* __restrict__ buf,
+                                          int64_t i, float lr, float alpha, float eps, float momentum) {
+  const float gi = g[i];
+  const float s = sq[i] * alpha + (1.f - alpha) * gi * gi;
+  sq[i] = s;
+  const float avg = sqrtf(s) + eps;
+  if (momentum > 0.f) {
+    const float bi = buf[i] * momentum + gi / avg;
+    buf[i] = bi;
+    return p[i] - lr * bi;
+  }
+  return p[i] - lr * (gi / avg);
+}
+
 __global__ void adam_ref_kernel(float* __restrict__ p, const float* __restrict__ g, float* __restrict__ m, float* __restrict__ v,
                                 float* __restrict__ vmax, int64_t n, float beta1, float beta2, float eps, float step_size,
                                 float sqrt_bc2, const StepState* state) {
@@ -360,35 +389,63 @@
     step_size = state->adam_step_size;
     sqrt_bc2 = state->adam_sqrt_bc2;
   }
-  for (int64_t i = (int64_t)blockIdx.x * blockDim.x + threadIdx.x; i < n; i += (int64_t)gridDim.x * blockDim.x) {
-    const float gi = g[i];
-    const float mi = m[i] * beta1 + (1.f - beta1) * gi;
-    float vi = v[i] * beta2 + (1.f - beta2) * gi * gi;
-    m[i] = mi;
-    v[i] = vi;
-    if (vmax) {
-      vi = fmaxf(vmax[i], vi);
-      vmax[i] = vi;
-    }
-    const float denom = (sqrtf(vi) + eps) / sqrt_bc2;
-    p[i] = p[i] - step_size * (mi / denom);
-  }
+  for (int64_t i = (int64_t)blockIdx.x * blockDim.x + threadIdx.x; i < n; i += (int64_t)gridDim.x * blockDim.x)
+    p[i] = adam_ref1(p, g, m, v, vmax, i, beta1, beta2, eps, step_size, sqrt_bc2);
 }
 
 __global__ void rmsprop_kernel(float* __restrict__ p, const float* __restrict__ g, float* __restrict__ sq, float* __restrict__ buf,
                                int64_t n, float lr, float alpha, float eps, float momentum) {
-  for (int64_t i = (int64_t)blockIdx.x * blockDim.x + threadIdx.x; i < n; i += (int64_t)gridDim.x * blockDim.x) {
-    const float gi = g[i];
-    const float s = sq[i] * alpha + (1.f - alpha) * gi * gi;
-    sq[i] = s;
-    const float avg = sqrtf(s) + eps;
-    if (momentum > 0.f) {
-      const float bi = buf[i] * momentum + gi / avg;
-      buf[i] = bi;
-      p[i] = p[i] - lr * bi;
-    } else {
-      p[i] = p[i] - lr * (gi / avg);
+  for (int64_t i = (int64_t)blockIdx.x * blockDim.x + threadIdx.x; i < n; i += (int64_t)gridDim.x * blockDim.x)
+    p[i] = rmsprop1(p, g, sq, buf, i, lr, alpha, eps, momentum);
+}
+
+struct RepackSel { RepackEntry e[REPACK_MAX]; int n; };
+__device__ __forceinline__ void repack_select(const RepackTable& tb, uint32_t base, RepackSel& s) {
+  if (threadIdx.x == 0) s.n = 0;
+  __syncthreads();
+  if ((int)threadIdx.x < tb.n) {
+    const RepackEntry E = tb.e[threadIdx.x];
+    if (E.first <= base + 255u && base <= E.first + E.span) s.e[atomicAdd(&s.n, 1)] = E;
+  }
+  __syncthreads();
+}
+__device__ __forceinline__ void repack1(const RepackSel& s, uint32_t i, float x, float* __restrict__ packed) {
+  for (int t = 0; t < s.n; ++t) {
+    const int64_t o = repack_offset(s.e[t], i);
+    if (o >= 0) packed[o] = x;
+  }
+}
+
+__global__ __launch_bounds__(256) void adam_ref_repack_kernel(float* __restrict__ p, const float* __restrict__ g, float* __restrict__ m,
+                                                              float* __restrict__ v, float* __restrict__ vmax, int64_t n, float beta1, float beta2,
+                                                              float eps, const StepState* state, float* __restrict__ packed, const RepackTable tb) {
+  __shared__ RepackSel sel;
+  const float step_size = state->adam_step_size, sqrt_bc2 = state->adam_sqrt_bc2;
+  for (int64_t base = (int64_t)blockIdx.x * 256; base < n; base += (int64_t)gridDim.x * 256) {
+    repack_select(tb, (uint32_t)base, sel);
+    const int64_t i = base + threadIdx.x;
+    if (i < n) {
+      const float x = adam_ref1(p, g, m, v, vmax, i, beta1, beta2, eps, step_size, sqrt_bc2);
+      p[i] = x;
+      repack1(sel, (uint32_t)i, x, packed);
     }
+    __syncthreads();
+  }
+}
+
+__global__ __launch_bounds__(256) void rmsprop_repack_kernel(float* __restrict__ p, const float* __restrict__ g, float* __restrict__ sq,
+                                                             float* __restrict__ buf, int64_t n, float lr, float alpha, float eps, float momentum,
+                                                             float* __restrict__ packed, const RepackTable tb) {
+  __shared__ RepackSel sel;
+  for (int64_t base = (int64_t)blockIdx.x * 256; base < n; base += (int64_t)gridDim.x * 256) {
+    repack_select(tb, (uint32_t)base, sel);
+    const int64_t i = base + threadIdx.x;
+    if (i < n) {
+      const float x = rmsprop1(p, g, sq, buf, i, lr, alpha, eps, momentum);
+      p[i] = x;
+      repack1(sel, (uint32_t)i, x, packed);
+    }
+    __syncthreads();
   }
 }
 
@@ -778,6 +835,41 @@
   return 0;
 }
 
+static int repack_table_ok(const RepackTable& tb, const float* p, int64_t n, const float* packed, size_t packed_n) {
+  ARDAE_CHECK_ARG(packed && packed_n > 0 && n < ((int64_t)1 << 31), "update_repack: bad arguments");
+  ARDAE_CHECK_ARG(packed + packed_n <= p || p + n <= packed, "update_repack: the packed buffer overlaps the parameters");
+  ARDAE_CHECK_ARG(tb.n >= 0 && tb.n <= REPACK_MAX, "update_repack: %d table entries (at most %d)", tb.n, REPACK_MAX);
+  for (int t = 0; t < tb.n; ++t) {
+    const RepackEntry& E = tb.e[t];
+    ARDAE_CHECK_ARG(E.mode <= 2 && E.rows > 0 && E.cols > 0 && E.cols <= E.ldw && (E.mode != 2 || E.cols == 1) &&
+                        (uint64_t)E.span == (uint64_t)(E.rows - 1) * E.ldw + E.cols - 1 && (uint64_t)E.first + E.span < ((uint64_t)1 << 31),
+                    "update_repack: bad table entry %d", t);
+    const size_t need = E.mode == 2 ? E.rows : E.mode == 1 ? packed_floats((int)E.cols, (int)E.rows) : packed_floats((int)E.rows, (int)E.cols);
+    ARDAE_CHECK_ARG(E.out <= packed_n && need <= packed_n - E.out, "update_repack: table entry %d leaves the packed buffer", t);
+  }
+  return 0;
+}
+
+int launch_rmsprop_repack(float* p, const float* g, float* sq, float* buf, int64_t n, double lr, double alpha, double eps, double momentum,
+                          const RepackTable& table, float* packed, size_t packed_n, hipStream_t st) {
+  ARDAE_CHECK_ARG(p && g && sq && n > 0 && (momentum <= 0.0 || buf), "rmsprop_repack: bad arguments");
+  ARDAE_TRY(repack_table_ok(table, p, n, packed, packed_n));
+  hipLaunchKernelGGL(rmsprop_repack_kernel, dim3(grid_for(n)), dim3(256), 0, st, p, g, sq, buf, n, (float)lr, (float)alpha, (float)eps,
+                     (float)momentum, packed, table);
+  ARDAE_LAUNCH_CHECK();
+  return 0;
+}
+
+int launch_adam_ref_repack_dev(float* p, const float* g, float* m, float* v, float* vmax, int64_t n, double beta1, double beta2, double eps,
+                               const void* state, const RepackTable& table, float* packed, size_t packed_n, hipStream_t st) {
+  ARDAE_CHECK_ARG(p && g && m && v && n > 0 && state, "adam_ref_repack_dev: bad arguments");
+  ARDAE_TRY(repack_table_ok(table, p, n, packed, packed_n));
+  hipLaunchKernelGGL(adam_ref_repack_kernel, dim3(grid_for(n)), dim3(256), 0, st, p, g, m, v, vmax, n, (float)beta1, (float)beta2, (float)eps,
+                     (const StepState*)state, packed, table);
+  ARDAE_LAUNCH_CHECK();
+  return 0;
+}
+
 int launch_weight_avg(float* avg, const float* p, int64_t n, int kind, double decay, int64_t origin, const void* state, int64_t t,
                       hipStream_t st) {
   ARDAE_CHECK_ARG(avg && p && n > 0 && origin >= 1, "weight_avg: bad arguments");
diff --git a/pytorch-ardae-vae_amd/csrc/host_util.h b/pytorch-ardae-vae_amd/csrc/host_util.h
--- a/pytorch-ardae-vae_amd/csrc/host_util.h
+++ b/pytorch-ardae-vae_amd/csrc/host_util.h
@@ -77,8 +77,33 @@
     f = panel(l.w + col0, l.in, l.out, k, false);
     b = panel(l.w + col0, l.in, k, l.out, true);
   }
+  struct Column { const float* src; int stride, n; float* out; };
+  std::vector<Column> columns;
+  size_t column(size_t src, int stride, int n) {
+    const size_t o = take(n);
+    if (packed) columns.push_back(Column{params + src, stride, n, packed + o});
+    return o;
+  }
   size_t total() const { return off; }
-  int launch(hipStream_t st) { return launch_pack_batch(items.data(), (int)items.size(), st); }
+  int launch(hipStream_t st) {
+    for (const Column& c : columns) ARDAE_TRY(launch_gather_strided(c.src, c.stride, c.n, c.out, st));
+    return launch_pack_batch(items.data(), (int)items.size(), st);
+  }
+  int repack_table(RepackTable& tb) const {
+    tb.n = 0;
+    auto add = [&](const float* src, int ldw, int rows, int cols, int mode, const float* out) {
+      ARDAE_CHECK_ARG(tb.n < REPACK_MAX, "update_repack: the pack list has more than %d entries", REPACK_MAX);
+      ARDAE_CHECK_ARG(src >= params && (src < (const float*)packed || src >= (const float*)packed + off), "update_repack: a panel of this network is not made of parameters");
+      RepackEntry& E = tb.e[tb.n++];
+      E.first = (uint32_t)(src - params); E.ldw = (uint32_t)ldw; E.rows = (uint32_t)rows; E.cols = (uint32_t)cols; E.mode = (uint32_t)mode;
+      E.span = (uint32_t)(rows - 1) * (uint32_t)ldw + (uint32_t)cols - 1;
+      E.out = (uint64_t)(out - packed);
+      return 0;
+    };
+    for (const PackItem& p : items) ARDAE_TRY(p.transpose ? add(p.W, p.ldw, p.k, p.nout, 1, p.out) : add(p.W, p.ldw, p.nout, p.k, 0, p.out));
+    for (const Column& c : columns) ARDAE_TRY(add(c.src, c.stride, c.n, 1, 2, c.out));
+    return 0;
+  }
 };
 
 struct WgradList {
@@ -189,6 +214,7 @@
                               DevFloat beta, float dloss, float* workspace, size_t wsf, hipStream_t);
   int (*vae_backward_sampler)(const ardae_model_desc&, const float* params, const float* packed, const float* x, const float* noise, int B, int nz,
                               const float* dz_extra, DevFloat seed_scale, float* workspace, size_t wsf, float* grads, float grads_beta, hipStream_t);
+  int (*repack_table)(const ardae_model_desc&, const float* params, float* packed, RepackTable& table, size_t* packed_n);
 };
 inline unsigned no_caps(const ardae_model_desc&) { return 0; }
 inline int desc_flags_ok(const ardae_model_desc* d, int allowed) {
@@ -214,6 +240,13 @@
   const Packed K(P, pl);
   return pl.launch(st);
 }
+template <class Layout, class Packed> int family_repack_table(const ardae_model_desc& d, const float* params, float* packed, RepackTable& table, size_t* packed_n) {
+  const Layout P(d);
+  PackList pl(params, packed);
+  const Packed K(P, pl);
+  *packed_n = pl.total();
+  return pl.repack_table(table);
+}
 
 template <class Layout, class Packed, class Ws> struct Entry {
   const Layout P; const Packed K; Bump ws; Ws W{};
diff --git a/pytorch-ardae-vae_amd/csrc/ipmodel.h b/pytorch-ardae-vae_amd/csrc/ipmodel.h
--- a/pytorch-ardae-vae_amd/csrc/ipmodel.h
+++ b/pytorch-ardae-vae_amd/csrc/ipmodel.h
@@ -117,6 +117,7 @@
   if constexpr (F::mlp_decoder) f.decode = mlp_decode<typename F::Layout, typename F::Packed>;
   else f.decode = ip_decode<F>;
   f.vae_forward = ip_vae_forward<F>; f.vae_backward = ip_vae_backward<F>;
+  if (pack == family_pack<typename F::Layout, typename F::Packed>) f.repack_table = family_repack_table<typename F::Layout, typename F::Packed>;
   return f;
 }
 }
diff --git a/pytorch-ardae-vae_amd/csrc/model.hip b/pytorch-ardae-vae_amd/csrc/model.hip
--- a/pytorch-ardae-vae_amd/csrc/model.hip
+++ b/pytorch-ardae-vae_amd/csrc/model.hip
@@ -12,52 +12,10 @@
 #include "ipmodel.h"
 #include "elementwise.h"
 #include "mlp.h"
+#include "model_layout.h"
 
 namespace ardae {
 namespace {
-
-struct ModelLayout {
-  int kind, D, nd, h, zd, nl, act;
-  std::vector<Lin> inp, stack, dec, heads;
-  std::vector<bool> stack_noise;
-  size_t total = 0;
-  explicit ModelLayout(const ardae_model_desc& d)
-      : kind(d.kind), D(d.input_dim), nd(d.noise_dim), h(d.h_dim), zd(d.z_dim), nl(d.n_layers), act(d.act) {
-    size_t off = 0;
-    auto add = [&](std::vector<Lin>& v, int out, int in) { v.push_back(next_lin(off, out, in)); };
-    const int n_inp = kind == 0 ? nl + 2 : nl;
-    for (int l = 0; l < n_inp; ++l) add(inp, h, l == 0 ? D : h);
-    if (kind == 0) {
-      add(stack, h, h + nd); stack_noise.push_back(true);
-      add(stack, zd, h); stack_noise.push_back(false);
-    } else {
-      for (int l = 0; l < nl; ++l) { add(stack, h, h + nd); stack_noise.push_back(true); }
-      add(stack, zd, h + nd); stack_noise.push_back(true);
-    }
-    const int n_dec = kind == 0 ? nl + 1 : nl;
-    for (int l = 0; l < n_dec; ++l) add(dec, h, l == 0 ? zd : h);
-    add(heads, D, h);
-    if (kind == 1) add(heads, D, h);
-    total = off;
-  }
-};
-
-struct ModelPacked {
-  MlpStack inp;
-  std::vector<size_t> sh_f, sh_b, sn_f;
-  MlpDecoder dec;
-  ModelPacked(const ModelLayout& P, PackList& pl) : inp(P.inp.data(), P.inp.size(), pl) {
-    const size_t ns = P.stack.size();
-    sh_f.resize(ns); sh_b.resize(ns); sn_f.assign(ns, 0);
-    for (size_t i = 0; i < ns; ++i) {
-      const Lin& l = P.stack[i];
-      pl.pair(l, sh_f[i], sh_b[i], 0, P.h);
-      if (P.stack_noise[i]) sn_f[i] = pl.panel(l.w + P.h, l.in, l.out, P.nd, false);
-    }
-    dec = MlpDecoder(P.dec.data(), P.dec.size(), P.heads.data(), (int)P.heads.size(), pl);
-  }
-  explicit ModelPacked(const ModelLayout& P, PackList&& sizing = PackList()) : ModelPacked(P, sizing) {}
-};
 
 struct ModelWs {
   float* x2;
@@ -246,6 +204,36 @@
   return family(d).pack(*d, params, packed, (hipStream_t)stream);
 }
 
+static int model_repack_table(const ardae_model_desc* d, const float* params, float* packed, int64_t n, RepackTable& tb, size_t* packed_n) {
+  ARDAE_TRY(desc_ok(d));
+  ARDAE_CHECK_ARG(params && packed, "model update_repack: null pointer");
+  ARDAE_CHECK_ARG(family(d).repack_table != nullptr, "model update_repack: this kind's pack composes weights: update, then ardae_model_pack");
+  ARDAE_CHECK_ARG(n > 0 && (size_t)n <= family(d).param_floats(*d), "model update_repack: n = %lld floats, the network has %zu", (long long)n, family(d).param_floats(*d));
+  return family(d).repack_table(*d, params, packed, tb, packed_n);
+}
+int ardae_model_update_repack_ok(const ardae_model_desc* d) {
+  if (desc_ok(d) || family(d).repack_table == nullptr) return 0;
+  float* const params = reinterpret_cast<float*>(uintptr_t(1) << 20);
+  RepackTable tb;
+  size_t packed_n = 0;
+  return family(d).repack_table(*d, params, params + family(d).param_floats(*d), tb, &packed_n) == 0 ? 1 : 0;
+}
+int ardae_model_rmsprop_repack_step(const ardae_model_desc* d, float* params, const float* g, float* square_avg, float* momentum_buffer, int64_t n,
+                                    double lr, double alpha, double eps, double momentum, float* packed, void* stream) {
+  RepackTable tb;
+  size_t packed_n = 0;
+  ARDAE_TRY(model_repack_table(d, params, packed, n, tb, &packed_n));
+  return launch_rmsprop_repack(params, g, square_avg, momentum_buffer, n, lr, alpha, eps, momentum, tb, packed, packed_n, (hipStream_t)stream);
+}
+int ardae_model_adam_ref_repack_step_dev(const ardae_model_desc* d, float* params, const float* g, float* exp_avg, float* exp_avg_sq,
+                                         float* max_exp_avg_sq, int64_t n, double beta1, double beta2, double eps, const void* state, float* packed,
+                                         void* stream) {
+  RepackTable tb;
+  size_t packed_n = 0;
+  ARDAE_TRY(model_repack_table(d, params, packed, n, tb, &packed_n));
+  return launch_adam_ref_repack_dev(params, g, exp_avg, exp_avg_sq, max_exp_avg_sq, n, beta1, beta2, eps, state, tb, packed, packed_n, (hipStream_t)stream);
+}
+
 static int model_common(const ardae_model_desc* d, const float* params, const float* packed, const float* x, int B, int nz,
                         float* workspace, size_t wsf, int mode) {
   ARDAE_TRY(desc_ok(d));
diff --git a/pytorch-ardae-vae_amd/csrc/model_layout.h b/pytorch-ardae-vae_amd/csrc/model_layout.h
--- /dev/null
+++ b/pytorch-ardae-vae_amd/csrc/model_layout.h
@@ -0,0 +1,52 @@
+#pragma once
+#include <vector>
+
+#include "ardae_hip.h"
+#include "mlp.h"
+
+namespace ardae {
+
+struct ModelLayout {
+  int kind, D, nd, h, zd, nl, act;
+  std::vector<Lin> inp, stack, dec, heads;
+  std::vector<bool> stack_noise;
+  size_t total = 0;
+  explicit ModelLayout(const ardae_model_desc& d)
+      : kind(d.kind), D(d.input_dim), nd(d.noise_dim), h(d.h_dim), zd(d.z_dim), nl(d.n_layers), act(d.act) {
+    size_t off = 0;
+    auto add = [&](std::vector<Lin>& v, int out, int in) { v.push_back(next_lin(off, out, in)); };
+    const int n_inp = kind == 0 ? nl + 2 : nl;
+    for (int l = 0; l < n_inp; ++l) add(inp, h, l == 0 ? D : h);
+    if (kind == 0) {
+      add(stack, h, h + nd); stack_noise.push_back(true);
+      add(stack, zd, h); stack_noise.push_back(false);
+    } else {
+      for (int l = 0; l < nl; ++l) { add(stack, h, h + nd); stack_noise.push_back(true); }
+      add(stack, zd, h + nd); stack_noise.push_back(true);
+    }
+    const int n_dec = kind == 0 ? nl + 1 : nl;
+    for (int l = 0; l < n_dec; ++l) add(dec, h, l == 0 ? zd : h);
+    add(heads, D, h);
+    if (kind == 1) add(heads, D, h);
+    total = off;
+  }
+};
+
+struct ModelPacked {
+  MlpStack inp;
+  std::vector<size_t> sh_f, sh_b, sn_f;
+  MlpDecoder dec;
+  ModelPacked(const ModelLayout& P, PackList& pl) : inp(P.inp.data(), P.inp.size(), pl) {
+    const size_t ns = P.stack.size();
+    sh_f.resize(ns); sh_b.resize(ns); sn_f.assign(ns, 0);
+    for (size_t i = 0; i < ns; ++i) {
+      const Lin& l = P.stack[i];
+      pl.pair(l, sh_f[i], sh_b[i], 0, P.h);
+      if (P.stack_noise[i]) sn_f[i] = pl.panel(l.w + P.h, l.in, l.out, P.nd, false);
+    }
+    dec = MlpDecoder(P.dec.data(), P.dec.size(), P.heads.data(), (int)P.heads.size(), pl);
+  }
+  explicit ModelPacked(const ModelLayout& P, PackList&& sizing = PackList()) : ModelPacked(P, sizing) {}
+};
+
+}
diff --git a/pytorch-ardae-vae_amd/engine.py b/pytorch-ardae-vae_amd/engine.py
--- a/pytorch-ardae-vae_amd/engine.py
+++ b/pytorch-ardae-vae_amd/engine.py
@@ -67,9 +67,11 @@
 
     RNG_STRIDE = RNG_STRIDE
 
-    def __init__(self, model, cdae, cfg: TrainConfig, batch_size, process_group=None, graph=True, force_dp=False, dp_comm="auto"):
+    def __init__(self, model, cdae, cfg: TrainConfig, batch_size, process_group=None, graph=True, force_dp=False, dp_comm="auto",
+                 fused_update=True):
         model._require_gpu()
         cdae._require_gpu()
+        self.fused_update = bool(fused_update)
         if int(cdae._desc.kind) not in (0, 1, 16, 17):
             raise TypeError(f"ArdaeEngine trains a conditional AR-DAE (net.MLPGradCARDAE / net.MLPResCARDAE), not a {type(cdae).__name__}: its step "
                             "block has no slot for a noise level beside beta (a plain conditional DAE runs in ArdaeCondScoreEngine)")
@@ -91,6 +93,7 @@
         if self.comm is not None and (self.comm.world, self.comm.rank) != (self.world, self.rank):
             raise ValueError(f"dp_comm is rank {self.comm.rank} of {self.comm.world}, the process group says {self.rank} of {self.world}")
         md, cd = model._desc, cdae._desc
+        self._fused_model = self.fused_update and bool(L.query("ardae_model_update_repack_ok", md))
         B, nzc, nzm = self.B, cfg.nz_cdae, cfg.nz_model
         N = B * nzc
         z, nd = model.z_dim, model._noise_width
@@ -375,10 +378,11 @@
     def _cdae_update(self):
         if self._in_step and self.opt_c.adam:
             self.opt_c.advance()
-        self.opt_c.apply(self.grads_c, self._in_step)
+        packed = self.opt_c.apply(self.grads_c, self._in_step, ("ardae_cdae", self.cdae._desc, self.pk_c) if self.fused_update else None)
         if not self._in_step:
             self.opt_c.steps += 1
-        self._pack_cdae()
+        if not packed:
+            self._pack_cdae()
 
     def _data_context(self, x, out):
         D = int(self.model.input_dim)
@@ -441,7 +445,7 @@
                    self.ws_vae, self.ws_vae.numel(), self.grads_m, 0.0)
 
     def _model_update(self):
-        self.opt_m.apply(self.grads_m, self._in_step)
+        packed = self.opt_m.apply(self.grads_m, self._in_step, ("ardae_model", self.model._desc, self.pk_m) if self._fused_model else None)
         if self.avg is not None:
             L.call("ardae_weight_avg", self.avg, self.model._flat, self.avg.numel(), WEIGHT_AVG_KINDS[self.wavg], float(self.cfg.m_weight_avg_decay),
                    self._avg_origin, self.state, 0)
@@ -449,7 +453,8 @@
             self.step_count += 1
             self.opt_m.steps = self.step_count
             self.opt_m.advance(self.RNG_STRIDE)
-        self._pack_model()
+        if not packed:
+            self._pack_model()
 
     def vae_phase(self, x, noise=None, beta=None, apply_update=True):
         nv = self.vae_forward_part(x, noise, beta)
diff --git a/pytorch-ardae-vae_amd/engine_common.py b/pytorch-ardae-vae_amd/engine_common.py
--- a/pytorch-ardae-vae_amd/engine_common.py
+++ b/pytorch-ardae-vae_amd/engine_common.py
@@ -98,8 +98,20 @@
         else:
             L.call("ardae_step_state_advance", self.state, rng_inc, self.lr, self.beta1, 0.999)
 
-    def apply(self, grads, in_step):
+    def apply(self, grads, in_step, repack=None):
         p, g = self.flat, grads
+        if repack is not None and self.kind == "rmsprop":
+            prefix, desc, packed = repack
+            L.call(prefix + "_rmsprop_repack_step", desc, p, g, self.a, self.b, self.n, self.lr, 0.99, 1e-8, self.momentum, packed)
+            return True
+        if repack is not None and self.kind in ("adam", "amsgrad") and in_step:
+            prefix, desc, packed = repack
+            L.call(prefix + "_adam_ref_repack_step_dev", desc, p, g, self.a, self.b, self.c, self.n, self.beta1, 0.999, 1e-8, self.state, packed)
+            return True
+        self._apply_plain(p, g, in_step)
+        return False
+
+    def _apply_plain(self, p, g, in_step):
         if self.kind == "sgd":
             L.call("ardae_sgd_step", p, g, self.n, self.lr)
         elif self.kind == "rmsprop":
```

Result: no change. 218.5 (-0.4%).
